# solemnwind/fast-go-icp

Hardware: AMD Instinct MI355X
Metric: BnB subcubes/sec + wall-clock to global optimum, bunny 40k pts, 1/2/4/8 GPU (higher is better)
Workload: dtype f32; 1 GPU; bunny-shape synthetic pair (nt=40256, ns=40097), lut_resolution=0.005, mse_threshold=5e-05, full FastGoICP::run() per step; schedule=round

## Files before the change

fast-go-icp_amd/_lib.py:

```python
import ctypes as C
import os

from . import build as _build

c_float_p = C.POINTER(C.c_float)
c_int_p = C.POINTER(C.c_int)
c_uint32_p = C.POINTER(C.c_uint32)
c_uint8_p = C.POINTER(C.c_uint8)
c_double_p = C.POINTER(C.c_double)


class CtxInfo(C.Structure):
    _fields_ = [("struct_size", C.c_size_t), ("lut_dims", C.c_int * 3), ("lut_layout", C.c_int), ("lut_nodes", C.c_uint64), ("lut_bytes", C.c_uint64),
                ("source_points_per_face_voxel", C.c_double), ("points_per_item", C.c_int), ("items_per_evaluation", C.c_int),
                ("max_subcubes_per_window", C.c_int), ("source_order", C.c_int), ("tree_order", C.c_int), ("chunks_per_item_with_thresholds", C.c_int)]


class CloudStats(C.Structure):
    _fields_ = [("n", C.c_uint64), ("centroid", C.c_float * 3), ("min", C.c_float * 3), ("max", C.c_float * 3), ("max_abs_centred", C.c_float),
                ("rms_radius", C.c_float)]


class Exchange(C.Structure):
    ALLREDUCE_MIN = C.CFUNCTYPE(C.c_int, c_float_p, C.c_size_t, C.c_void_p)
    ALLGATHER = C.CFUNCTYPE(C.c_int, c_float_p, c_float_p, C.c_size_t, C.c_void_p)
    ALLGATHER_DEVICE = C.CFUNCTYPE(C.c_int, C.c_void_p, C.c_size_t, C.c_void_p)
    _fields_ = [("struct_size", C.c_size_t), ("rank", C.c_int), ("world_size", C.c_int), ("allreduce_min", ALLREDUCE_MIN),
                ("allgather", ALLGATHER), ("user", C.c_void_p), ("allgather_device", ALLGATHER_DEVICE)]

    def __init__(self, rank=0, world_size=1, allreduce_min=None, allgather=None, user=None, allgather_device=None):
        super().__init__()
        self.struct_size = C.sizeof(Exchange)
        self.rank, self.world_size, self.user = rank, world_size, user
        if allreduce_min is not None:
            self.allreduce_min = allreduce_min
        if allgather is not None:
            self.allgather = allgather
        if allgather_device is not None:
            self.allgather_device = allgather_device


class SolverOpts(C.Structure):
    _fields_ = [("schedule", C.c_int), ("round_width", C.c_int), ("ctx_flags", C.c_uint), ("device", C.c_int), ("trim_fraction", C.c_float)]


class RunStats(C.Structure):
    _fields_ = [("trans_cubes", C.c_uint64), ("bounds_calls", C.c_uint64), ("rot_cubes", C.c_uint64),
                ("icp_runs", C.c_uint64), ("icp_iters", C.c_uint64), ("inner_bnb", C.c_uint64),
                ("rounds", C.c_uint64), ("seconds_total", C.c_double), ("seconds_bnb", C.c_double),
                ("seconds_icp", C.c_double), ("initial_icp_sse", C.c_double)]

    def as_dict(self):
        return {n: getattr(self, n) for n, _ in self._fields_}


FLAG_NO_WEIGHT_QUANT = 1 << 0
FLAG_NO_MORTON = 1 << 1
FLAG_PROFILE = 1 << 2
FLAG_BRUTE_FORCE_NN = 1 << 3
FLAG_CURVE_ORDER = 1 << 4
class BatchPair(C.Structure):
    _fields_ = [("tgt_xyz", c_float_p), ("nt", C.c_size_t), ("src_xyz", c_float_p), ("ns", C.c_size_t), ("lut_resolution", C.c_float),
                ("mse_threshold", C.c_float)]


class BatchOpts(C.Structure):
    _fields_ = [("struct_size", C.c_size_t), ("solver", SolverOpts), ("max_live", C.c_int), ("trim_fractions", c_float_p),
                ("alignment", C.c_int)]
# ... 130 lines not shown

    def __init__(self):
        super().__init__()
        self.struct_size = C.sizeof(MeshInfo)


OUTLIER_STATISTICAL = 0
OUTLIER_RADIUS = 1

SCHEDULE_SERIAL = 0
SCHEDULE_ROUND = 1

_SIGS = {
    "fgoicp_last_error": (C.c_char_p, []),
    "fgoicp_version": (C.c_char_p, []),
    "fgoicp_dev_knobs": (C.c_int, []),
    "fgoicp_abi_version": (C.c_int, []),
    "fgoicp_ctx_create": (C.c_int, [c_float_p, C.c_size_t, c_float_p, C.c_size_t, c_float_p, C.c_float, C.c_int, C.c_uint,
                                    C.POINTER(C.c_void_p)]),
    "fgoicp_ctx_destroy": (None, [C.c_void_p]),
    "fgoicp_lut_dims": (C.c_int, [C.c_void_p, c_int_p]),
    "fgoicp_ctx_get_info": (C.c_int, [C.c_void_p, C.POINTER(CtxInfo)]),
    "fgoicp_cloud_stats": (C.c_int, [c_float_p, C.c_size_t, C.POINTER(CloudStats)]),
    "fgoicp_voxel_downsample": (C.c_int, [c_float_p, C.c_size_t, C.c_float, c_float_p, C.c_int, c_float_p, C.c_size_t, c_uint32_p, c_uint32_p, C.POINTER(VoxelInfo)]),
    "fgoicp_remove_outliers": (C.c_int, [c_float_p, C.c_size_t, C.c_int, C.c_int, C.c_float, C.c_int, c_float_p, C.c_size_t, c_uint32_p, c_uint8_p, c_double_p, c_float_p,
                                         C.POINTER(OutlierInfo)]),
    "fgoicp_farthest_point_sample": (C.c_int, [c_float_p, C.c_size_t, C.c_size_t, C.c_size_t, C.c_int, c_float_p, c_uint32_p, c_float_p, c_float_p, c_uint32_p,
                                               C.POINTER(FpsInfo)]),
    "fgoicp_cluster_dbscan": (C.c_int, [c_float_p, C.c_size_t, C.c_float, C.c_int, C.c_size_t, C.c_int, c_float_p, C.c_size_t, c_uint32_p, C.POINTER(C.c_int32), c_uint32_p,
                                        C.POINTER(C.c_uint64), C.c_size_t, C.POINTER(ClusterInfo)]),
    "fgoicp_segment_planes": (C.c_int, [c_float_p, C.c_size_t, C.c_float, C.c_int, C.c_uint64, C.c_int, C.c_size_t, C.c_int, C.c_int, C.c_int, c_float_p, C.c_size_t,
                                        c_uint32_p, C.POINTER(C.c_int32), C.POINTER(SegmentModel), C.c_size_t, C.c_size_t, C.POINTER(SegmentInfo)]),
    "fgoicp_segment_hypotheses": (C.c_int, [c_float_p, C.c_size_t, c_uint32_p, C.c_size_t, C.c_int, C.c_uint64, C.c_int, c_uint32_p, C.POINTER(C.c_double), c_uint8_p]),
    "fgoicp_segment_fit_from_moments": (C.c_int, [C.c_uint64, C.POINTER(C.c_double), C.POINTER(C.c_double), C.POINTER(C.c_double), C.POINTER(C.c_double),
                                                  C.POINTER(C.c_double)]),
    "fgoicp_mesh_sample": (C.c_int, [c_float_p, C.c_size_t, c_uint32_p, C.c_size_t, C.c_size_t, C.c_uint64, C.c_int, c_float_p, c_float_p, c_uint32_p, c_double_p, c_double_p,
                                     C.POINTER(MeshInfo)]),
    "fgoicp_solver_set_target_normals": (C.c_int, [C.c_void_p, c_float_p]),
    "fgoicp_solver_set_source_normals": (C.c_int, [C.c_void_p, c_float_p]),
    "fgoicp_lut_read": (C.c_int, [C.c_void_p, c_float_p, C.c_size_t]),
    "fgoicp_lut_search": (C.c_int, [C.c_void_p, c_float_p, C.c_size_t, c_float_p]),
    "fgoicp_lut_nodes": (C.c_int, [C.c_void_p, c_int_p, C.c_size_t, c_float_p]),
    "fgoicp_bounds_point_distances": (C.c_int, [C.c_void_p, c_float_p, C.c_float, c_float_p, C.c_int, c_float_p]),
    "fgoicp_ctx_sort_fallbacks": (C.c_int, [C.c_void_p, C.POINTER(C.c_uint64), C.POINTER(C.c_uint64)]),
    "fgoicp_ctx_test_sort_fault": (C.c_int, [C.c_void_p, C.c_int]),
    "fgoicp_test_live_resources": (C.c_int, [C.POINTER(C.c_uint64)]),
    "fgoicp_bounds_batch": (C.c_int, [C.c_void_p, c_float_p, C.c_float, c_float_p, C.c_int, C.c_int, c_float_p, c_float_p]),
    "fgoicp_bounds_multi": (C.c_int, [C.c_void_p, C.c_int, c_float_p, c_float_p, c_int_p, c_int_p, c_float_p, c_float_p,
                                      c_float_p]),
    "fgoicp_bounds_submit": (C.c_int, [C.c_void_p, C.c_int, C.c_int, c_float_p, c_float_p, c_int_p, c_int_p, c_float_p]),
    "fgoicp_bounds_submit_twins": (C.c_int, [C.c_void_p, C.c_int, C.c_int, c_float_p, c_float_p, c_int_p, c_int_p, c_float_p, c_int_p]),
    "fgoicp_bounds_submit_cut": (C.c_int, [C.c_void_p, C.c_int, C.c_int, c_float_p, c_float_p, c_int_p, c_int_p, c_float_p, c_int_p, c_float_p]),
    "fgoicp_bounds_submit_leaf": (C.c_int, [C.c_void_p, C.c_int, C.c_int, c_float_p, c_float_p, c_int_p, c_int_p, c_float_p, c_int_p, c_float_p, c_float_p]),
    "fgoicp_ctx_cut_stats": (C.c_int, [C.c_void_p, C.POINTER(C.c_uint64), C.POINTER(C.c_uint64), C.c_int]),
    "fgoicp_solver_set_early_exit": (C.c_int, [C.c_void_p, C.c_int]),
    "fgoicp_bounds_collect": (C.c_int, [C.c_void_p, C.c_int, c_float_p, c_float_p]),
    "fgoicp_sse": (C.c_int, [C.c_void_p, c_float_p, c_float_p, c_float_p]),
    "fgoicp_alignment": (C.c_int, [C.c_void_p, c_float_p, c_float_p, c_uint32_p, c_float_p, c_uint8_p, c_uint8_p, C.POINTER(AlignmentSummary)]),
    "fgoicp_solver_alignment": (C.c_int, [C.c_void_p, c_uint32_p, c_float_p, c_uint8_p, c_uint8_p, C.POINTER(AlignmentSummary)]),
    "fgoicp_batch_alignment": (C.c_int, [C.c_void_p, C.c_int, c_uint32_p, c_float_p, c_uint8_p, c_uint8_p, C.POINTER(AlignmentSummary)]),
    "fgoicp_information": (C.c_int, [C.c_void_p, c_float_p, c_float_p, C.c_float, C.POINTER(Information)]),
    "fgoicp_solver_information": (C.c_int, [C.c_void_p, C.c_float, C.POINTER(Information)]),
    "fgoicp_batch_information": (C.c_int, [C.c_void_p, C.c_int, C.POINTER(Information)]),
    "fgoicp_information_from_moments": (C.c_int, [C.c_uint64, C.POINTER(C.c_double), C.POINTER(C.c_double), c_float_p, C.c_float, C.POINTER(C.c_double),
                                                  C.POINTER(C.c_double), C.POINTER(C.c_double)]),
    "fgoicp_ctx_set_target_normals": (C.c_int, [C.c_void_p, c_float_p, C.c_int]),
    "fgoicp_target_normals": (C.c_int, [C.c_void_p, c_float_p]),
    "fgoicp_target_knn": (C.c_int, [C.c_void_p, C.c_int, c_uint32_p, c_float_p]),
    "fgoicp_plane_moments": (C.c_int, [C.c_void_p, c_float_p, c_float_p, C.c_float, C.POINTER(PlaneMoments)]),
    "fgoicp_plane_step_from_moments": (C.c_int, [C.c_uint64, C.POINTER(C.c_double), C.POINTER(C.c_double), c_int_p]),
    "fgoicp_plane_apply_step": (C.c_int, [c_float_p, c_float_p, C.POINTER(C.c_double), c_float_p, c_float_p]),
    "fgoicp_icp_plane": (C.c_int, [C.c_void_p, c_float_p, c_float_p, C.c_size_t, C.c_float, C.c_float, C.POINTER(PlaneResult)]),
    "fgoicp_solver_refine_plane": (C.c_int, [C.c_void_p, C.c_int, C.c_size_t, C.c_float, C.c_float, C.POINTER(PlaneResult)]),
    "fgoicp_ctx_set_source_normals": (C.c_int, [C.c_void_p, c_float_p, C.c_int]),
    "fgoicp_source_normals": (C.c_int, [C.c_void_p, c_float_p]),
    "fgoicp_gicp_moments": (C.c_int, [C.c_void_p, c_float_p, c_float_p, C.c_float, C.c_double, C.POINTER(PlaneMoments)]),
    "fgoicp_icp_gicp": (C.c_int, [C.c_void_p, c_float_p, c_float_p, C.c_size_t, C.c_float, C.c_float, C.c_double, C.POINTER(PlaneResult)]),
    "fgoicp_solver_refine_gicp": (C.c_int, [C.c_void_p, C.c_int, C.c_size_t, C.c_float, C.c_float, C.c_double, C.POINTER(PlaneResult)]),
    "fgoicp_gicp_terms": (C.c_int, [c_float_p, c_float_p, c_float_p, c_float_p, c_float_p, C.c_double, C.POINTER(C.c_double), C.POINTER(C.c_double)]),
    "fgoicp_robust_weight": (C.c_int, [C.c_int, C.c_double, C.c_double, C.POINTER(C.c_double)]),
    "fgoicp_robust_moments": (C.c_int, [C.c_void_p, c_float_p, c_float_p, C.c_float, C.c_int, C.c_double, C.c_int, C.c_double, C.POINTER(RobustMoments)]),
    "fgoicp_robust_residuals": (C.c_int, [C.c_void_p, c_float_p, c_float_p, C.c_float, C.c_int, C.c_double, C.c_int, C.c_double, C.POINTER(C.c_double),
                                          C.POINTER(C.c_double), c_uint8_p]),
    "fgoicp_robust_scale": (C.c_int, [C.c_void_p, c_float_p, c_float_p, C.c_float, C.c_int, C.c_double, C.POINTER(C.c_double)]),
    "fgoicp_icp_robust": (C.c_int, [C.c_void_p, c_float_p, c_float_p, C.c_size_t, C.c_float, C.c_float, C.c_int, C.c_double, C.c_int, C.c_double, C.POINTER(RobustResult)]),
    "fgoicp_solver_refine_robust": (C.c_int, [C.c_void_p, C.c_int, C.c_int, C.c_size_t, C.c_float, C.c_float, C.c_double, C.c_int, C.c_double, C.POINTER(RobustResult)]),
    "fgoicp_icp": (C.c_int, [C.c_void_p, c_float_p, c_float_p, C.c_size_t, C.c_float, c_float_p, c_float_p, c_float_p, c_int_p]),
    "fgoicp_icp_batch": (C.c_int, [C.c_void_p, C.c_int, c_float_p, c_float_p, C.c_size_t, C.c_float, c_float_p, c_float_p, c_float_p, c_int_p]),
    "fgoicp_procrustes": (C.c_int, [C.c_void_p, c_float_p, c_float_p, c_float_p, c_float_p, c_float_p, c_int_p]),
    "fgoicp_ctx_set_inliers": (C.c_int, [C.c_void_p, C.c_size_t]),
    "fgoicp_ctx_profile": (C.c_int, [C.c_void_p, C.POINTER(C.c_double), C.POINTER(C.c_uint64), C.POINTER(C.c_uint64), C.c_int]),
    "fgoicp_ctx_profile_evaluations": (C.c_int, [C.c_void_p, C.POINTER(C.c_uint64)]),
    "fgoicp_ctx_profile_select_ms": (C.c_int, [C.c_void_p, C.POINTER(C.c_double)]),
    "fgoicp_ctx_trim_stats": (C.c_int, [C.c_void_p, C.POINTER(C.c_uint64), C.c_int]),
    "fgoicp_ctx_set_coop_split": (C.c_int, [C.c_void_p, C.c_size_t, C.c_size_t]),
    "fgoicp_ctx_set_profile": (C.c_int, [C.c_void_p, C.c_int]),
    "fgoicp_ctx_ns": (C.c_size_t, [C.c_void_p]),
    "fgoicp_ctx_nt": (C.c_size_t, [C.c_void_p]),
    "fgoicp_solver_create": (C.c_int, [c_float_p, C.c_size_t, c_float_p, C.c_size_t, C.c_float, C.c_float,
                                       C.POINTER(SolverOpts), C.POINTER(C.c_void_p)]),
    "fgoicp_solver_destroy": (None, [C.c_void_p]),
    "fgoicp_solver_set_exchange": (C.c_int, [C.c_void_p, C.POINTER(Exchange)]),
    "fgoicp_solver_set_log": (C.c_int, [C.c_void_p, C.c_void_p, C.c_void_p]),
    "fgoicp_solver_run": (C.c_int, [C.c_void_p, c_float_p, c_float_p]),
    "fgoicp_solver_best_error": (C.c_int, [C.c_void_p, c_float_p]),
    "fgoicp_solver_best_transform": (C.c_int, [C.c_void_p, c_float_p, c_float_p]),
# ... 99 lines not shown
```

fast-go-icp_amd/csrc/device/bounds_item.hpp:

```cpp
#pragma once

constexpr double kCutMargin = 1.000001;

typedef float f2v __attribute__((ext_vector_type(2)));
typedef float f4v __attribute__((ext_vector_type(4)));
typedef unsigned u4v __attribute__((ext_vector_type(4)));

__device__ __forceinline__ f2v pk_fma(f2v a, f2v b, f2v c) { return __builtin_elementwise_fma(a, b, c); }
__device__ __forceinline__ f2v splat2(float v) { return f2v{v, v}; }

struct ItemGeom {
    f2v off_xy, dmax_xy;
    float off_z, dmax_z, scale;
    float pyf;
    int px;
    int c0;
    unsigned nbx3, nby2;
    unsigned nby3;
};
__device__ __forceinline__ ItemGeom item_geom(const LutGeom& g) {
    ItemGeom G;
    G.off_xy = f2v{g.off_x, g.off_y};
    G.dmax_xy = f2v{(float)(g.dx - 1), (float)(g.dy - 1)};
    G.off_z = g.off_z;
// ... 103 lines not shown
            const float4a send = odd ? qp[k].r1 : qp[k].r2;
            float4a recv;
            recv.x = swap_lane_pair(send.x); recv.y = swap_lane_pair(send.y); recv.z = swap_lane_pair(send.z); recv.w = swap_lane_pair(send.w);
            const float4a a = odd ? recv : qp[k].r1, b = odd ? qp[k].r2 : recv;
            ga[k] = f4v{a.x, a.y, a.z, a.w};
            gb[k] = f4v{b.x, b.y, b.z, b.w};
        }
    }
    float te0[TRIM ? P : 1], te1[TRIM ? P : 1];
#pragma unroll
    for (int k = 0; k < P; ++k) {
        float dsq;
        if (LAYOUT == 1 || LAYOUT == 6) dsq = item_blend(tx[k], f2v{ga[k].x, ga[k].y}, f2v{ga[k].z, ga[k].w}, f2v{gb[k].x, gb[k].y}, f2v{gb[k].z, gb[k].w});
        else dsq = item_blend(tx[k], f2v{ga[k].x, ga[k].y}, f2v{gb[k].x, gb[k].y}, f2v{ga[k].z, ga[k].w}, f2v{gb[k].z, gb[k].w});
        const float d1 = sqrtf(dsq);
        const float d0 = d1 - 2.0f * p[k].w * sin_half;
        const int i = first + 64 * k;
        if (TRIM) {
            const float e0 = fmaxf(MODE == 1 ? d0 : d1, 0.0f), e1 = fmaxf(d0, 0.0f);
            if (FULL || i < ns) {
                row0[i] = e0;
                if (MODE == 2) row1[i] = e1;
            }
            te0[k] = e0;
            te1[k] = e1;
            continue;
        }
        if (MODE != 1) {
            const float m = fmaxf(d1, 0.0f), l = fmaxf(d1 - trans_radius, 0.0f);
            const float ubv = m * m, lbv = l * l;
            acc[0] += (FULL || i < ns) ? (double)ubv : 0.0;
            acc[1] += (FULL || i < ns) ? (double)lbv : 0.0;
        }
        if (MODE != 0) {
            const float m = fmaxf(d0, 0.0f), l = fmaxf(d0 - trans_radius, 0.0f);
            const float ubv = m * m, lbv = l * l;
            acc[MODE == 2 ? 2 : 0] += (FULL || i < ns) ? (double)ubv : 0.0;
            acc[MODE == 2 ? 3 : 1] += (FULL || i < ns) ? (double)lbv : 0.0;
        }
    }
    if (TRIM && samp_shift > 0) {
        const size_t off = trim_sample_offset(ns);
#pragma unroll
        for (int k = 0; k < P; ++k) {
            const int i = first + 64 * k;
            if ((FULL || i < ns) && trim_is_sample(i, samp_shift, ns)) {
                row0[off + (size_t)(i >> samp_shift)] = te0[k];
                if (MODE == 2) row1[off + (size_t)(i >> samp_shift)] = te1[k];
            }
        }
    }
}

template <int LAYOUT, int TRIM, bool WIDE, bool QUANT, int MODE>
__device__ __forceinline__ void item_walk(const float4* __restrict__ src, int ns, const char* __restrict__ lutp, const ItemGeom& G, const float (&R)[9], f2v t_xy, float t_z,
                                          float sin_half, float trans_radius, int base, int chunk_pts, int lane, double (&acc)[4], float* __restrict__ row0,
                                          float* __restrict__ row1, int samp_shift) {
    const int odd = lane & 1;
    for (int pass = 0; pass < chunk_pts; pass += 256) {
        const int first = base + pass + lane;
        if (base + pass + 256 <= ns)
            item_pass<LAYOUT, TRIM, WIDE, QUANT, MODE, true>(src, ns, lutp, G, R, t_xy, t_z, sin_half, trans_radius, first, odd, acc, row0, row1, samp_shift);
        else
            item_pass<LAYOUT, TRIM, WIDE, QUANT, MODE, false>(src, ns, lutp, G, R, t_xy, t_z, sin_half, trans_radius, first, odd, acc, row0, row1, samp_shift);
    }
}

template <int LAYOUT, int TRIM, bool WIDE, bool QUANT, bool SPAN >
__global__ __launch_bounds__(64) void bounds_item_kernel(const float4* __restrict__ src, int ns, const char* __restrict__ lutp, LutGeom g,
                                                         const TickGroup* __restrict__ groups, const TickSub* __restrict__ subs, const unsigned* __restrict__ sorted,
                                                         int nchunk, int chunk_pts, double2* __restrict__ partials, float* __restrict__ evals, size_t erow, int samp_shift,
                                                         unsigned nitems, unsigned* __restrict__ sort_err, TickCut cut, int span ) {
    unsigned slot;
    if (!TRIM && cut.tier_split && sorted) {
        const unsigned n0 = min(*cut.tier_split, gridDim.x);
        slot = blockIdx.x < n0 ? xcd_remap(blockIdx.x, n0) : n0 + xcd_remap(blockIdx.x - n0, gridDim.x - n0);
    } else {
        slot = xcd_remap(blockIdx.x, gridDim.x);
    }
    const unsigned item = sorted ? sorted[slot] : slot;
    if (item >= nitems) {
        if (sort_err && threadIdx.x == 0) *sort_err = 1u;
        return;
    }
    const unsigned per_eval = SPAN ? ((unsigned)nchunk + (unsigned)span - 1u) / (unsigned)span : (unsigned)nchunk;
    const int s = (int)(item / per_eval);
    const int chunk0 = (int)(item - (unsigned)s * per_eval) * (SPAN ? span : 1);
    const int nsub = SPAN ? min(span, nchunk - chunk0) : 1;
    const int lane = (int)threadIdx.x;
    const TickSub sb = subs[s];
    bool cutting = false, term0 = false, term1 = false;
    if (!TRIM && cut.acc) {
        TickGate* const gate = cut.gate + s;
        const unsigned long long gw = __hip_atomic_load(reinterpret_cast<unsigned long long*>(gate), __ATOMIC_RELAXED, __HIP_MEMORY_SCOPE_WORKGROUP);
        if (__builtin_amdgcn_readfirstlane((int)(unsigned)gw) && !(cut.probe & 4)) return;
        const unsigned flags = (unsigned)__builtin_amdgcn_readfirstlane((int)(unsigned)(gw >> 32));
        cutting = (flags & kGateCutting) != 0u;
        term0 = (flags & kGateTerm0) != 0u;
        term1 = (flags & kGateTerm1) != 0u;
        if (cutting && !(cut.probe & 1)) {
            const double a0 = __hip_atomic_load(&cut.acc[2 * (size_t)s], __ATOMIC_RELAXED, __HIP_MEMORY_SCOPE_AGENT);
            const double a1 = sb.dual ? __hip_atomic_load(&cut.acc[2 * (size_t)s + 1], __ATOMIC_RELAXED, __HIP_MEMORY_SCOPE_AGENT) : 0.0;
            const bool reached = a0 >= (double)sb.cut0 * kCutMargin && (!sb.dual || a1 >= (double)sb.cut1 * kCutMargin);
            if (__builtin_amdgcn_readfirstlane((int)reached)) {
                if (lane == 0) __hip_atomic_store(&gate->done, 1u, __ATOMIC_RELAXED, __HIP_MEMORY_SCOPE_AGENT);
                return;
            }
        }
    }
    const TickGroup gr = groups[sb.group];
    float R[9];
#pragma unroll
    for (int k = 0; k < 9; ++k) R[k] = gr.R[k];
    const ItemGeom G = item_geom(g);
    const float trans_radius = kSqrt3 * sb.span;
    const f2v t_xy = f2v{sb.tx, sb.ty};
    float* row0 = TRIM ? evals + (size_t)sb.out0 * erow : nullptr;
    float* row1 = TRIM ? evals + (size_t)sb.out1 * erow : nullptr;
    double lb_fix = 0.0, lb_rot = 0.0;
    for (int sub = 0; sub < (SPAN ? nsub : 1); ++sub) {
        const int chunk = chunk0 + sub;
        const int base = chunk * chunk_pts;
        double acc[4] = {0.0, 0.0, 0.0, 0.0};
        if (sb.dual) item_walk<LAYOUT, TRIM, WIDE, QUANT, 2>(src, ns, lutp, G, R, t_xy, sb.tz, gr.sin_half, trans_radius, base, chunk_pts, lane, acc, row0, row1, samp_shift);
        else if (gr.fix_rot) item_walk<LAYOUT, TRIM, WIDE, QUANT, 0>(src, ns, lutp, G, R, t_xy, sb.tz, gr.sin_half, trans_radius, base, chunk_pts, lane, acc, row0, row1, samp_shift);
        else item_walk<LAYOUT, TRIM, WIDE, QUANT, 1>(src, ns, lutp, G, R, t_xy, sb.tz, gr.sin_half, trans_radius, base, chunk_pts, lane, acc, row0, row1, samp_shift);
        if (TRIM) continue;
        const double r0 = wave_sum(acc[0]), r1 = wave_sum(acc[1]);
        lb_fix += term0 ? r0 : r1;
        if (sb.dual) {
            const double r2 = wave_sum(acc[2]), r3 = wave_sum(acc[3]);
            lb_rot += term1 ? r2 : r3;
            if (lane == 0) {
                partials[(size_t)sb.out0 * nchunk + chunk] = make_double2(r0, r1);
                partials[(size_t)sb.out1 * nchunk + chunk] = make_double2(r2, r3);
            }
        } else if (lane == 0) {
            partials[(size_t)sb.out0 * nchunk + chunk] = make_double2(r0, r1);
        }
    }
    if (!TRIM && cutting && lane == 0 && !(cut.probe & 2)) {
        unsafeAtomicAdd(&cut.acc[2 * (size_t)s], lb_fix);
        if (sb.dual) unsafeAtomicAdd(&cut.acc[2 * (size_t)s + 1], lb_rot);
    }
}
```

fast-go-icp_amd/csrc/device/ctx.hip:

```cpp
#include <hip/hip_runtime.h>

#include <algorithm>
#include <chrono>
#include <limits>
#include <memory>
#include <cmath>
#include <cstddef>
#include <cstdio>
#include <cstdlib>
#include <cstring>
#include <numeric>
#include <string>
#include <thread>
#include <vector>

#include "../../../include/fgoicp_amd.h"
#include "../host/math3.hpp"
#include "../host/knobs.hpp"
#include "ctx.hpp"
#include "kernels.hpp"
#include "arena.hpp"
#include "morton.hpp"

namespace fgoicp {
// ... 19 lines not shown
            const hipError_t q = query();
            if (q != hipErrorNotReady) return q;
#if defined(__x86_64__)
            __builtin_ia32_pause();
#endif
            if ((spins & 15u) == 15u && std::chrono::steady_clock::now() - t0 > std::chrono::microseconds(g_spin_sync_us)) break;
        }
    }
    return block();
}
static hipError_t wait_event(hipEvent_t ev) { return spin_then_block([&] { return hipEventQuery(ev); }, [&] { return hipEventSynchronize(ev); }); }
static hipError_t wait_stream(hipStream_t st) { return spin_then_block([&] { return hipStreamQuery(st); }, [&] { return hipStreamSynchronize(st); }); }

int ctx_flush_profile(fgoicp_ctx* c) {
    for (int i = 0; i < c->ev_used; ++i) {
        float ms = 0.f;
        HIPCHK(hipEventElapsedTime(&ms, c->ev_start[i], c->ev_stop[i]));
        c->prof_ms += ms;
        static const bool tick_log = dev_env("FGOICP_TICK_LOG") != nullptr;
        if (tick_log && i < (int)c->ev_evals.size()) std::fprintf(stderr, "[tick] evals %d us %.1f\n", c->ev_evals[i], ms * 1e3);
        if (c->ev_has_sel[i]) {
            HIPCHK(hipEventSynchronize(c->ev_sel_stop[i]));
            HIPCHK(hipEventElapsedTime(&ms, c->ev_sel_start[i], c->ev_sel_stop[i]));
            c->prof_sel_ms += ms;
            c->ev_has_sel[i] = 0;
        }
    }
    c->ev_used = 0;
    return FGOICP_OK;
}

namespace {
struct TickTiming {
    bool on = dev_env("FGOICP_TIMING") != nullptr;
    double pack = 0, enqueue = 0, wait = 0, copyout = 0;
    uint64_t ticks = 0;
};
TickTiming g_tt;
constexpr float kNoCut = std::numeric_limits<float>::infinity();
inline double now_s() { return std::chrono::duration<double>(std::chrono::steady_clock::now().time_since_epoch()).count(); }
}

static int tick_launch_window(fgoicp_ctx* c, fgoicp_ctx::TickSlot& sl) {
    const int ng = sl.win_groups, neval = sl.win_evals, rows = sl.win_rows;
    const int span = sl.win_cut ? c->cut_span : 1;
    const int per_eval = (c->nchunk1 + span - 1) / span;
    const bool tiers = sl.win_cut && c->cut_tier_level > 0.0f;
    const size_t nitems = (size_t)neval * (size_t)per_eval;
    const bool small = nitems <= (size_t)c->small_tick_items;
    const TickGroup* dev_groups = small ? sl.h_groups.dev() : sl.d_groups;
    const TickSub* dev_subs = small ? sl.h_subs.dev() : sl.d_subs;
    TickCut cut;
    if (sl.win_cut) { cut.acc = sl.d_cut_acc; cut.gate = sl.d_cut_gate; cut.row_cut = sl.d_row_cut; cut.row_term = sl.d_row_term; cut.stat = c->d_cut_stat; }
    if (tiers && !small) cut.tier_split = sl.d_cursor + kTickTierSplit;
    static const int cut_probe = [] { const char* e = dev_env("FGOICP_CUT_PROBE"); return e ? std::atoi(e) : 0; }();
    cut.probe = cut_probe;
    *sl.h_sort_err = 0u;
    unsigned* fused_err = !small && c->sort_check ? sl.h_sort_err.dev() : nullptr;
    if (!small) {
        static const int upload_kernel = [] { const char* e = dev_env("FGOICP_UPLOAD_KERNEL"); return e ? std::atoi(e) : 1; }();
        if (upload_kernel) {
            launch_tick_upload(sl.h_groups.dev(), sl.d_groups, ng, sl.h_subs.dev(), sl.d_subs, neval, sl.sort_stream);
        } else {
            HIPCHK(hipMemcpyAsync(sl.d_groups, sl.h_groups, sizeof(TickGroup) * ng, hipMemcpyHostToDevice, sl.sort_stream));
            HIPCHK(hipMemcpyAsync(sl.d_subs, sl.h_subs, sizeof(TickSub) * neval, hipMemcpyHostToDevice, sl.sort_stream));
        }
        ++c->sorted_ticks;
        const int fault = c->sort_fault_tick && c->sorted_ticks == (uint64_t)c->sort_fault_tick;
        launch_tick_sort(c->geom, span > 1 ? c->d_span_cen : c->d_chunk_cen, per_eval, sl.d_groups, sl.d_subs, neval, c->cell_shift, sl.d_keys, sl.d_ranks, sl.d_hist, sl.d_hist_xcd, sl.d_xoff, sl.d_block_sums, sl.d_cursor, sl.d_sorted,
                         c->sort_xcd ? 1 : 0, c->sort_check ? 1 : 0, fault, sl.sort_stream, tiers ? c->d_lut : nullptr, c->cut_tier_level / (float)c->ns,
                         sl.win_cut ? &cut : nullptr, sl.d_partials, c->nchunk1, span);
        HIPCHK(hipEventRecord(sl.sorted_ev, sl.sort_stream));
        HIPCHK(hipStreamWaitEvent(sl.stream, sl.sorted_ev, 0));
    } else if (sl.win_cut) {
        launch_tick_prefill(dev_subs, neval, c->nchunk1, cut, sl.d_partials, sl.stream);
    }
    hipEvent_t e0 = nullptr, e1 = nullptr;
    if (c->profile) {
        if (c->ev_used == (int)c->ev_start.size()) {
            HIPCHK(hipStreamSynchronize(c->stream));
            int rc = ctx_flush_profile(c);
            if (rc) return rc;
        }
        e0 = c->ev_start[c->ev_used];
        e1 = c->ev_stop[c->ev_used];
        if ((int)c->ev_evals.size() <= c->ev_used) c->ev_evals.resize(c->ev_start.size(), 0);
        c->ev_evals[c->ev_used] = neval;
        c->ev_used++;
        c->prof_launches++;
        c->prof_subcubes += rows;
        c->prof_evals += neval;
    }
    const bool cut_on = launch_bounds_sorted(c->d_src, (int)c->ns, c->d_lut_zp, c->lut_layout, c->geom, c->nchunk1, c->chunk_pts, dev_groups, dev_subs, neval, small ? nullptr : sl.d_sorted,
                                             sl.d_partials, c->inliers ? sl.d_evals : nullptr, c->erow, c->trim_samp_shift, fused_err, cut, span, e0, e1, sl.stream);
    if (cut_on) c->cut_items_offered += (size_t)neval * c->nchunk1;
    hipStream_t fin = c->finalize_on_side ? sl.sort_stream : sl.stream;
    if (fin != sl.stream) {
        HIPCHK(hipEventRecord(sl.bounds_ev, sl.stream));
        HIPCHK(hipStreamWaitEvent(fin, sl.bounds_ev, 0));
    }
    if (c->inliers) {
        const int pi = e0 ? c->ev_used - 1 : -1;
        if (pi >= 0) { HIPCHK(hipEventRecord(c->ev_sel_start[pi], fin)); c->ev_has_sel[pi] = 1; }
        launch_trim_rows(sl.d_evals, c->erow, (int)c->ns, (int)c->inliers, rows, sl.h_row_span.dev(), sl.h_ub.dev(), sl.h_lb.dev(), fin, c->trim_samp_shift, c->trim_margin, c->d_trim_stat);
        if (pi >= 0) HIPCHK(hipEventRecord(c->ev_sel_stop[pi], fin));
    } else
        launch_bounds_finalize(sl.d_partials, c->nchunk1, rows, sl.h_lb.dev(), sl.h_ub.dev(), cut_on ? cut : TickCut(), fin);
    HIPCHK(hipGetLastError());
    HIPCHK(hipEventRecord(sl.done, fin));
    return FGOICP_OK;
}

static int tick_enqueue_window(fgoicp_ctx* c, fgoicp_ctx::TickSlot& sl, int G, const float* R9, const float* rot_span, const int* fix_rot,
                               const int* offsets, const float* tn4, const int* twin, const float* cut_above, const float* ub_below_span, int pos, int* end_out) {
    const double t0 = g_tt.on ? now_s() : 0;
    int g = 0;
    while (g < G && offsets[g + 1] <= pos) ++g;
    const int cap = c->inliers ? std::min(c->max_subcubes, c->vals_rows) : c->max_subcubes;
    int end = pos, ng = 0;
    sl.row_group.resize((size_t)cap);
    for (int gg = g; gg < G && ng < c->max_groups && end - pos < cap; ++gg) {
        TickGroup& tg = sl.h_groups[ng];
        std::memcpy(tg.R, R9 + 9 * gg, sizeof(tg.R));
        const float half_angle = rot_span[gg] * kSqrt3 * kPi / 2.0f;
        tg.sin_half = std::sin(half_angle);
        tg.fix_rot = fix_rot[gg] ? 1 : 0;
        tg.pad_ = gg;
        const int first = std::max(offsets[gg], pos);
        const int last = std::min(offsets[gg + 1], pos + cap);
        for (int i = first; i < last; ++i) sl.row_group[(size_t)(i - pos)] = ng;
        end = std::max(end, last);
        ++ng;
        if (last < offsets[gg + 1]) break;
    }
    const int rows = end - pos;
    *end_out = end;
    if (rows <= 0) return FGOICP_OK;
    static const bool leaf_rule = [] { const char* e = dev_env("FGOICP_CUT_LEAF"); return !e || std::atoi(e) != 0; }();
    const auto terminal = [&](int sub_group, float span) { return leaf_rule && cut_above && ub_below_span && span < ub_below_span[sub_group]; };
    int neval = 0;
    for (int r = 0; r < rows; ++r) {
        const int i = pos + r;
        const int gi = sl.row_group[(size_t)r];
        sl.h_row_span[r] = tn4[4 * (size_t)i + 3];
        int j = twin ? twin[i] : -1;
        if (j >= pos && j < end && j != i && twin[j] == i) {
            const int gj = sl.row_group[(size_t)(j - pos)];
            const TickGroup &a = sl.h_groups[gi], &b = sl.h_groups[gj];
            const bool ok = a.fix_rot != b.fix_rot && a.sin_half == b.sin_half && std::memcmp(a.R, b.R, sizeof(a.R)) == 0 &&
                            std::memcmp(tn4 + 4 * (size_t)i, tn4 + 4 * (size_t)j, 4 * sizeof(float)) == 0;
            if (ok) {
                if (j < i) continue;
                TickSub& ts = sl.h_subs[neval++];
                ts.tx = tn4[4 * (size_t)i]; ts.ty = tn4[4 * (size_t)i + 1]; ts.tz = tn4[4 * (size_t)i + 2]; ts.span = tn4[4 * (size_t)i + 3];
                ts.group = gi;
                ts.out0 = a.fix_rot ? r : j - pos;
                ts.out1 = a.fix_rot ? j - pos : r;
                ts.dual = 1;
                const float ca = cut_above ? cut_above[a.pad_] : kNoCut, cb = cut_above ? cut_above[b.pad_] : kNoCut;
                ts.cut0 = a.fix_rot ? ca : cb;
                ts.cut1 = a.fix_rot ? cb : ca;
                const unsigned ta = terminal(a.pad_, ts.span) ? 1u : 0u, tb = terminal(b.pad_, ts.span) ? 1u : 0u;
                ts.term = a.fix_rot ? (ta * kSubTerm0 | tb * kSubTerm1) : (tb * kSubTerm0 | ta * kSubTerm1);
                ts.pad_ = 0;
                continue;
            }
        }
        TickSub& ts = sl.h_subs[neval++];
        ts.tx = tn4[4 * (size_t)i]; ts.ty = tn4[4 * (size_t)i + 1]; ts.tz = tn4[4 * (size_t)i + 2]; ts.span = tn4[4 * (size_t)i + 3];
        ts.group = gi;
        ts.out0 = r;
        ts.out1 = r;
        ts.dual = 0;
        ts.cut0 = ts.cut1 = cut_above ? cut_above[sl.h_groups[gi].pad_] : kNoCut;
        ts.term = terminal(sl.h_groups[gi].pad_, ts.span) ? kSubTerm0 : 0u;
        ts.pad_ = 0;
    }
    sl.win_cut = cut_above != nullptr && !c->inliers;
    for (int k = 0; k < ng; ++k) sl.h_groups[k].pad_ = 0;
    const double t1 = g_tt.on ? now_s() : 0;
    sl.win_pos = pos;
    sl.win_rows = rows;
    sl.win_groups = ng;
    sl.win_evals = neval;
    const int rc = tick_launch_window(c, sl);
    if (g_tt.on) { g_tt.pack += t1 - t0; g_tt.enqueue += now_s() - t1; g_tt.ticks++; }
    return rc;
}

static int tick_wait_window(fgoicp_ctx* c, fgoicp_ctx::TickSlot& sl) {
    const double t2 = g_tt.on ? now_s() : 0;
    HIPCHK(wait_event(sl.done));
    if (*sl.h_sort_err) {
        c->sort_xcd = false;
        c->sort_fallbacks++;
        HIPCHK(hipStreamSynchronize(sl.sort_stream));
        HIPCHK(hipMemsetAsync(sl.d_hist, 0, sizeof(unsigned) * kTickNumKeys, sl.sort_stream));
        HIPCHK(hipMemsetAsync(sl.d_hist_xcd, 0, sizeof(unsigned) * 16 * kTickNumKeys, sl.sort_stream));
        int rc = tick_launch_window(c, sl);
        if (rc) return rc;
        HIPCHK(hipEventSynchronize(sl.done));
        if (*sl.h_sort_err) { set_error("tick sort did not produce a permutation of the work items (device-scope atomics)"); return FGOICP_ERR_HIP; }
    }
#ifdef FGOICP_DEV_KNOBS
    const bool cut_verify = [] { const char* e = dev_env("FGOICP_CUT_VERIFY"); return e && std::atoi(e) != 0; }();
    if (cut_verify && sl.win_cut) {
        const int rows = sl.win_rows;
        std::vector<float> lb(sl.h_lb.get(), sl.h_lb + rows), ub(sl.h_ub.get(), sl.h_ub + rows);
        sl.win_cut = false;
        int rc = tick_launch_window(c, sl);
        sl.win_cut = true;
        if (rc) return rc;
        HIPCHK(hipEventSynchronize(sl.done));
        if (*sl.h_sort_err) { set_error("FGOICP_CUT_VERIFY: the repeated window's sort failed"); return FGOICP_ERR_HIP; }
        for (int e = 0; e < sl.win_evals; ++e) {
            const TickSub& ts = sl.h_subs[e];
            for (int v = 0; v < (ts.dual ? 2 : 1); ++v) {
                const int r = v ? ts.out1 : ts.out0;
                const float T = v ? ts.cut1 : ts.cut0;
                const bool term = (ts.term & (v ? kSubTerm1 : kSubTerm0)) != 0u;
                const bool above = (term ? sl.h_ub[r] : sl.h_lb[r]) >= T;
                const bool ok = above ? (lb[(size_t)r] == T && ub[(size_t)r] == T)
                                      : (std::memcmp(&lb[(size_t)r], &sl.h_lb[r], 4) == 0 && std::memcmp(&ub[(size_t)r], &sl.h_ub[r], 4) == 0);
                c->cut_verify_rows++;
                c->cut_verify_above += above ? 1 : 0;
                if (!ok) {
                    if (c->cut_verify_bad++ < 5)
                        std::fprintf(stderr, "[fgoicp cut verify] row %d: threshold %.9g, exact {%.9g, %.9g}, reported {%.9g, %.9g}\n", r, (double)T, (double)sl.h_lb[r], (double)sl.h_ub[r],
                                     (double)lb[(size_t)r], (double)ub[(size_t)r]);
                }
            }
        }
        c->cut_verify_windows++;
        std::memcpy(sl.h_lb, lb.data(), sizeof(float) * rows);
        std::memcpy(sl.h_ub, ub.data(), sizeof(float) * rows);
    }
#endif
    const double t3 = g_tt.on ? now_s() : 0;
    std::memcpy(sl.lb.data() + sl.win_pos, sl.h_lb, sizeof(float) * sl.win_rows);
    std::memcpy(sl.ub.data() + sl.win_pos, sl.h_ub, sizeof(float) * sl.win_rows);
    if (g_tt.on) { g_tt.wait += t3 - t2; g_tt.copyout += now_s() - t3; }
    return FGOICP_OK;
}

int ctx_bounds_submit(fgoicp_ctx* c, int slot, int G, const float* R9, const float* rot_span, const int* fix_rot, const int* offsets,
                      const float* tn4, const int* twin, const float* cut_above, const float* ub_below_span) {
    HIPCHK(hipSetDevice(c->device));
    fgoicp_ctx::TickSlot& sl = c->slots[slot];
    if (sl.inflight) { set_error("fgoicp_bounds_submit: slot still in flight (collect it first)"); return FGOICP_ERR_INVALID_ARG; }
    sl.total = offsets[G];
    sl.lb.resize(sl.total);
    sl.ub.resize(sl.total);
    sl.win_rows = 0;
    int pos = 0;
    while (pos < sl.total) {
        int end = pos;
        int rc = tick_enqueue_window(c, sl, G, R9, rot_span, fix_rot, offsets, tn4, twin, cut_above, ub_below_span, pos, &end);
        if (rc) return rc;
        if (end <= pos) break;
        pos = end;
        if (pos < sl.total) {
            rc = tick_wait_window(c, sl);
            if (rc) return rc;
            sl.win_rows = 0;
        }
    }
    sl.inflight = true;
    return FGOICP_OK;
}

int ctx_cut_stats(fgoicp_ctx* c, uint64_t* items_offered, uint64_t* items_cut, int reset) {
    HIPCHK(hipSetDevice(c->device));
    unsigned long long now = 0;
    if (c->d_cut_stat) {
        unsigned long long part[kCutStatSlots];
        HIPCHK(hipDeviceSynchronize());
        HIPCHK(hipMemcpy(part, c->d_cut_stat, sizeof(part), hipMemcpyDeviceToHost));
        for (unsigned long long v : part) now += v;
    }
    if (items_offered) *items_offered = c->cut_items_offered;
    if (items_cut) *items_cut = (uint64_t)now - c->cut_stat_base;
    if (reset) { c->cut_items_offered = 0; c->cut_stat_base = (uint64_t)now; }
    return FGOICP_OK;
}

int ctx_bounds_collect(fgoicp_ctx* c, int slot, float* lb_out, float* ub_out) {
    HIPCHK(hipSetDevice(c->device));
    fgoicp_ctx::TickSlot& sl = c->slots[slot];
    if (!sl.inflight) { set_error("fgoicp_bounds_collect: nothing submitted on this slot"); return FGOICP_ERR_INVALID_ARG; }
    if (sl.win_rows > 0) {
        int rc = tick_wait_window(c, sl);
        if (rc) return rc;
    }
    sl.inflight = false;
    std::memcpy(lb_out, sl.lb.data(), sizeof(float) * sl.total);
    std::memcpy(ub_out, sl.ub.data(), sizeof(float) * sl.total);
    if (c->profile && !c->slots[0].inflight && !c->slots[1].inflight) {
        int rc = ctx_flush_profile(c);
        if (rc) return rc;
    }
    return FGOICP_OK;
}

int ctx_bounds_multi(fgoicp_ctx* c, int G, const float* R9, const float* rot_span, const int* fix_rot, const int* offsets,
                     const float* tn4, float* lb_out, float* ub_out, const float* cut_above) {
    HIPCHK(hipSetDevice(c->device));
    int rc = ctx_bounds_submit(c, 0, G, R9, rot_span, fix_rot, offsets, tn4, nullptr, cut_above);
    if (rc) return rc;
    return ctx_bounds_collect(c, 0, lb_out, ub_out);
}

static double tree64(double (&v)[64]) {
    for (int off = 32; off > 0; off >>= 1)
        for (int i = 0; i < off; ++i) v[i] += v[i + off];
    return v[0];
}
static double fold_blocks(const double* bp, int nblocks, int width, int k) {
    double lane[64] = {0};
    for (int b = 0; b < nblocks; ++b) lane[b & 63] += bp[(size_t)b * width + k];
    return tree64(lane);
}
static double fold_wave_sums(const double* w, int nwaves) {
    double lane[64] = {0};
    const int nblocks = (nwaves + 3) / 4;
    for (int b = 0; b < nblocks; ++b) {
        double blk = w[4 * b];
        for (int k = 1; k < 4; ++k) blk += 4 * b + k < nwaves ? w[4 * b + k] : 0.0;
        lane[b & 63] += blk;
    }
    return tree64(lane);
}
static bool icp_fused(const fgoicp_ctx* c) { return c->icp_fuse && !c->brute_force_nn && !c->inliers && c->ns <= 262144; }

static bool trim_skips(const fgoicp_ctx* c) { return c->inliers && c->trim_skip; }

// ... 1027 lines not shown
    if (c->brute_force_nn) {
        Dev<float4> d_tgt_shift;
        e3 = d_tgt_shift.alloc(nt);
        if (e3 == hipSuccess) e3 = hipMemcpy(d_tgt_shift, hs.data(), sizeof(float4) * nt, hipMemcpyHostToDevice);
        if (e3 == hipSuccess) {
            launch_lut_build(d_tgt_shift, (int)nt, g, c->d_lut, c->stream);
            e3 = hipGetLastError();
            if (e3 == hipSuccess) e3 = hipStreamSynchronize(c->stream);
        }
    } else {
        std::vector<uint32_t> order;
        c->tree_order = bvh_kd_order() ? 1 : 0;
        HIPCHK(bvh_upload(bvh_build_host(h.data(), nt, &order), &c->bvh_tgt));
        BvhOwned shifted;
        e3 = bvh_upload(bvh_build_host(hs.data(), nt, &order), &shifted);
        Dev<float> scratch;
        if (e3 == hipSuccess) e3 = scratch.alloc(total);
        static const bool want_idx = [] { const char* e = dev_env("FGOICP_LUT_INDEX"); return e && std::atoi(e) != 0; }();
        if (e3 == hipSuccess && want_idx && c->d_lut_idx.alloc(total) != hipSuccess) (void)hipGetLastError();
        if (e3 == hipSuccess) {
            launch_lut_build_scan(shifted.view(), g, scratch, c->d_lut, c->stream, c->d_lut_idx);
            e3 = hipGetLastError();
            if (e3 == hipSuccess) e3 = hipStreamSynchronize(c->stream);
        }
    }
    if (e3 != hipSuccess) { set_error(std::string("LUT build failed: ") + hipGetErrorString(e3)); return e3 == hipErrorOutOfMemory ? FGOICP_ERR_OOM : FGOICP_ERR_HIP; }
    g.idx = c->d_lut_idx;
    return FGOICP_OK;
}
int create_packed_lut(fgoicp_ctx* c) {
    const LutGeom& g = c->geom;
    const size_t total = (size_t)g.px * g.py * g.pz;
    const double face_voxels = (double)g.dx * g.dy + (double)g.dy * g.dz + (double)g.dx * g.dz;
    int layout = ((double)c->ns / face_voxels < 0.5 && total * sizeof(float4) <= ((size_t)16 << 30)) ? 2 : 1;
    const size_t apron_bytes = packed_lut_bytes(g, 4);
    if (layout == 2 && apron_bytes <= ((size_t)16 << 30)) layout = 4;
    if (layout == 4 && apron_bytes > ((size_t)256 << 20)) layout = 6;
    if (const char* e = dev_env("FGOICP_LUT_ZPAIR")) { const int v = std::atoi(e); if (v == 1 || v == 2 || v == 4 || v == 6) layout = v; }
    if ((layout == 4 || layout == 6) && (g.px > 1023 || g.py > 1023 || g.pz > 1023)) layout = 2;
    c->lut_layout = layout;
    if (layout == 6) {
        HIPCHK(c->d_lut_zp.alloc(packed_lut_bytes(g, 6) / sizeof(float2)));
        launch_lut_zpair_apron(c->d_lut, g, c->d_lut_zp, c->stream);
    } else if (layout == 4) {
        HIPCHK(c->d_lut_zp.alloc(apron_bytes / sizeof(float2)));
        launch_lut_quad_apron(c->d_lut, g, reinterpret_cast<float4*>(c->d_lut_zp.get()), c->stream);
    } else if (layout == 2) {
        HIPCHK(c->d_lut_zp.alloc(total * 2));
        launch_lut_quad(c->d_lut, g, reinterpret_cast<float4*>(c->d_lut_zp.get()), c->stream);
    } else {
        HIPCHK(c->d_lut_zp.alloc(total));
        launch_lut_zpair(c->d_lut, g, c->d_lut_zp, c->stream);
    }
    HIPCHK(hipGetLastError());
    HIPCHK(hipStreamSynchronize(c->stream));
    return FGOICP_OK;
}
int create_window_sizes(fgoicp_ctx* c) {
    const LutGeom& g = c->geom;
    const size_t ns = c->ns;
    const double face_voxels = (double)g.dx * g.dy + (double)g.dy * g.dz + (double)g.dx * g.dz;
    const double density = (double)ns / face_voxels;
    c->chunk_pts = density >= 1.0 ? 2048 : density >= 0.5 ? 1024 : density >= 0.25 ? 512 : 256;
    if (const char* e = dev_env("FGOICP_CHUNK_PTS")) {
        const int v = std::atoi(e);
        if (v == 256 || v == 512 || v == 1024 || v == 2048 || v == 4096) c->chunk_pts = v;
    }
    const size_t nchunk1 = (ns + c->chunk_pts - 1) / c->chunk_pts;
    const size_t fit = ((size_t)4 << 30) / (nchunk1 * (sizeof(double2) + 2 * sizeof(unsigned) + sizeof(unsigned short)));
    c->max_subcubes = (int)std::max<size_t>(4096, std::min<size_t>(131072, fit));
    if (const char* e = dev_env("FGOICP_MAX_SUBCUBES")) c->max_subcubes = std::max(kMaxBatch, std::min(1 << 18, std::atoi(e)));
    const size_t launch_fit = (((size_t)1 << 24) - 1) / nchunk1;
    if (launch_fit < (size_t)kMaxBatch) {
        set_error("fgoicp_ctx_create: source cloud too large for one bounds launch per batch (ns > ~134M)");
        return FGOICP_ERR_TOO_LARGE;
    }
    c->max_subcubes = (int)std::min<size_t>((size_t)c->max_subcubes, launch_fit);
    c->nchunk1 = (int)nchunk1;
    c->max_groups = std::max(512, c->max_subcubes / 8);
    if (const char* e = dev_env("FGOICP_FINALIZE_SIDE")) c->finalize_on_side = std::atoi(e) != 0;
    if (const char* e = dev_env("FGOICP_ICP_SEED")) c->icp_seeding = std::atoi(e) != 0;
    if (const char* e = dev_env("FGOICP_COOP_SPLIT_MIN")) c->coop_split_min = c->coop_split_trim_min = (size_t)std::max(0L, std::atol(e));
    if (const char* e = dev_env("FGOICP_SMALL_TICK")) c->small_tick_items = std::max(0, std::atoi(e));
    const int maxd = std::max(g.dx, std::max(g.dy, g.dz));
    c->cell_shift = 0;
    while ((maxd >> c->cell_shift) > 32) ++c->cell_shift;
    c->cut_span = c->chunk_pts == 256 ? 2 : 1;
    if (const char* e = dev_env("FGOICP_CUT_TIERS")) c->cut_tier_level = (float)std::atof(e);
    if (const char* e = dev_env("FGOICP_CUT_SPAN")) { const int v = std::atoi(e); if (v == 1 || v == 2 || v == 4) c->cut_span = v; }
    return FGOICP_OK;
}
int create_run_centres(fgoicp_ctx* c, const float* src_xyz, size_t pts, Dev<float4>& d_cen) {
    const size_t ns = c->ns, n = (ns + pts - 1) / pts;
    std::vector<float4> cen(n);
    for (size_t k = 0; k < n; ++k) {
        double sx = 0, sy = 0, sz = 0;
        const size_t a = k * pts, b = std::min(ns, a + pts);
        for (size_t i = a; i < b; ++i) {
            const float* p = src_xyz + 3 * (size_t)c->perm[i];
            sx += p[0]; sy += p[1]; sz += p[2];
        }
        const double inv = 1.0 / (double)(b - a);
        cen[k] = make_float4((float)(sx * inv), (float)(sy * inv), (float)(sz * inv), 0.f);
    }
    HIPCHK(d_cen.alloc(n));
    HIPCHK(hipMemcpy(d_cen, cen.data(), sizeof(float4) * n, hipMemcpyHostToDevice));
    return FGOICP_OK;
}
int create_tick_slot(fgoicp_ctx* c, fgoicp_ctx::TickSlot& sl) {
    const size_t subcubes = (size_t)c->max_subcubes, max_items = subcubes * c->nchunk1;
    sl.stream.borrow(c->stream);
    HIPCHK(sl.done.create(hipEventDisableTiming));
    const char* e = dev_env("FGOICP_SORT_STREAM");
    if (e && std::atoi(e) == 0) sl.sort_stream.borrow(c->stream);
    else {
        const char* pe = dev_env("FGOICP_SIDE_PRIORITY");
        const int pri = pe ? std::atoi(pe) : 0;
        int least = 0, greatest = 0;
        if (pri) HIPCHK(hipDeviceGetStreamPriorityRange(&least, &greatest));
        if (pri) HIPCHK(sl.sort_stream.create(hipStreamNonBlocking, pri < 0 ? greatest : least));
        else HIPCHK(sl.sort_stream.create(hipStreamNonBlocking));
    }
    for (Event* ev : {&sl.sorted_ev, &sl.bounds_ev}) HIPCHK(ev->create(hipEventDisableTiming));
    HIPCHK(sl.d_groups.alloc(c->max_groups));
    HIPCHK(sl.d_subs.alloc(subcubes));
    HIPCHK(sl.h_groups.alloc(c->max_groups));
    HIPCHK(sl.h_subs.alloc(subcubes));
    HIPCHK(sl.h_row_span.alloc(subcubes));
    HIPCHK(sl.h_sort_err.alloc(4));
    *sl.h_sort_err = 0u;
    HIPCHK(sl.d_keys.alloc(max_items));
    HIPCHK(sl.d_ranks.alloc(max_items));
    HIPCHK(sl.d_hist.alloc(kTickNumKeys));
    HIPCHK(hipMemset(sl.d_hist, 0, sizeof(unsigned) * kTickNumKeys));
    HIPCHK(sl.d_block_sums.alloc(64));
    HIPCHK(sl.d_hist_xcd.alloc(16 * kTickNumKeys));
    HIPCHK(hipMemset(sl.d_hist_xcd, 0, sizeof(unsigned) * 16 * kTickNumKeys));
    HIPCHK(sl.d_xoff.alloc(16 * kTickNumKeys));
    HIPCHK(sl.d_cursor.alloc(kTickNumKeys));
    HIPCHK(sl.d_sorted.alloc(max_items));
    HIPCHK(sl.d_partials.alloc(max_items));
    HIPCHK(sl.d_cut_acc.alloc(2 * subcubes));
    HIPCHK(hipMemset(sl.d_cut_acc, 0, sizeof(double) * 2 * subcubes));
    static_assert(sizeof(float) == sizeof(unsigned), "d_row_term is the second half of d_row_cut's allocation");
    HIPCHK(sl.d_row_cut.alloc(2 * subcubes));
    sl.d_row_term = reinterpret_cast<unsigned*>(sl.d_row_cut + subcubes);
    HIPCHK(sl.d_cut_gate.alloc(subcubes));
    if (!c->d_cut_stat) { HIPCHK(c->d_cut_stat.alloc(kCutStatSlots)); HIPCHK(hipMemset(c->d_cut_stat, 0, sizeof(unsigned long long) * kCutStatSlots)); }
    for (Mapped<float>* h : {&sl.h_lb, &sl.h_ub}) HIPCHK(h->alloc(subcubes));
    return FGOICP_OK;
}
int create_icp_lane(fgoicp_ctx* c, fgoicp_ctx::IcpLane& L, bool first) {
    const size_t ns = c->ns;
    if (first) L.stream.borrow(c->stream);
    else HIPCHK(L.stream.create(hipStreamNonBlocking));
    HIPCHK(L.d_work.alloc(ns));
    HIPCHK(L.d_min_bits.alloc(ns));
    if (first) HIPCHK(L.d_thr_bits.alloc(ns));
    for (Dev<uint32_t>* d : {&L.d_first_idx, &L.d_first_idx2}) HIPCHK(d->alloc(ns));
    for (Dev<double>* d : {&L.d_bp, &L.d_bp2, &L.d_bp3}) HIPCHK(d->alloc(1024 * 16));
    HIPCHK(L.icp_stream.create(hipStreamNonBlocking));
    for (Event* e : {&L.icp_ev_w, &L.icp_ev_b}) HIPCHK(e->create(hipEventDisableTiming));
    HIPCHK(L.d_cen.alloc(8));
    HIPCHK(L.h_cen.alloc(8));
    HIPCHK(L.h_sums.alloc(16));
    HIPCHK(L.d_wsum.alloc(4096 * 6));
    HIPCHK(L.h_wsse.alloc(4096));
    HIPCHK(L.h_covbp.alloc(1024 * 9));
    return FGOICP_OK;
}
}

template <class T, class Launch>
static int lut_query(fgoicp_ctx* c, const T* q, size_t n, float* out, Launch launch) {
    if (!c || !q || !out) return FGOICP_ERR_INVALID_ARG;
    if (n == 0) return FGOICP_OK;
    HIPCHK(hipSetDevice(c->device));
    Dev<T> dq;
    Dev<float> dout;
    HIPCHK(dq.alloc(3 * n));
    hipError_t e = dout.alloc(n);
    if (e == hipSuccess) e = hipMemcpyAsync(dq, q, 3 * n * sizeof(T), hipMemcpyHostToDevice, c->stream);
    if (e == hipSuccess) { launch(dq.get(), dout.get()); e = hipGetLastError(); }
    if (e == hipSuccess) e = hipMemcpyAsync(out, dout, n * sizeof(float), hipMemcpyDeviceToHost, c->stream);
    if (e == hipSuccess) e = hipStreamSynchronize(c->stream);
    HIPCHK(e);
    return FGOICP_OK;
}

}

using namespace fgoicp;

static RefineSpec refine_spec(bool weighted, float max_dist2, int model, double epsilon, int loss, double scale) {
    RefineSpec r;
    r.weighted = weighted; r.model = model; r.epsilon = epsilon; r.loss = loss; r.scale = scale; r.max_dist2 = max_dist2;
// ... 83 lines not shown
    *out = nullptr;
    const CreateArgs a{tgt_xyz, nt, src_xyz, ns, bounds6, lut_resolution, device, flags};
    return fgoicp::abi_guard("fgoicp_ctx_create", [&] { return ctx_create_impl(a, out); });
}

fgoicp_ctx::~fgoicp_ctx() {
    (void)hipSetDevice(device);
    stream.sync();
    for (auto& L : lanes) { L.stream.sync(); L.icp_stream.sync(); }
    for (auto& sl : slots) sl.sort_stream.sync();
}

void fgoicp_ctx_destroy(fgoicp_ctx* c) {
    if (!c) return;
    if (c->cut_verify_windows)
        std::fprintf(stderr, "[fgoicp cut verify] %llu windows with thresholds evaluated again without them: %llu rows, %llu of them at or above their threshold, %llu violations of the contract\n",
                     (unsigned long long)c->cut_verify_windows, (unsigned long long)c->cut_verify_rows, (unsigned long long)c->cut_verify_above, (unsigned long long)c->cut_verify_bad);
    if (g_tt.on && g_tt.ticks) {
        std::fprintf(stderr, "[fgoicp timing] ticks %llu: pack %.1f us, enqueue %.1f us, wait %.1f us, copyout %.1f us per tick\n", (unsigned long long)g_tt.ticks,
                     1e6 * g_tt.pack / g_tt.ticks, 1e6 * g_tt.enqueue / g_tt.ticks, 1e6 * g_tt.wait / g_tt.ticks, 1e6 * g_tt.copyout / g_tt.ticks);
        g_tt = TickTiming{};
    }
    delete c;
}

int fgoicp_lut_dims(const fgoicp_ctx* c, int* dims3) {
    if (!c || !dims3) return FGOICP_ERR_INVALID_ARG;
    dims3[0] = c->geom.dx; dims3[1] = c->geom.dy; dims3[2] = c->geom.dz;
    return FGOICP_OK;
}

int fgoicp_ctx_get_info(const fgoicp_ctx* c, fgoicp_ctx_info* out) {
    if (!c || !out) return FGOICP_ERR_INVALID_ARG;
    const size_t caller = out->struct_size;
    if (caller < offsetof(fgoicp_ctx_info, lut_layout)) { set_error("fgoicp_ctx_get_info: set struct_size = sizeof(fgoicp_ctx_info) before the call"); return FGOICP_ERR_INVALID_ARG; }
    fgoicp_ctx_info full{};
    fgoicp_ctx_info* const user_out = out;
    out = &full;
    const LutGeom& g = c->geom;
    *out = fgoicp_ctx_info{};
    out->lut_dims[0] = g.dx; out->lut_dims[1] = g.dy; out->lut_dims[2] = g.dz;
    out->lut_layout = c->d_lut_zp ? c->lut_layout : 0;
    out->lut_nodes = (uint64_t)g.dx * g.dy * g.dz;
    const uint64_t padded = (uint64_t)g.px * g.py * g.pz;
    const size_t packed = c->d_lut_zp ? packed_lut_bytes(g, c->lut_layout) : 0;
    out->lut_bytes = padded * sizeof(float) + packed + (c->d_lut_idx ? padded * sizeof(uint32_t) : 0);
    out->source_points_per_face_voxel = (double)c->ns / ((double)g.dx * g.dy + (double)g.dy * g.dz + (double)g.dx * g.dz);
    out->points_per_item = c->chunk_pts;
    out->items_per_evaluation = c->nchunk1;
    out->max_subcubes_per_window = c->max_subcubes;
    out->source_order = c->source_order;
    out->tree_order = c->tree_order;
    out->chunks_per_item_with_thresholds = c->cut_span;
    full.struct_size = caller < sizeof(full) ? caller : sizeof(full);
    std::memcpy(user_out, &full, full.struct_size);
    return FGOICP_OK;
}

int fgoicp_lut_read(fgoicp_ctx* c, float* out, size_t capacity) {
    if (!c || !out) return FGOICP_ERR_INVALID_ARG;
    const size_t total = (size_t)c->geom.dx * c->geom.dy * c->geom.dz;
    if (capacity < total) { set_error("fgoicp_lut_read: buffer too small"); return FGOICP_ERR_INVALID_ARG; }
    HIPCHK(hipSetDevice(c->device));
    Dev<float> d;
    HIPCHK(d.alloc(total));
    launch_lut_unpad(c->d_lut, c->geom, d, c->stream);
    HIPCHK(hipMemcpyAsync(out, d, total * sizeof(float), hipMemcpyDeviceToHost, c->stream));
    HIPCHK(hipStreamSynchronize(c->stream));
    return FGOICP_OK;
}

int fgoicp_lut_nodes(fgoicp_ctx* c, const int* xyz, size_t n, float* out) {
    return lut_query(c, xyz, n, out, [&](const int* dq, float* dout) { launch_lut_nodes(c->d_lut, c->geom, dq, n, dout, c->stream); });
}
int fgoicp_lut_search(fgoicp_ctx* c, const float* q, size_t n, float* out) {
    return lut_query(c, q, n, out, [&](const float* dq, float* dout) { launch_lut_search(c->d_lut, c->geom, dq, n, dout, c->stream); });
}

int fgoicp_bounds_multi(fgoicp_ctx* c, int G, const float* R9, const float* rot_span, const int* fix_rot, const int* offsets,
                        const float* tn4, float* lb_out, float* ub_out) {
    if (!c || G < 0 || (G > 0 && (!R9 || !rot_span || !fix_rot || !offsets || !tn4 || !lb_out || !ub_out))) return FGOICP_ERR_INVALID_ARG;
    if (G == 0) return FGOICP_OK;
    for (int g = 0; g < G; ++g)
        if (offsets[g + 1] < offsets[g] || offsets[0] != 0) { set_error("fgoicp_bounds_multi: offsets must start at 0 and be non-decreasing"); return FGOICP_ERR_INVALID_ARG; }
    if (offsets[G] == 0) return FGOICP_OK;
    return ctx_bounds_multi(c, G, R9, rot_span, fix_rot, offsets, tn4, lb_out, ub_out);
}

int fgoicp_bounds_submit_twins(fgoicp_ctx* c, int slot, int G, const float* R9, const float* rot_span, const int* fix_rot, const int* offsets,
                               const float* tn4, const int* twin) {
    return fgoicp_bounds_submit_cut(c, slot, G, R9, rot_span, fix_rot, offsets, tn4, twin, nullptr);
}

int fgoicp_bounds_submit_cut(fgoicp_ctx* c, int slot, int G, const float* R9, const float* rot_span, const int* fix_rot, const int* offsets,
                             const float* tn4, const int* twin, const float* cut_above) {
    return fgoicp_bounds_submit_leaf(c, slot, G, R9, rot_span, fix_rot, offsets, tn4, twin, cut_above, nullptr);
}

int fgoicp_bounds_submit_leaf(fgoicp_ctx* c, int slot, int G, const float* R9, const float* rot_span, const int* fix_rot, const int* offsets,
                              const float* tn4, const int* twin, const float* cut_above, const float* ub_below_span) {
    if (!c || slot < 0 || slot > 1 || G < 0 || (G > 0 && (!R9 || !rot_span || !fix_rot || !offsets || !tn4))) return FGOICP_ERR_INVALID_ARG;
    static const int zero[1] = {0};
    if (G == 0) offsets = zero;
    for (int g = 0; g < G; ++g)
        if (offsets[g + 1] < offsets[g] || offsets[0] != 0) { set_error("fgoicp_bounds_submit: offsets must start at 0 and be non-decreasing"); return FGOICP_ERR_INVALID_ARG; }
    return ctx_bounds_submit(c, slot, G, R9, rot_span, fix_rot, offsets, tn4, twin, cut_above, ub_below_span);
}

int fgoicp_ctx_cut_stats(fgoicp_ctx* c, uint64_t* items_offered, uint64_t* items_cut, int reset) {
    if (!c) return FGOICP_ERR_INVALID_ARG;
    return ctx_cut_stats(c, items_offered, items_cut, reset);
}

int fgoicp_bounds_submit(fgoicp_ctx* c, int slot, int G, const float* R9, const float* rot_span, const int* fix_rot, const int* offsets,
                         const float* tn4) {
    return fgoicp_bounds_submit_twins(c, slot, G, R9, rot_span, fix_rot, offsets, tn4, nullptr);
}

int fgoicp_bounds_collect(fgoicp_ctx* c, int slot, float* lb_out, float* ub_out) {
    if (!c || slot < 0 || slot > 1 || !lb_out || !ub_out) return FGOICP_ERR_INVALID_ARG;
    return ctx_bounds_collect(c, slot, lb_out, ub_out);
}

int fgoicp_bounds_batch(fgoicp_ctx* c, const float* R9, float rot_span, const float* tn4, int B, int fix_rot, float* lb_out, float* ub_out) {
    if (B < 0) return FGOICP_ERR_INVALID_ARG;
    const int offsets[2] = {0, B};
    return fgoicp_bounds_multi(c, 1, R9, &rot_span, &fix_rot, offsets, tn4, lb_out, ub_out);
}

int fgoicp_bounds_point_distances(fgoicp_ctx* c, const float* R9, float rot_span, const float* tnode4, int fix_rot, float* e_out) {
    if (!c || !R9 || !tnode4 || !e_out) return FGOICP_ERR_INVALID_ARG;
    if (!c->inliers) { set_error("fgoicp_bounds_point_distances: trimming is off (fgoicp_ctx_set_inliers)"); return FGOICP_ERR_INVALID_ARG; }
    const int offsets[2] = {0, 1};
    float lb = 0.f, ub = 0.f;
    int rc = ctx_bounds_submit(c, 0, 1, R9, &rot_span, &fix_rot, offsets, tnode4, nullptr);
    if (rc) return rc;
    rc = ctx_bounds_collect(c, 0, &lb, &ub);
    if (rc) return rc;
    std::vector<float> row(c->ns);
    HIPCHK(hipMemcpy(row.data(), c->slots[0].d_evals, sizeof(float) * c->ns, hipMemcpyDeviceToHost));
    for (size_t i = 0; i < c->ns; ++i) e_out[c->perm[i]] = row[i];
    return FGOICP_OK;
}

int fgoicp_ctx_test_sort_fault(fgoicp_ctx* c, int nth_tick) {
    if (!c || nth_tick < 0) return FGOICP_ERR_INVALID_ARG;
    c->sort_fault_tick = nth_tick ? (int)c->sorted_ticks + nth_tick : 0;
    return FGOICP_OK;
}

int fgoicp_test_live_resources(uint64_t out4[4]) {
    if (!out4) return FGOICP_ERR_INVALID_ARG;
    out4[0] = live::dev; out4[1] = live::pinned; out4[2] = live::streams; out4[3] = live::events;
    return FGOICP_OK;
}

int fgoicp_ctx_sort_fallbacks(const fgoicp_ctx* c, uint64_t* sorted_ticks, uint64_t* fallbacks) {
    if (!c) return FGOICP_ERR_INVALID_ARG;
    if (sorted_ticks) *sorted_ticks = c->sorted_ticks;
// ... 219 lines not shown
```

fast-go-icp_amd/csrc/device/ctx.hpp:

```cpp
#pragma once
#include <exception>
#include <new>
#include <string>
#include <hip/hip_runtime.h>

#include <cstdint>
#include <cstring>
#include <string>
#include <vector>

#include "../host/math3.hpp"
#include "../host/icp_loop.hpp"
#include "../host/abi_guard.hpp"
#include "../host/information.hpp"
#include "../host/plane.hpp"
#include "../host/gicp.hpp"
#include "../host/robust.hpp"
#include "bvh.hpp"
#include "kernels.hpp"
#include "owned.hpp"

struct fgoicp_ctx {
    ~fgoicp_ctx();
    int device = 0;
    fgoicp::Stream stream;
    size_t ns = 0, nt = 0;
    bool profile = false;

    fgoicp::Dev<float4> d_src;
    fgoicp::Dev<float4> d_tgt;
    fgoicp::Dev<float> d_lut;
    int lut_layout = 1;
    int source_order = 0, tree_order = 0;
    fgoicp::Dev<uint32_t> d_lut_idx;
    fgoicp::Dev<float2> d_lut_zp;
    fgoicp::LutGeom geom{};
    fgoicp::BvhOwned bvh_tgt;
    bool brute_force_nn = false;
    std::vector<uint32_t> perm;

    int max_subcubes = 0;

    struct TickSlot {
        fgoicp::Stream stream;
        fgoicp::Event done;
        fgoicp::Stream sort_stream;
        fgoicp::Event bounds_ev;
        fgoicp::Event sorted_ev;
        fgoicp::Dev<fgoicp::TickGroup> d_groups; fgoicp::Mapped<fgoicp::TickGroup> h_groups;
        fgoicp::Dev<fgoicp::TickSub> d_subs; fgoicp::Mapped<fgoicp::TickSub> h_subs;
        fgoicp::Dev<unsigned short> d_keys;
        fgoicp::Dev<unsigned> d_ranks;
        fgoicp::Dev<unsigned> d_hist, d_block_sums, d_cursor, d_sorted;
        fgoicp::Dev<unsigned> d_hist_xcd, d_xoff;
        fgoicp::Dev<double2> d_partials;
        fgoicp::Dev<double> d_cut_acc;
        fgoicp::Dev<float> d_row_cut;
        unsigned* d_row_term = nullptr;
        fgoicp::Dev<fgoicp::TickGate> d_cut_gate;
        bool win_cut = false;
        fgoicp::Mapped<float> h_lb, h_ub;
        fgoicp::Dev<float> d_evals;
        fgoicp::Mapped<float> h_row_span;
        fgoicp::Mapped<unsigned> h_sort_err;
        int win_groups = 0, win_evals = 0;
        std::vector<float> lb, ub;
        std::vector<int> row_group;
        int total = 0, win_pos = 0, win_rows = 0;
        bool inflight = false;
    };
    fgoicp::Dev<unsigned long long> d_cut_stat;
    uint64_t cut_items_offered = 0;
    uint64_t cut_verify_windows = 0, cut_verify_rows = 0, cut_verify_above = 0, cut_verify_bad = 0;
    uint64_t cut_stat_base = 0;
    bool sort_xcd = true;
    bool sort_check = true;
    int sort_fault_tick = 0;
    uint64_t sorted_ticks = 0, sort_fallbacks = 0;
    int nchunk1 = 0, max_groups = 0, cell_shift = 4;
    int chunk_pts = 256;
    bool finalize_on_side = true;
    int small_tick_items = 4096;
    size_t coop_split_min = (size_t)-1;
    size_t coop_split_trim_min = 262144;
    bool icp_seeding = true;
    fgoicp::Dev<float4> d_chunk_cen;
    float cut_tier_level = 0.5f;
    int cut_span = 1;
    fgoicp::Dev<float4> d_span_cen;
    TickSlot slots[2];

    size_t inliers = 0;
    int vals_rows = 0;
    size_t erow = 0;
    int trim_samp_shift = 5;
    float trim_margin_sd = 1.0f;
    int trim_margin = 0;
    fgoicp::Dev<uint32_t> d_coop;
    size_t coop_cap = 0;
    fgoicp::Dev<unsigned long long> d_trim_stat;
    uint64_t trim_stat_acc[3] = {0, 0, 0};
    bool trim_ready = false;
    bool trim_skip = true;
    float bounds6[6] = {0, 0, 0, 0, 0, 0};
    float tgt_box6[6] = {0, 0, 0, 0, 0, 0};
    fgoicp::Dev<uint32_t> d_orig_of_slot;

    struct AlignScratch {
        fgoicp::Dev<char> base;
        uint32_t* d_idx = nullptr;
        uint32_t* d_corr = nullptr;
        float* d_d2 = nullptr;
        unsigned char *d_inl = nullptr, *d_hit = nullptr;
        uint2* d_partials = nullptr;
        uint32_t* d_sum = nullptr;
        size_t nt16 = 0;
        fgoicp::MomentRow<fgoicp::kAlignInfoTerms>* d_info_rows = nullptr;
        unsigned long long* d_info = nullptr;
    } align;

    fgoicp::Dev<float4> d_normals;
    bool normals_set = false;
    fgoicp::Dev<float4> d_src_normals;
    bool src_normals_set = false;
    fgoicp::Dev<fgoicp::MomentRow<fgoicp::kPlaneTerms>> d_plane_rows;
    fgoicp::Dev<fgoicp::MomentRow<fgoicp::kRobustTerms>> d_robust_rows;
    fgoicp::Dev<unsigned long long> d_refine_out;
    fgoicp::Dev<double> d_robust_point;
    fgoicp::Dev<unsigned char> d_robust_counted;
    fgoicp::Event refine_ready;

    struct IcpLane {
        fgoicp::Stream stream;
        fgoicp::Stream icp_stream;
        fgoicp::Event icp_ev_w, icp_ev_b;
        fgoicp::Dev<float4> d_work;
        fgoicp::Dev<uint32_t> d_min_bits, d_thr_bits, d_first_idx, d_first_idx2;
        fgoicp::Dev<double> d_bp, d_bp2, d_bp3;
        fgoicp::Mapped<double> h_sums;
        fgoicp::Dev<float> d_cen;
        fgoicp::Mapped<float> h_cen;
        fgoicp::Dev<float> d_d2;
        fgoicp::Dev<float> d_nn_lb, d_nn_ub, d_nn_lb2, d_nn_ub2;
        fgoicp::Dev<uint32_t> d_sel, d_eq, d_sel_wide, d_sel_wide2;
        fgoicp::Dev<unsigned char> d_use;
        fgoicp::Mapped<float> h_trim;
        fgoicp::Dev<double> d_wsum;
        fgoicp::Mapped<double> h_wsse;
        fgoicp::Mapped<double> h_covbp;
        bool cov_on_host = false, sse_on_host = false;
        int cov_blocks = 0;
    };
    std::vector<IcpLane> lanes;
    bool icp_overlap = true;
    bool icp_fuse = true;
    int icp_dual_env = -1;

    std::vector<fgoicp::Event> ev_start, ev_stop, ev_sel_start, ev_sel_stop;
    std::vector<char> ev_has_sel;
    std::vector<int> ev_evals;
    double prof_sel_ms = 0.0, prof_sel_ms_last = 0.0;
    int ev_used = 0;
    double prof_ms = 0.0;
    uint64_t prof_launches = 0, prof_subcubes = 0, prof_evals = 0;
};

namespace fgoicp {
void set_error(const std::string& s);

int ctx_bounds_multi(fgoicp_ctx* c, int G, const float* R9, const float* rot_span, const int* fix_rot, const int* offsets,
                     const float* tn4, float* lb_out, float* ub_out, const float* cut_above = nullptr);
int ctx_cut_stats(fgoicp_ctx* c, uint64_t* items_offered, uint64_t* items_cut, int reset);
int ctx_bounds_submit(fgoicp_ctx* c, int slot, int G, const float* R9, const float* rot_span, const int* fix_rot, const int* offsets, const float* tn4,
                      const int* twin = nullptr, const float* cut_above = nullptr, const float* ub_below_span = nullptr);
int ctx_bounds_collect(fgoicp_ctx* c, int slot, float* lb_out, float* ub_out);
int ctx_set_inliers(fgoicp_ctx* c, size_t k);
inline unsigned trim_ctx_flags(unsigned flags, float f) { return flags | (f > 0.0f ? (unsigned)FGOICP_FLAG_CURVE_ORDER : 0u); }
inline size_t trim_inliers(size_t ns, float f) {
    if (!(f > 0.0f)) return 0;
    size_t k = (size_t)((double)ns * (1.0 - (double)f));
    if (k < 1) k = 1;
    return k < ns ? k : 0;
}
int ctx_set_inliers_batch(fgoicp_ctx* c, size_t k);
size_t trim_rows_budget(size_t free_bytes);
size_t trim_icp_bytes(size_t ns, size_t lanes);
int ctx_sse(fgoicp_ctx* c, const float* R9, const float* t3, float* sse_out, const uint32_t* seed_idx = nullptr);
int ctx_alignment(fgoicp_ctx* c, const float* R9, const float* t3, uint32_t* corr_idx, float* dist2, uint8_t* inlier, uint8_t* target_hit,
                  fgoicp_alignment_summary* out);
int ctx_information(fgoicp_ctx* c, const float* R9, const float* t3, float max_dist2, InfoMoments* m);
int ctx_alignment_information(fgoicp_ctx* c, const float* R9, const float* t3, uint32_t* corr_idx, float* dist2, uint8_t* inlier, uint8_t* target_hit,
                              fgoicp_alignment_summary* out, float max_dist2, InfoMoments* m);
int ctx_set_target_normals(fgoicp_ctx* c, const float* normals, int k);
int ctx_target_normals(fgoicp_ctx* c, float* out_nt3);
int ctx_target_knn(fgoicp_ctx* c, int k, uint32_t* idx, float* d2);
int ctx_set_source_normals(fgoicp_ctx* c, const float* normals, int k);
int ctx_source_normals(fgoicp_ctx* c, float* out_ns3);
struct RefineSpec {
    int model = FGOICP_MODEL_PLANE;
    double epsilon = 1e-3;
    bool weighted = false;
    int loss = FGOICP_LOSS_NONE;
    double scale = 0.0;
    float max_dist2 = 0.f;
};
enum class ScaleCheck { none, given, or_estimated };
int refine_refusals(const fgoicp_ctx* c, const RefineSpec& r, ScaleCheck scale, const char* where);
int refine_evaluate(fgoicp_ctx* c, const float* R9, const float* t3, const RefineSpec& r, RefineMoments* m, float* sse_out = nullptr, double* residual = nullptr,
                    double* weight = nullptr, unsigned char* counted = nullptr);
int ctx_robust_scale(fgoicp_ctx* c, const float* R9, const float* t3, const RefineSpec& r, double* scale, const char* where);
struct RefineEnd {
    Mat3f R;
    Vec3f t;
    RefineMoments m;
    float sse = 0.f;
    int iterations = 0, rank = 0;
    RefineSpec spec;
    int scale_estimated = 0;
};
int refine_loop(fgoicp_ctx* c, const float* R0, const float* t0, size_t max_iter, float thr, const RefineSpec& spec, const char* where, RefineEnd* end);
struct RefineStepRun {
    RefineEnd end;
    size_t max_iter = 0;
    float thr = 0.f;
    std::string where;
    bool stop = false, done = false;
    int evaluations = 0;
// ... 33 lines not shown
```

fast-go-icp_amd/csrc/device/kernels.hip:

```cpp
#include "kernels.hpp"

#include <algorithm>
#include <cstdio>
#include <cstdlib>

#include "../host/knobs.hpp"
#include "dist_sq.hpp"
#include "slab.hpp"
#include "bvh.hpp"
#include "../host/math3.hpp"
#include "../host/gicp.hpp"
#include "../host/robust.hpp"

namespace fgoicp {
namespace {

typedef float float2u __attribute__((ext_vector_type(2), aligned(4)));

struct Rt {
    float R[9];
    float t[3];
};

__device__ __forceinline__ void rotate(const float* R, float x, float y, float z, float& ox, float& oy, float& oz) {
// ... 135 lines not shown
__global__ __launch_bounds__(kBlock) void lut_quad_kernel(const float* __restrict__ lut, LutGeom g, float4* __restrict__ qd) {
    const size_t total = (size_t)g.px * g.py * g.pz, sy = (size_t)g.px, sz = (size_t)g.px * g.py;
    for (size_t n = (size_t)blockIdx.x * kBlock + threadIdx.x; n < total; n += (size_t)gridDim.x * kBlock) {
        const size_t nz = n + sz < total ? n + sz : n, ny = n + sy < total ? n + sy : n, nyz = n + sy + sz < total ? n + sy + sz : n;
        qd[n] = make_float4(lut[n], lut[nz], lut[ny], lut[nyz]);
    }
}

__global__ __launch_bounds__(kBlock) void lut_zpair_kernel(const float* __restrict__ lut, LutGeom g, float2* __restrict__ zp) {
    const size_t total = (size_t)g.px * g.py * g.pz, sz = (size_t)g.px * g.py;
    for (size_t n = (size_t)blockIdx.x * kBlock + threadIdx.x; n < total; n += (size_t)gridDim.x * kBlock)
        zp[n] = make_float2(lut[n], n + sz < total ? lut[n + sz] : lut[n]);
}

__device__ __forceinline__ unsigned xcd_remap(unsigned id, unsigned total) {
    const unsigned q = total >> 3, r = total & 7u, xcd = id & 7u, k = id >> 3;
    return (xcd < r ? xcd * (q + 1) : r * (q + 1) + (xcd - r) * q) + k;
}

constexpr int kKeyBits = 15;
constexpr int kNumKeys = 1 << kKeyBits;

__device__ __forceinline__ unsigned part1by2_5(unsigned v) {
    v &= 31u;
    v = (v | (v << 8)) & 0x100fu;
    v = (v | (v << 4)) & 0x10c3u;
    v = (v | (v << 2)) & 0x1249u;
    return v;
}

__device__ __forceinline__ unsigned hilbert15(unsigned x, unsigned y, unsigned z) {
    unsigned X[3] = {x & 31u, y & 31u, z & 31u};
#pragma unroll
    for (unsigned Q = 16u; Q > 1u; Q >>= 1) {
        const unsigned P = Q - 1u;
#pragma unroll
        for (int i = 0; i < 3; ++i) {
            if (X[i] & Q) X[0] ^= P;
            else { const unsigned t = (X[0] ^ X[i]) & P; X[0] ^= t; X[i] ^= t; }
        }
    }
    X[1] ^= X[0];
    X[2] ^= X[1];
    unsigned t = 0;
#pragma unroll
    for (unsigned Q = 16u; Q > 1u; Q >>= 1)
        if (X[2] & Q) t ^= Q - 1u;
    X[0] ^= t; X[1] ^= t; X[2] ^= t;
    return part1by2_5(X[2]) | (part1by2_5(X[1]) << 1) | (part1by2_5(X[0]) << 2);
}

constexpr int kTickXcds = 16;

__device__ __forceinline__ void cut_prefill(const TickSub& sb, int s, int chunk_first, int chunk_end, int row_chunks, const TickCut& cut, double2* __restrict__ partials) {
    const bool cutting = sb.cut0 < kCutNone && (!sb.dual || sb.cut1 < kCutNone);
    if (chunk_first == 0) {
        *reinterpret_cast<uint2*>(cut.gate + s) = make_uint2(0u, (cutting ? kGateCutting : 0u) | sb.term << 1);
        cut.row_cut[sb.out0] = sb.cut0;
        cut.row_term[sb.out0] = sb.term & kSubTerm0;
        if (sb.dual) { cut.row_cut[sb.out1] = sb.cut1; cut.row_term[sb.out1] = sb.term & kSubTerm1; }
    }
    if (!cutting) return;
    for (int chunk = chunk_first; chunk < chunk_end; ++chunk) {
        partials[(size_t)sb.out0 * row_chunks + chunk] = make_double2(-1.0, (double)sb.cut0);
        if (sb.dual) partials[(size_t)sb.out1 * row_chunks + chunk] = make_double2(0.0, (double)sb.cut1);
    }
}
__global__ __launch_bounds__(64) void tick_prefill_kernel(const TickSub* __restrict__ subs, int nsub, int nchunk, TickCut cut, double2* __restrict__ partials) {
    const size_t nitems = (size_t)nsub * nchunk;
    for (size_t i = (size_t)blockIdx.x * 64 + threadIdx.x; i < nitems; i += (size_t)gridDim.x * 64) {
        const int s = (int)(i / nchunk), c = (int)(i - (size_t)s * nchunk);
        cut_prefill(subs[s], s, c, c + 1, nchunk, cut, partials);
    }
}

template <int XCD>
__global__ __launch_bounds__(64) void tick_keys_kernel(const float4* __restrict__ chunk_cen, int nchunk, const TickGroup* __restrict__ groups,
                                                       const TickSub* __restrict__ subs, int nsub, LutGeom g, int cell_shift,
                                                       unsigned short* __restrict__ keys, unsigned* __restrict__ ranks, unsigned* __restrict__ hist,
                                                       unsigned* __restrict__ prefill ,
                                                       const float* __restrict__ tier_lut , float tier_level,
                                                       TickCut cut, double2* __restrict__ partials ,
                                                       int row_chunks, int span) {
    const size_t nitems = (size_t)nsub * nchunk;
    for (size_t i = (size_t)blockIdx.x * 64 + threadIdx.x; i < nitems; i += (size_t)gridDim.x * 64) {
        if (prefill) prefill[i] = 0xFFFFFFFFu;
        const int s = (int)(i / nchunk), c = (int)(i - (size_t)s * nchunk);
        const TickSub sb = subs[s];
        if (partials) cut_prefill(sb, s, c * span, min(c * span + span, row_chunks), row_chunks, cut, partials);
        const TickGroup& gr = groups[sb.group];
        const float4 cc = chunk_cen[c];
        float rx, ry, rz;
        rotate(gr.R, cc.x, cc.y, cc.z, rx, ry, rz);
        const int vx = (int)fminf(fmaxf((rx + sb.tx + g.off_x) * g.scale, 0.0f), (float)(g.dx - 1)) >> cell_shift;
        const int vy = (int)fminf(fmaxf((ry + sb.ty + g.off_y) * g.scale, 0.0f), (float)(g.dy - 1)) >> cell_shift;
        const int vz = (int)fminf(fmaxf((rz + sb.tz + g.off_z) * g.scale, 0.0f), (float)(g.dz - 1)) >> cell_shift;
        unsigned key = hilbert15((unsigned)vx, (unsigned)vy, (unsigned)vz);
        if (tier_lut) {
            const int ix = (int)fminf(fmaxf((rx + sb.tx + g.off_x) * g.scale, 0.0f), (float)(g.dx - 1));
            const int iy = (int)fminf(fmaxf((ry + sb.ty + g.off_y) * g.scale, 0.0f), (float)(g.dy - 1));
            const int iz = (int)fminf(fmaxf((rz + sb.tz + g.off_z) * g.scale, 0.0f), (float)(g.dz - 1));
            const float d = sqrtf(tier_lut[((size_t)(iz + 1) * g.py + (size_t)(iy + 1)) * g.px + (size_t)(ix + 1)]);
            const float r_rot = 2.0f * gr.sin_half * sqrtf(cc.x * cc.x + cc.y * cc.y + cc.z * cc.z);
            const bool term0 = (sb.term & kSubTerm0) != 0u, term1 = (sb.term & kSubTerm1) != 0u;
            const float e_fix = fmaxf(d - (term0 ? 0.0f : kSqrt3 * sb.span), 0.0f);
            const float e_rot = fmaxf(d - ((sb.dual ? term1 : term0) ? 0.0f : kSqrt3 * sb.span) - r_rot, 0.0f);
            bool heavy;
            if (sb.dual) heavy = e_fix * e_fix >= tier_level * sb.cut0 && e_rot * e_rot >= tier_level * sb.cut1;
            else heavy = (gr.fix_rot ? e_fix * e_fix : e_rot * e_rot) >= tier_level * sb.cut0;
            key = (key >> 1) | (heavy ? 0u : 1u << 14);
        }
        keys[i] = (unsigned short)key;
        if (XCD) {
// ... 501 lines not shown
    use[i] = u < vk ? 1 : (u == vk ? 2 : 0);
    if (u == vk) atomicAdd(equal_count, 1u);
}
__global__ __launch_bounds__(1024) void icp_inlier_ties_kernel(int n, const uint32_t* __restrict__ sel_info, const uint32_t* __restrict__ equal_count,
                                                               const uint32_t* __restrict__ orig_of_slot, unsigned char* __restrict__ use) {
    const uint32_t need = sel_info[1];
    if (*equal_count == need) {
        for (int i = blockIdx.x * 1024 + threadIdx.x; i < n; i += gridDim.x * 1024)
            if (use[i] == 2) use[i] = 1;
        return;
    }
    if (blockIdx.x != 0) return;
    __shared__ unsigned hist[2048];
    __shared__ unsigned s_bin, s_below;
    const int tid = threadIdx.x;
    unsigned prefix = 0, mask = 0, want = need;
    for (int lvl = 0; lvl < 3; ++lvl) {
        const int shift = lvl == 0 ? 21 : lvl == 1 ? 10 : 0, nb = lvl == 2 ? 1024 : 2048;
        for (int q = tid; q < 2048; q += 1024) hist[q] = 0;
        __syncthreads();
        for (int i = tid; i < n; i += 1024) {
            if (use[i] != 2) continue;
            const unsigned o = orig_of_slot[i];
            if ((o & mask) == prefix) atomicAdd(&hist[(o >> shift) & (nb - 1)], 1u);
        }
        __syncthreads();
        if (tid == 0) {
            unsigned below = 0;
            int q = 0;
            for (; q < nb - 1; ++q) {
                if (want <= below + hist[q]) break;
                below += hist[q];
            }
            s_bin = (unsigned)q;
            s_below = below;
        }
        __syncthreads();
        prefix |= s_bin << shift;
        mask |= (unsigned)(nb - 1) << shift;
        want -= s_below;
        __syncthreads();
    }
    for (int i = tid; i < n; i += 1024)
        if (use[i] == 2) use[i] = orig_of_slot[i] <= prefix ? 1 : 0;
}

__global__ __launch_bounds__(64) void bounds_finalize_kernel(const double2* __restrict__ partials, int nchunk, int total,
                                                             float* __restrict__ out_lb, float* __restrict__ out_ub, TickCut cut) {
    const int s = blockIdx.x;
    if (s >= total) return;
    const double2* row = partials + (size_t)s * nchunk;
    double u = 0.0, l = 0.0;
    unsigned skipped = 0;
    for (int c = threadIdx.x; c < nchunk; c += 64) {
        const double2 v = row[c];
        skipped += v.x < 0.0 ? 1u : 0u;
        u += v.x;
        l += v.y;
    }
    u = wave_sum(u);
    l = wave_sum(l);
    if (cut.stat) {
        for (int off = 32; off > 0; off >>= 1) skipped += __shfl_down(skipped, off);
        if (threadIdx.x == 0 && skipped) atomicAdd(&cut.stat[s & (kCutStatSlots - 1)], (unsigned long long)skipped);
    }
    if (threadIdx.x == 0) {
        float ubf = (float)u, lbf = (float)l;
        if (cut.row_cut) {
            const float T = cut.row_cut[s];
            if (lbf >= T || (cut.row_term[s] && ubf >= T)) lbf = ubf = T;
        }
        out_ub[s] = ubf;
        out_lb[s] = lbf;
    }
    if (cut.acc && threadIdx.x < 2) cut.acc[2 * (size_t)s + threadIdx.x] = 0.0;
}

constexpr int kLutNodes = 4;
constexpr int kTile = 1024;

__global__ __launch_bounds__(kBlock) void lut_build_kernel(const float4* __restrict__ tgt, int nt, LutGeom g, float* __restrict__ lut) {
    __shared__ float4 tile[kTile];
    const size_t total = (size_t)g.px * g.py * g.pz;
    const size_t base = (size_t)blockIdx.x * (kBlock * kLutNodes) + threadIdx.x;
    float cx[kLutNodes], cy[kLutNodes], cz[kLutNodes], m[kLutNodes];
#pragma unroll
    for (int k = 0; k < kLutNodes; ++k) {
        size_t n = base + (size_t)k * kBlock;
        if (n >= total) n = total - 1;
        const int x = (int)(n % g.px);
        const size_t r = n / g.px;
        const int y = (int)(r % g.py);
        const int z = (int)(r / g.py);
        cx[k] = (float)min(max(x - 1, 0), g.dx - 1) * g.resolution;
        cy[k] = (float)min(max(y - 1, 0), g.dy - 1) * g.resolution;
        cz[k] = (float)min(max(z - 1, 0), g.dz - 1) * g.resolution;
        m[k] = 3.402823466e+38f;
    }
    for (int t0 = 0; t0 < nt; t0 += kTile) {
        const int cnt = min(kTile, nt - t0);
        for (int j = threadIdx.x; j < cnt; j += kBlock) tile[j] = tgt[t0 + j];
        __syncthreads();
        for (int j = 0; j < cnt; ++j) {
            const float4 p = tile[j];
#pragma unroll
            for (int k = 0; k < kLutNodes; ++k) {
                const float d = dist_sq(cx[k], cy[k], cz[k], p.x, p.y, p.z);
                m[k] = m[k] < d ? m[k] : d;
            }
        }
        __syncthreads();
    }
#pragma unroll
    for (int k = 0; k < kLutNodes; ++k) {
        const size_t n = base + (size_t)k * kBlock;
        if (n < total) lut[n] = m[k];
    }
}

__global__ __launch_bounds__(kBlock) void lut_unpad_kernel(const float* __restrict__ lut, LutGeom g, float* __restrict__ out) {
    const size_t total = (size_t)g.dx * g.dy * g.dz;
    for (size_t n = (size_t)blockIdx.x * kBlock + threadIdx.x; n < total; n += (size_t)gridDim.x * kBlock) {
        const int x = (int)(n % g.dx);
        const size_t r = n / g.dx;
        const int y = (int)(r % g.dy);
        const int z = (int)(r / g.dy);
        out[n] = lut[((size_t)(z + 1) * g.py + (y + 1)) * g.px + (x + 1)];
    }
}

__global__ __launch_bounds__(kBlock) void lut_nodes_kernel(const float* __restrict__ lut, LutGeom g, const int* __restrict__ xyz, size_t n, float* __restrict__ out) {
    for (size_t i = (size_t)blockIdx.x * kBlock + threadIdx.x; i < n; i += (size_t)gridDim.x * kBlock) {
        const int x = min(max(xyz[3 * i], 0), g.dx - 1), y = min(max(xyz[3 * i + 1], 0), g.dy - 1), z = min(max(xyz[3 * i + 2], 0), g.dz - 1);
        out[i] = lut[((size_t)(z + 1) * g.py + (y + 1)) * g.px + (x + 1)];
    }
}

__global__ __launch_bounds__(kBlock) void lut_search_kernel(const float* __restrict__ lut, LutGeom g, const float* __restrict__ q,
                                                            size_t n, float* __restrict__ out) {
    for (size_t i = (size_t)blockIdx.x * kBlock + threadIdx.x; i < n; i += (size_t)gridDim.x * kBlock)
        out[i] = lut_search(lut, g, q[3 * i], q[3 * i + 1], q[3 * i + 2]);
}

constexpr int kNnQ = 4;

__device__ __forceinline__ void load_queries(const float4* __restrict__ pts, int n, const Rt& rt, int apply, float (&qx)[kNnQ],
                                             float (&qy)[kNnQ], float (&qz)[kNnQ], int (&qi)[kNnQ]) {
#pragma unroll
    for (int k = 0; k < kNnQ; ++k) {
        const int i = (blockIdx.x * kNnQ + k) * kBlock + threadIdx.x;
        qi[k] = i;
        const float4 p = pts[i < n ? i : n - 1];
        if (apply) {
            float rx, ry, rz;
            rotate(rt.R, p.x, p.y, p.z, rx, ry, rz);
            qx[k] = rx + rt.t[0];
            qy[k] = ry + rt.t[1];
            qz[k] = rz + rt.t[2];
        } else {
            qx[k] = p.x;
            qy[k] = p.y;
            qz[k] = p.z;
        }
    }
}

__global__ __launch_bounds__(kBlock) void nn_min_kernel(const float4* __restrict__ pts, int n, const float4* __restrict__ tgt, int nt,
                                                        Rt rt, int apply, int slice_len, uint32_t* __restrict__ min_bits) {
    __shared__ float4 tile[kTile];
    float qx[kNnQ], qy[kNnQ], qz[kNnQ], best[kNnQ];
    int qi[kNnQ];
    load_queries(pts, n, rt, apply, qx, qy, qz, qi);
#pragma unroll
    for (int k = 0; k < kNnQ; ++k) best[k] = kInf;
    const int s0 = blockIdx.y * slice_len;
    const int s1 = min(nt, s0 + slice_len);
    for (int t0 = s0; t0 < s1; t0 += kTile) {
        const int cnt = min(kTile, s1 - t0);
        for (int j = threadIdx.x; j < cnt; j += kBlock) tile[j] = tgt[t0 + j];
        __syncthreads();
// ... 944 lines not shown

void launch_fused_trim_select(const FusedTrimRow* rows, int nrows, float* out_ub, float* out_lb, hipStream_t s) {
    if (nrows <= 0) return;
    hipLaunchKernelGGL(fused_trim_select_kernel, dim3(nrows), dim3(kTrimThreads), 0, s, rows, out_ub, out_lb);
}

void launch_fused_finalize(const FusedEval* evals, int nevals, const double2* partials, float* out_lb, float* out_ub, hipStream_t s) {
    if (nevals <= 0) return;
    hipLaunchKernelGGL(fused_bounds_finalize_kernel, dim3(nevals), dim3(64), 0, s, evals, nevals, partials, out_lb, out_ub);
}

void launch_tick_upload(const TickGroup* h_groups, TickGroup* d_groups, int ngroups, const TickSub* h_subs, TickSub* d_subs, int nsubs, hipStream_t s) {
    static_assert(sizeof(TickGroup) % 16 == 0 && sizeof(TickSub) % 16 == 0, "descriptors are copied in 16-byte units");
    const unsigned ng16 = (unsigned)ngroups * (sizeof(TickGroup) / 16), ns16 = (unsigned)nsubs * (sizeof(TickSub) / 16);
    hipLaunchKernelGGL(tick_upload_kernel, dim3(std::min(1024u, (ng16 + ns16 + 63) / 64)), dim3(64), 0, s, reinterpret_cast<const uint4*>(h_groups),
                       reinterpret_cast<uint4*>(d_groups), ng16, reinterpret_cast<const uint4*>(h_subs), reinterpret_cast<uint4*>(d_subs), ns16);
}

void launch_tick_prefill(const TickSub* subs, int nsub, int nchunk, const TickCut& cut, double2* partials, hipStream_t s) {
    const size_t nitems = (size_t)nsub * nchunk;
    if (nitems == 0) return;
    hipLaunchKernelGGL(tick_prefill_kernel, dim3((unsigned)std::min<size_t>((nitems + 63) / 64, 8192)), dim3(64), 0, s, subs, nsub, nchunk, cut, partials);
}

void launch_bounds_finalize(const double2* partials, int nchunk, int total, float* out_lb, float* out_ub, const TickCut& cut, hipStream_t s) {
    hipLaunchKernelGGL(bounds_finalize_kernel, dim3(total), dim3(64), 0, s, partials, nchunk, total, out_lb, out_ub, cut);
}

void launch_lut_build(const float4* tgt_shifted, int nt, const LutGeom& g, float* lut_padded, hipStream_t s) {
    const size_t total = (size_t)g.px * g.py * g.pz;
    const size_t per_block = (size_t)kBlock * kLutNodes;
    const unsigned blocks = (unsigned)((total + per_block - 1) / per_block);
    hipLaunchKernelGGL(lut_build_kernel, dim3(blocks), dim3(kBlock), 0, s, tgt_shifted, nt, g, lut_padded);
}

void launch_lut_quad_apron(const float* lut_padded, const LutGeom& g, float4* qd, hipStream_t s) {
    hipLaunchKernelGGL(lut_quad_apron_kernel, dim3(4096), dim3(kBlock), 0, s, lut_padded, g, qd);
}
void launch_lut_zpair_apron(const float* lut_padded, const LutGeom& g, float2* zp, hipStream_t s) {
    hipLaunchKernelGGL(lut_zpair_apron_kernel, dim3(4096), dim3(kBlock), 0, s, lut_padded, g, zp);
}
void launch_lut_quad(const float* lut_padded, const LutGeom& g, float4* qd, hipStream_t s) {
    hipLaunchKernelGGL(lut_quad_kernel, dim3(8192), dim3(kBlock), 0, s, lut_padded, g, qd);
}

void launch_lut_zpair(const float* lut_padded, const LutGeom& g, float2* zp, hipStream_t s) {
    hipLaunchKernelGGL(lut_zpair_kernel, dim3(8192), dim3(kBlock), 0, s, lut_padded, g, zp);
}

void launch_lut_unpad(const float* lut_padded, const LutGeom& g, float* out, hipStream_t s) {
    hipLaunchKernelGGL(lut_unpad_kernel, dim3(4096), dim3(kBlock), 0, s, lut_padded, g, out);
}

void launch_lut_nodes(const float* lut, const LutGeom& g, const int* xyz, size_t n, float* out, hipStream_t s) {
    const unsigned blocks = (unsigned)((n + kBlock - 1) / kBlock);
    hipLaunchKernelGGL(lut_nodes_kernel, dim3(blocks < 4096 ? (blocks ? blocks : 1) : 4096), dim3(kBlock), 0, s, lut, g, xyz, n, out);
}

void launch_lut_search(const float* lut, const LutGeom& g, const float* q_xyz, size_t n, float* out, hipStream_t s) {
    const unsigned blocks = (unsigned)((n + kBlock - 1) / kBlock);
    hipLaunchKernelGGL(lut_search_kernel, dim3(blocks < 4096 ? (blocks ? blocks : 1) : 4096), dim3(kBlock), 0, s, lut, g, q_xyz, n, out);
}

void launch_fill_u32(uint32_t* p, uint32_t v, size_t n, hipStream_t s) {
    const unsigned blocks = (unsigned)((n + kBlock - 1) / kBlock);
    hipLaunchKernelGGL(fill_u32_kernel, dim3(blocks < 2048 ? (blocks ? blocks : 1) : 2048), dim3(kBlock), 0, s, p, v, n);
}

void launch_nn_min(const float4* pts, int n, const float4* tgt, int nt, const float* R9, const float* t3, int apply,
                   uint32_t* min_bits, hipStream_t s) {
    const int qtiles = (n + kBlock * kNnQ - 1) / (kBlock * kNnQ);
    const int slices = nn_slices(n, nt);
    const int slice_len = ((nt + slices - 1) / slices + kTile - 1) / kTile * kTile;
    const int nsl = (nt + slice_len - 1) / slice_len;
    hipLaunchKernelGGL(nn_min_kernel, dim3(qtiles, nsl), dim3(kBlock), 0, s, pts, n, tgt, nt, make_rt(R9, t3), apply, slice_len, min_bits);
}

void launch_nn_tie_threshold(const uint32_t* min_bits, int n, uint32_t* thr_bits, hipStream_t s) {
    hipLaunchKernelGGL(nn_tie_threshold_kernel, dim3((n + kBlock - 1) / kBlock), dim3(kBlock), 0, s, min_bits, n, thr_bits);
}

void launch_nn_first_index(const float4* pts, int n, const float4* tgt, int nt, const uint32_t* thr_bits, uint32_t* first_idx,
                           hipStream_t s) {
    const int qtiles = (n + kBlock * kNnQ - 1) / (kBlock * kNnQ);
    const int slices = nn_slices(n, nt);
    const int slice_len = ((nt + slices - 1) / slices + kTile - 1) / kTile * kTile;
    const int nsl = (nt + slice_len - 1) / slice_len;
    hipLaunchKernelGGL(nn_first_index_kernel, dim3(qtiles, nsl), dim3(kBlock), 0, s, pts, n, tgt, nt, slice_len, thr_bits, first_idx);
}

void launch_nn_scan(const float4* pts, int n, const BvhView& t, const float* lut, const LutGeom& g, const float* R9, const float* t3, int apply,
                    int want_index, const float4* tgt, int nt, const uint32_t* seed_idx, const float* skip_lb, const uint32_t* skip_u, uint32_t* out, hipStream_t s,
                    float4* writeback, const float* rt_dev, const int* done, double* wsum) {
    const int groups = (n + 63) / 64;
    int nparts = 4;
    while (nparts < 8 && groups * nparts < 4096) nparts <<= 1;
    const int forced = [] { const char* e = dev_env("FGOICP_NN_PARTS"); return e ? std::atoi(e) : 0; }();
    if (forced == 1 || forced == 2 || forced == 4 || forced == 8 || forced == 16) nparts = forced;
    const int dyn_env = [] { const char* e = dev_env("FGOICP_NN_CLAIM"); return e ? std::atoi(e) : -1; }();
    const int dyn = dyn_env >= 0 ? dyn_env : (groups * nparts <= 8192 ? 1 : 0);
    const int flat = [] { const char* e = dev_env("FGOICP_NN_FLAT"); return e ? std::atoi(e) : 0; }();
    if (want_index) hipLaunchKernelGGL(nn_scan_kernel<1>, dim3(groups), dim3(64 * nparts), 0, s, pts, n, t, lut, g, make_rt(R9, t3), apply, tgt, nt, seed_idx, skip_lb, skip_u, out, writeback, rt_dev, done, wsum, dyn, flat);
    else hipLaunchKernelGGL(nn_scan_kernel<0>, dim3(groups), dim3(64 * nparts), 0, s, pts, n, t, lut, g, make_rt(R9, t3), apply, tgt, nt, seed_idx, skip_lb, skip_u, out, writeback, rt_dev, done, wsum, dyn, flat);
}

void launch_nn_scan_dual(const float4* ptsA, const float* RA9, const float* tA3, int applyA, const float4* ptsB, const float* RB9, const float* tB3, int n, const BvhView& t,
// ... 497 lines not shown
```

fast-go-icp_amd/csrc/device/kernels.hpp:

```cpp
#pragma once
#include <hip/hip_runtime.h>

#include <cstddef>
#include <cstdint>

#include "fixed_sum.hpp"

namespace fgoicp {

struct BvhView;

constexpr int kMaxBatch = 32;
constexpr int kBlock = 256;
constexpr float kSqrt3 = 1.732050807568877f;
constexpr float kPi = 3.141592653589793f;
constexpr float kInf = 1E+10f;

struct LutGeom {
    float off_x, off_y, off_z;
    float scale;
    float resolution;
    int dx, dy, dz;
    int px, py, pz;
    int quantize;
    const uint32_t* idx;
};

struct TickGroup {
    float R[9];
    float sin_half;
    int fix_rot;
    int pad_;
};
struct TickSub {
    float tx, ty, tz, span;
    int group;
    int out0;
    int out1;
    int dual;
    float cut0;
    float cut1;
    unsigned term;
    int pad_;
};
constexpr unsigned kSubTerm0 = 1u, kSubTerm1 = 2u;
static_assert(sizeof(TickSub) == 48, "TickSub is copied in 16-byte units");
constexpr int kCutStatSlots = 64;
constexpr float kCutNone = 3.0e38f;
struct TickGate {
    unsigned done;
    unsigned flags;
};
static_assert(sizeof(TickGate) == 8, "TickGate is read and written as one 8-byte word");
constexpr unsigned kGateCutting = 1u;
constexpr unsigned kGateTerm0 = 2u, kGateTerm1 = 4u;
struct TickCut {
    double* acc = nullptr;
    TickGate* gate = nullptr;
    float* row_cut = nullptr;
    unsigned* row_term = nullptr;
    unsigned long long* stat = nullptr;
    const unsigned* tier_split = nullptr;
    int probe = 0;
};
constexpr int kTickNumKeys = 1 << 15;
void launch_tick_sort(const LutGeom& g, const float4* chunk_cen, int nchunk, const TickGroup* groups, const TickSub* subs, int nsub, int cell_shift,
                      unsigned short* keys, unsigned* ranks , unsigned* hist ,
                      unsigned* hist_xcd , unsigned* xoff ,
                      unsigned* block_sums , unsigned* cursor, unsigned* sorted,
                      int allow_xcd , int prefill ,
                      int inject_fault , hipStream_t s,
                      const float* tier_lut = nullptr ,
                      float tier_level = 0.0f ,
                      const TickCut* prefill_cut = nullptr ,
                      double2* partials = nullptr, int row_chunks = 0 , int span = 1 );
constexpr int kTickTierSplit = 1 << 14;
void launch_tick_prefill(const TickSub* subs, int nsub, int nchunk, const TickCut& cut, double2* partials, hipStream_t s);
void launch_tick_upload(const TickGroup* hd_groups, TickGroup* d_groups, int ngroups, const TickSub* hd_subs, TickSub* d_subs, int nsubs, hipStream_t s);
bool launch_bounds_sorted(const float4* src, int ns, const float2* packed, int layout , const LutGeom& g,
                          int nchunk, int chunk_pts , const TickGroup* groups, const TickSub* subs, int nsub, const unsigned* sorted,
                          double2* partials, float* evals_or_null , size_t erow ,
                          int samp_shift ,
                          unsigned* sort_err ,
                          const TickCut& cut ,
                          int span ,
                          hipEvent_t ev_start, hipEvent_t ev_stop, hipStream_t s);
void launch_trim_rows(const float* evals, size_t erow, int n, int k, int rows, const float* row_span, float* out_ub, float* out_lb, hipStream_t s,
                      int samp_shift = 0, int margin = 0, unsigned long long* stat = nullptr);
void launch_trim_select(const float* vals, int n, int k, float* out, uint32_t* sel_info,
                        uint32_t* wide_scratch , hipStream_t s);
void launch_icp_inliers(const float4* work, const float4* tgt, const uint32_t* idx, int n, int nt, int k, float* d2, uint32_t* sel_info,
                        uint32_t* equal_count, const uint32_t* orig_of_slot, unsigned char* use, uint32_t* wide_scratch, hipStream_t s);
void launch_inlier_mask(const float* d2, int n, int k, uint32_t* sel_info, uint32_t* equal_count, const uint32_t* orig_of_slot, unsigned char* use,
                        uint32_t* wide_scratch, hipStream_t s);
void launch_align_scatter(const uint32_t* idx, const uint32_t* min_bits, const unsigned char* use, const uint32_t* orig_of_slot, int n, int nt, uint32_t* corr_out,
                          float* d2_out, unsigned char* inlier_out, unsigned char* target_hit, size_t nt16, uint2* partials, uint32_t* summary3, hipStream_t s);
constexpr int kAlignInfoTerms = 10;
void launch_align_info(const unsigned char* inlier, const float* d2, const uint32_t* corr, const float4* tgt, int n, int nt, float max_d2, MomentRow<kAlignInfoTerms>* rows,
                       unsigned long long* out11, hipStream_t s);
constexpr int kKnnMin = 4, kKnnMax = 32;
void launch_target_knn(const BvhView& t, const float4* tgt, int nt, int k, uint32_t* knn_idx, float* knn_d2, float4* normals, hipStream_t s);
constexpr int kOutlierKnnMin = 2;
void launch_outlier_knn(const BvhView& t, int nt, int k, double* mean_dist, float* kth_dist2, hipStream_t s);
void launch_cluster_count(const BvhView& t, int nt, float eps2, uint32_t min_points, uint32_t* neighbours, uint32_t* core, unsigned long long* core_count, hipStream_t s);
void launch_cluster_round(const BvhView& t, int nt, float eps2, const uint32_t* core, uint32_t* parent, uint32_t* changed, hipStream_t s);
void launch_cluster_border(const BvhView& t, int nt, float eps2, const uint32_t* core, const uint32_t* parent, const uint32_t* rank, int32_t* label, hipStream_t s);
struct RefineInputs {
    const float4* moved;
    const uint32_t* orig_of_slot;
    const unsigned char* inlier;
    const float* d2;
    const uint32_t* corr;
    const float4 *tgt, *normals, *src_normals;
    int n, nt;
    float max_d2;
};
constexpr int kPlaneTerms = 28, kRobustTerms = 29;
// ... 6 lines not shown
    RefineInputs in;
    float R[9];
    int loss;
    double eps, scale;
    void* rows;
    int first_block;
    int nblocks;
};
void launch_fused_refine_moments(bool gicp, bool weighted, const FusedRefineView* views, int n, int total_blocks, unsigned long long* out, hipStream_t s);
void launch_slot_order(const float4* in, const uint32_t* orig_of_slot, int n, float4* out, hipStream_t s);
struct FusedPairView {
    const float4* src;
    const char* lutp;
    LutGeom g;
    int ns;
    int chunk_pts;
};
struct FusedEval {
    float R[9];
    float sin_half;
    float tx, ty, tz, span;
    int fix_rot;
    int pair;
    int nchunk;
    int samp_shift;
    union {
        unsigned long long partial_base;
        unsigned long long row_off;
    };
};
static_assert(sizeof(FusedEval) == 80, "FusedEval: one layout for both kinds of row");
struct FusedTrimRow {
    const float* row;
    int n, k, samp_shift, margin;
    float span;
    int out;
};
bool bounds_lut_wide(const LutGeom& g, int layout);
size_t packed_lut_bytes(const LutGeom& g, int layout);
void launch_fused_bounds(int layout, bool wide, bool quant, const FusedPairView* pairs, const FusedEval* evals, const uint2* items, unsigned nitems, double2* partials,
                         hipStream_t s);
void launch_fused_finalize(const FusedEval* evals, int nevals, const double2* partials, float* out_lb, float* out_ub, hipStream_t s);
void launch_fused_trim_bounds(int layout, bool wide, bool quant, const FusedPairView* pairs, const FusedEval* evals, const uint2* items, unsigned nitems, float* arena,
                              hipStream_t s);
void launch_fused_trim_select(const FusedTrimRow* rows, int nrows, float* out_ub, float* out_lb, hipStream_t s);

void launch_bounds_finalize(const double2* partials, int nchunk, int total, float* out_lb, float* out_ub, const TickCut& cut, hipStream_t s);

void launch_lut_build(const float4* tgt_shifted, int nt, const LutGeom& g, float* lut_padded, hipStream_t s);
void launch_lut_zpair(const float* lut_padded, const LutGeom& g, float2* zp, hipStream_t s);
void launch_lut_quad(const float* lut_padded, const LutGeom& g, float4* qd, hipStream_t s);
void launch_lut_quad_apron(const float* lut_padded, const LutGeom& g, float4* qd , hipStream_t s);
void launch_lut_zpair_apron(const float* lut_padded, const LutGeom& g, float2* zp , hipStream_t s);
void launch_lut_unpad(const float* lut_padded, const LutGeom& g, float* out, hipStream_t s);
void launch_lut_search(const float* lut, const LutGeom& g, const float* q_xyz, size_t n, float* out, hipStream_t s);
void launch_lut_nodes(const float* lut_padded, const LutGeom& g, const int* xyz , size_t n, float* out, hipStream_t s);

void launch_fill_u32(uint32_t* p, uint32_t v, size_t n, hipStream_t s);
void launch_nn_min(const float4* pts, int n, const float4* tgt, int nt, const float* R9, const float* t3, int apply,
                   uint32_t* min_bits, hipStream_t s);
void launch_nn_tie_threshold(const uint32_t* min_bits, int n, uint32_t* thr_bits, hipStream_t s);
void launch_nn_first_index(const float4* pts, int n, const float4* tgt, int nt, const uint32_t* thr_bits, uint32_t* first_idx,
                           hipStream_t s);

void launch_nn_scan(const float4* pts, int n, const BvhView& t, const float* lut, const LutGeom& g, const float* R9, const float* t3, int apply,
                    int want_index, const float4* tgt, int nt, const uint32_t* seed_idx,
                    const float* skip_lb , const uint32_t* skip_u, uint32_t* out, hipStream_t s,
                    float4* writeback = nullptr ,
                    const float* rt_dev = nullptr ,
                    const int* done = nullptr ,
                    double* wsum = nullptr );
void launch_nn_scan_dual(const float4* ptsA, const float* RA9, const float* tA3, int applyA, const float4* ptsB, const float* RB9, const float* tB3, int n, const BvhView& t,
                         const float* lut, const LutGeom& g, const float4* tgt, int nt, const uint32_t* seed_idx, const float* skip_lbA, const uint32_t* skip_uA,
                         const float* skip_lbB, const uint32_t* skip_uB, uint32_t* out_idx, uint32_t* out_min, float4* writeback, double* wsumA, double* wsumB, hipStream_t s);
void launch_nn_prep(const float4* pts, int n, const float* lut, const LutGeom& g, const float* R9, const float* t3, int apply, const float4* tgt, int nt,
                    const uint32_t* seed_idx, const float* box6, float* ub_out, float* lb_out, hipStream_t s);
void launch_lut_build_scan(const BvhView& shifted_targets, const LutGeom& g, float* scratch_padded, float* lut_padded, hipStream_t s, uint32_t* lut_idx_padded = nullptr);

void launch_sum_f32_as_f64(const uint32_t* bits, int n, double* block_partials, int nblocks, hipStream_t s, const int* done = nullptr);
void launch_sum_partials(const double* block_partials, int nblocks, int width, double* out, hipStream_t s);

void launch_transform_inplace(float4* pts, int n, const float* R9, const float* t3, hipStream_t s);
void launch_icp_sums(const float4* work, const float4* tgt, const uint32_t* idx, int n, int nt, const unsigned char* use_or_null,
                     double* block_partials, int nblocks, hipStream_t s, const int* done = nullptr);
void launch_icp_centroids(const double* block_partials, int nblocks, int ns, float* cen_dev, float* cen_host, hipStream_t s);
void launch_icp_cov(const float4* work, const float4* tgt, const uint32_t* idx, int n, int nt, const float* cen_dev, const unsigned char* use_or_null,
                    double* block_partials, int nblocks, hipStream_t s);


void launch_icp_cov_cen(const float4* work, const float4* tgt, const uint32_t* idx, int n, int nt, const double* sums_bp, int sums_nblocks, int from_waves,
                        float* cen_out, double* block_partials, int nblocks, hipStream_t s, const int* done = nullptr);

int reduce_blocks_for(int n);

}
```

fast-go-icp_amd/csrc/host/driver.hpp:

```cpp
#pragma once
#include <algorithm>
#include <atomic>
#include <chrono>
#include <condition_variable>
#include <cstdlib>
#include <array>
#include <functional>
#include <iterator>
#include <map>
#include <thread>
#include <tuple>
#include <cstdint>
#include <cstdio>
#include <cstring>
#include <memory>
#include <mutex>
#include <queue>
#include <vector>

#include "math3.hpp"
#include "knobs.hpp"

namespace fgoicp {

// ... 971 lines not shown
            int hit = -1;
            for (uint32_t sl = (uint32_t)NodeKeyHash()(ki) & 1023u; table[sl] >= 0; sl = (sl + 1) & 1023u)
                if (node_key(lb.batch[(size_t)table[sl]]) == ki) { hit = table[sl]; break; }
            if (hit >= 0) tw.push_back({ub.brow[i], lb.brow[(size_t)hit]});
            else if (memo_on && !lb.memo.find(ki)) {
                tw.push_back({ub.brow[i], lb.nrows + (int)lb.phantom.size()});
                lb.phantom.push_back(ub.batch[i]);
            }
        }
    }
    static void pack_group(Half& h, size_t a, const Task& tk, const RotCube& cube) {
        std::memcpy(&h.R9[9 * a], cube.q.R.m, 9 * sizeof(float));
        h.spans[a] = cube.span;
        h.fix[a] = tk.fix_rot ? 1 : 0;
        h.cut[a] = tk.cut_above();
        float* base = &h.tn4[4 * (size_t)h.offsets[a]];
        for (size_t q = 0; q < tk.batch.size(); ++q) {
            if (tk.brow[q] < 0) continue;
            const TransCube& c = tk.batch[q];
            float* out = base + 4 * (size_t)tk.brow[q];
            out[0] = c.t.x; out[1] = c.t.y; out[2] = c.t.z; out[3] = c.span;
        }
        float* out = base + 4 * (size_t)tk.nrows;
        for (const TransCube& c : tk.phantom) { out[0] = c.t.x; out[1] = c.t.y; out[2] = c.t.z; out[3] = c.span; out += 4; }
    }
    static void rebalance(Half& from, Half& to) {
        if (from.members.size() < to.members.size() + 2 + to.members.size() / 4) return;
        const size_t move = (from.members.size() - to.members.size()) / 2;
        std::vector<size_t> keep;
        keep.reserve(from.members.size());
        size_t moved = 0, unit = 0;
        for (size_t k = from.members.size(); k-- > 0;) {
            const bool pair = k > 0 && (from.members[k] ^ 1) == from.members[k - 1];
            const size_t n = pair ? 2 : 1;
            const bool go = moved + n <= move && (unit & 1) == 0;
            for (size_t q = 0; q < n; ++q) {
                if (go) { to.members.push_back(from.members[k - (n - 1) + q]); ++moved; }
                else keep.push_back(from.members[k - q]);
            }
            if (pair) --k;
            ++unit;
        }
        std::reverse(keep.begin(), keep.end());
        from.members.swap(keep);
    }
    template <class O>
    static auto submit_leaf(O& ops, int slot, Half& h, int) -> decltype(ops.bounds_submit_leaf(slot, 0, h.R9.data(), h.spans.data(), h.fix.data(), h.offsets.data(), h.tn4.data(), h.twin.data(), h.cut.data(), h.leaf.data())) {
        return ops.bounds_submit_leaf(slot, (int)h.live.size(), h.R9.data(), h.spans.data(), h.fix.data(), h.offsets.data(), h.tn4.data(), h.twin.data(), h.cut.data(), h.leaf.data());
    }
    template <class O>
    static int submit_leaf(O& ops, int slot, Half& h, long) {
        return ops.bounds_submit(slot, (int)h.live.size(), h.R9.data(), h.spans.data(), h.fix.data(), h.offsets.data(), h.tn4.data(), h.twin.data(), h.cut.data());
    }
    int submit_half(int slot, Half& h) {
        if (use_cut_) return submit_leaf(ops_, slot, h, 0);
        return ops_.bounds_submit(slot, (int)h.live.size(), h.R9.data(), h.spans.data(), h.fix.data(), h.offsets.data(), h.tn4.data(), h.twin.data(), nullptr);
    }
    void consume_half(Half& h, std::vector<Task*>& tasks, bool par) {
        const std::function<void(size_t)> push_fn = [&](size_t k) {
            Task& tk = *tasks[h.live[k]];
            const float *lb = h.lb.data() + h.offsets[k], *ub = h.ub.data() + h.offsets[k];
            for (size_t q = 0; q < tk.batch.size(); ++q)
                if (tk.brow[q] >= 0) { tk.blb[q] = lb[tk.brow[q]]; tk.bub[q] = ub[tk.brow[q]]; }
            for (size_t j = 0; j < tk.phantom.size(); ++j)
                tk.memo.insert(node_key(tk.phantom[j]), lb[tk.nrows + (int)j], ub[tk.nrows + (int)j]);
            tk.consume(tk.blb.data(), tk.bub.data());
        };
        if (par) pool_->parallel_for(h.live.size(), push_fn);
        else for (size_t k = 0; k < h.live.size(); ++k) push_fn(k);
        if (account_submissions_) stats_.bounds_calls++;
    }

    void overlap_report(std::vector<Task*>& tasks, const std::vector<const RotCube*>& cubes) {
        for (size_t i = 0; i + 1 < tasks.size(); i += 2) {
            if (cubes[i] != cubes[i + 1]) continue;
            auto &a = tasks[i]->seen, &b = tasks[i + 1]->seen;
            std::sort(a.begin(), a.end()); std::sort(b.begin(), b.end());
            std::vector<std::array<uint32_t, 4>> both;
            std::set_intersection(a.begin(), a.end(), b.begin(), b.end(), std::back_inserter(both));
            ov_ub_ += a.size(); ov_lb_ += b.size(); ov_both_ += both.size();
        }
    }
    int run_task_list(std::vector<Task*>& tasks, const std::vector<const RotCube*>& cubes) {
        const int rc_ = run_task_list_impl(tasks, cubes);
        if (overlap_stats_) overlap_report(tasks, cubes);
        if (account_submissions_)
            for (const Task* t : tasks) stats_.trans_cubes += t->count;
        return rc_;
    }
    int run_task_list_impl(std::vector<Task*>& tasks, const std::vector<const RotCube*>& cubes) {
        const bool par = tasks.size() >= 8 && pool_->size() > 1;
        const bool timing = timing_;
        if (tasks.size() >= 4 && ops_.async()) {
            Half h[2];
            for (size_t i = 0; i < tasks.size(); ++i) h[(i >> 1) & 1].members.push_back(i);
            for (;;) {
                bool any = false;
                for (int k = 0; k < 2; ++k) {
                    const auto ta = clock::now();
                    if (h[k].inflight) {
                        int rc = ops_.bounds_collect(k, h[k].lb.data(), h[k].ub.data());
                        if (rc) return rc;
                        h[k].inflight = false;
                    }
                    const auto tb = clock::now();
                    if (!h[k].live.empty()) consume_half(h[k], tasks, par);
                    h[k].live.clear();
                    const auto tc = clock::now();
// ... 73 lines not shown
```

fast-go-icp_amd/csrc/host/solver.cpp:

```cpp
#include <cstddef>
#include <cstdlib>
#include <cmath>
#include <cstring>
#include <memory>
#include <string>
#include <vector>

#include "../../../include/fgoicp_amd.h"
#include "../device/ctx.hpp"
#include "driver.hpp"
#include "segment.hpp"

namespace fgoicp {

struct HipOps {
    fgoicp_ctx* ctx = nullptr;
    int bounds_multi(int G, const float* R9, const float* rot_span, const int* fix_rot, const int* offsets, const float* tn4, float* lb,
                     float* ub, const float* cut_above) {
        return ctx_bounds_multi(ctx, G, R9, rot_span, fix_rot, offsets, tn4, lb, ub, cut_above);
    }
    int bounds_submit(int slot, int G, const float* R9, const float* rot_span, const int* fix_rot, const int* offsets, const float* tn4,
                      const int* twin, const float* cut_above) {
        return ctx_bounds_submit(ctx, slot, G, R9, rot_span, fix_rot, offsets, tn4, twin, cut_above);
    }
    int bounds_submit_leaf(int slot, int G, const float* R9, const float* rot_span, const int* fix_rot, const int* offsets, const float* tn4,
                           const int* twin, const float* cut_above, const float* ub_below_span) {
        return ctx_bounds_submit(ctx, slot, G, R9, rot_span, fix_rot, offsets, tn4, twin, cut_above, ub_below_span);
    }
    int bounds_collect(int slot, float* lb, float* ub) { return ctx_bounds_collect(ctx, slot, lb, ub); }
    bool async() const { return pipeline; }
    bool twins() const { return true; }
    int icp(const float* R0, const float* t0, size_t max_iter, float thr, float* sse, float* R9, float* t3, int* iters) {
        return ctx_icp(ctx, R0, t0, max_iter, thr, sse, R9, t3, iters);
    }
    int icp_coop(int rank, int world, int (*gather)(void*, size_t, void*), void* user, const float* R0, const float* t0, size_t max_iter, float thr, float* sse,
                 float* R9, float* t3, int* iters) {
        return ctx_icp_coop(ctx, rank, world, gather, user, R0, t0, max_iter, thr, sse, R9, t3, iters);
    }
    int icp_background(const float* R0, const float* t0, size_t max_iter, float thr, float* sse, float* R9, float* t3, int* iters) {
        return ctx_icp_lane(ctx, 1, R0, t0, max_iter, thr, sse, R9, t3, iters);
    }
    bool pipeline = [] { const char* e = dev_env("FGOICP_PIPELINE"); return e ? std::atoi(e) != 0 : true; }();
};

void information_from_moments(uint64_t n, const double* sq_s, const double* sqq_s, const float* offset3, float scale, double* info36, double* sum_q3_out,
                                     double* sum_qq6_out) {
    const double N = (double)n, s = (double)scale;
    const double c[3] = {offset3 ? (double)offset3[0] : 0.0, offset3 ? (double)offset3[1] : 0.0, offset3 ? (double)offset3[2] : 0.0};
    double q[3], qq[6];
    static const int A[6] = {0, 0, 0, 1, 1, 2}, B[6] = {0, 1, 2, 1, 2, 2};
    if (!offset3 && scale == 1.0f) {
        for (int k = 0; k < 3; ++k) q[k] = sq_s[k];
        for (int k = 0; k < 6; ++k) qq[k] = sqq_s[k];
    } else {
        for (int k = 0; k < 3; ++k) q[k] = sq_s[k] / s + N * c[k];
        for (int k = 0; k < 6; ++k) {
            const int a = A[k], b = B[k];
            qq[k] = sqq_s[k] / (s * s) + (c[a] * sq_s[b] + sq_s[a] * c[b]) / s + N * c[a] * c[b];
        }
    }
    if (sum_q3_out) std::memcpy(sum_q3_out, q, sizeof(q));
    if (sum_qq6_out) std::memcpy(sum_qq6_out, qq, sizeof(qq));
    if (!info36) return;
    const double xx = qq[0], xy = qq[1], xz = qq[2], yy = qq[3], yz = qq[4], zz = qq[5];
    const double M[6][6] = {{yy + zz, -xy, -xz, 0.0, -q[2], q[1]},
                            {-xy, xx + zz, -yz, q[2], 0.0, -q[0]},
                            {-xz, -yz, xx + yy, -q[1], q[0], 0.0},
                            {0.0, q[2], -q[1], N, 0.0, 0.0},
                            {-q[2], 0.0, q[0], 0.0, N, 0.0},
                            {q[1], -q[0], 0.0, 0.0, 0.0, N}};
    for (int r = 0; r < 6; ++r)
        for (int k = 0; k < 6; ++k) info36[6 * r + k] = M[r][k] + 0.0;
}

}

using namespace fgoicp;

struct fgoicp_solver {
    std::vector<Vec3f> pcs, pct;
// ... 359 lines not shown
```

fast-go-icp_amd/registration.py:

```python
import ctypes as C

import numpy as np

from . import _lib
from .nodes import RotNode, from_glm, pack_tnodes, to_glm


def _fp(a):
    return a.ctypes.data_as(_lib.c_float_p)


def _cloud(pc):
    a = np.ascontiguousarray(pc, dtype=np.float32)
    if a.ndim != 2 or a.shape[1] != 3:
        raise ValueError("point cloud must be (n, 3)")
    return a


class StreamPool:

    def __init__(self, size=32):
        self.size = size


# ... 403 lines not shown
    return np.triu(M) + np.triu(M, 1).T, v


class Registration:

    def __init__(self, pct, pcs, target_bounds, lut_resolution, device=0, flags=0):
        self._lib = _lib.load()
        self.pct = _cloud(pct)
        self.pcs = _cloud(pcs)
        self.nt, self.ns = len(self.pct), len(self.pcs)
        b = np.asarray(target_bounds, dtype=np.float32).reshape(6)
        self._h = C.c_void_p()
        _lib.check(self._lib.fgoicp_ctx_create(_fp(self.pct), self.nt, _fp(self.pcs), self.ns, _fp(b), float(lut_resolution),
                                               int(device), int(flags), C.byref(self._h)), "fgoicp_ctx_create")

    @classmethod
    def _borrow(cls, handle, owner):
        self = cls.__new__(cls)
        self._lib = _lib.load()
        self._h = C.c_void_p(handle)
        self._owner = owner
        self.ns = self._lib.fgoicp_ctx_ns(self._h)
        self.nt = self._lib.fgoicp_ctx_nt(self._h)
        return self

    def close(self):
        if getattr(self, "_h", None) and not hasattr(self, "_owner"):
            self._lib.fgoicp_ctx_destroy(self._h)
        self._h = None

    def __del__(self):
        try:
            self.close()
        except Exception:
            pass

    def lut_dims(self):
        d = (C.c_int * 3)()
        _lib.check(self._lib.fgoicp_lut_dims(self._h, d), "fgoicp_lut_dims")
        return tuple(d)

    def set_coop_split(self, min_points_untrimmed=None, min_points_trimmed=None):
        never = (1 << 64) - 1
        _lib.check(self._lib.fgoicp_ctx_set_coop_split(self._h, never if min_points_untrimmed is None else int(min_points_untrimmed),
                                                       never if min_points_trimmed is None else int(min_points_trimmed)), "fgoicp_ctx_set_coop_split")

    def info(self):
        i = _lib.CtxInfo()
        i.struct_size = C.sizeof(_lib.CtxInfo)
        _lib.check(self._lib.fgoicp_ctx_get_info(self._h, C.byref(i)), "fgoicp_ctx_get_info")
        return dict(lut_dims=tuple(i.lut_dims), lut_layout=i.lut_layout, lut_nodes=i.lut_nodes, lut_bytes=i.lut_bytes,
                    source_points_per_face_voxel=i.source_points_per_face_voxel, points_per_item=i.points_per_item,
                    items_per_evaluation=i.items_per_evaluation, max_subcubes_per_window=i.max_subcubes_per_window,
                    source_order=i.source_order, tree_order=i.tree_order, chunks_per_item_with_thresholds=i.chunks_per_item_with_thresholds)

    def lut_read(self):
        dx, dy, dz = self.lut_dims()
        out = np.empty(dx * dy * dz, dtype=np.float32)
        _lib.check(self._lib.fgoicp_lut_read(self._h, _fp(out), out.size), "fgoicp_lut_read")
        return out.reshape(dz, dy, dx)

    def lut_nodes(self, xyz):
        q = np.ascontiguousarray(xyz, dtype=np.int32).reshape(-1, 3)
        out = np.empty(len(q), dtype=np.float32)
        _lib.check(self._lib.fgoicp_lut_nodes(self._h, q.ctypes.data_as(_lib.c_int_p), len(q), _fp(out)), "fgoicp_lut_nodes")
        return out

    def lut_search(self, queries):
        q = _cloud(queries)
        out = np.empty(len(q), dtype=np.float32)
        _lib.check(self._lib.fgoicp_lut_search(self._h, _fp(q), len(q), _fp(out)), "fgoicp_lut_search")
        return out

    def compute_sse_error(self, *args):
        if isinstance(args[0], RotNode):
            rnode, tnodes, fix_rot = args[0], args[1], args[2]
            return self.compute_bounds(rnode.q.R, rnode.span, tnodes, fix_rot)
        R, t = args
        Rg = to_glm(R)
        tt = np.ascontiguousarray(t, dtype=np.float32).reshape(3)
        out = C.c_float()
        _lib.check(self._lib.fgoicp_sse(self._h, _fp(Rg), _fp(tt), C.byref(out)), "fgoicp_sse")
        return np.float32(out.value)

    def alignment(self, R, t):
        Rg = to_glm(R)
        tt = np.ascontiguousarray(t, dtype=np.float32).reshape(3)
        return _alignment(lambda *a: self._lib.fgoicp_alignment(self._h, _fp(Rg), _fp(tt), *a), "fgoicp_alignment", self.ns, self.nt)

    def information(self, R, t, max_dist2=np.inf):
        Rg = to_glm(R)
        tt = np.ascontiguousarray(t, dtype=np.float32).reshape(3)
        return _information(lambda out: self._lib.fgoicp_information(self._h, _fp(Rg), _fp(tt), float(max_dist2), out), "fgoicp_information")

    def set_target_normals(self, normals=None, k=16):
        if normals is None:
            _lib.check(self._lib.fgoicp_ctx_set_target_normals(self._h, None, int(k)), "fgoicp_ctx_set_target_normals")
            return
        n = _cloud(normals)
        if len(n) != self.nt:
            raise ValueError("normals must be (nt, 3)")
        _lib.check(self._lib.fgoicp_ctx_set_target_normals(self._h, _fp(n), int(k)), "fgoicp_ctx_set_target_normals")

    def target_normals(self):
        out = np.empty((self.nt, 3), np.float32)
        _lib.check(self._lib.fgoicp_target_normals(self._h, _fp(out)), "fgoicp_target_normals")
        return out
# ... 57 lines not shown
            return
        n = _cloud(normals)
        if len(n) != self.ns:
            raise ValueError("normals must be (ns, 3)")
        _lib.check(self._lib.fgoicp_ctx_set_source_normals(self._h, _fp(n), int(k)), "fgoicp_ctx_set_source_normals")

    def source_normals(self):
        out = np.empty((self.ns, 3), np.float32)
        _lib.check(self._lib.fgoicp_source_normals(self._h, _fp(out)), "fgoicp_source_normals")
        return out

    def gicp_moments(self, R, t, max_dist2=np.inf, epsilon=1e-3):
        Rg = to_glm(R)
        tt = np.ascontiguousarray(t, dtype=np.float32).reshape(3)
        raw = _lib.PlaneMoments()
        _lib.check(self._lib.fgoicp_gicp_moments(self._h, _fp(Rg), _fp(tt), float(max_dist2), float(epsilon), C.byref(raw)), "fgoicp_gicp_moments")
        return PlaneMomentsResult(raw)

    def icp_gicp(self, R, t, max_iter=30, conv_thr=1e-6, max_dist2=np.inf, epsilon=1e-3, loss=None, loss_scale=None):
        if loss is not None:
            return self._icp_robust(_lib.MODEL_GICP, R, t, max_iter, conv_thr, max_dist2, epsilon, loss, loss_scale)
        Rg = to_glm(R)
        tt = np.ascontiguousarray(t, dtype=np.float32).reshape(3)
        raw = _lib.PlaneResult()
        _lib.check(self._lib.fgoicp_icp_gicp(self._h, _fp(Rg), _fp(tt), int(max_iter), float(conv_thr), float(max_dist2), float(epsilon), C.byref(raw)), "fgoicp_icp_gicp")
        return GicpRefinement(raw)

    def compute_bounds(self, R, rot_span, tnodes, fix_rot):
        Rg = to_glm(R)
        tn = pack_tnodes(tnodes)
        B = len(tn)
        lb = np.empty(B, dtype=np.float32)
        ub = np.empty(B, dtype=np.float32)
        _lib.check(self._lib.fgoicp_bounds_batch(self._h, _fp(Rg), float(rot_span), _fp(tn), B, int(bool(fix_rot)), _fp(lb), _fp(ub)),
                   "fgoicp_bounds_batch")
        return lb, ub

    def compute_bounds_multi(self, Rs, rot_spans, fix_rots, tnode_groups):
        G = len(Rs)
        Rg = np.concatenate([to_glm(R) for R in Rs]).astype(np.float32) if G else np.zeros(0, np.float32)
        spans = np.asarray(rot_spans, dtype=np.float32)
        fr = np.asarray([int(bool(f)) for f in fix_rots], dtype=np.int32)
        packed = [pack_tnodes(t) for t in tnode_groups]
        offs = np.zeros(G + 1, dtype=np.int32)
        offs[1:] = np.cumsum([len(p) for p in packed])
        tn = np.concatenate(packed) if G else np.zeros((0, 4), np.float32)
        lb = np.empty(len(tn), dtype=np.float32)
        ub = np.empty(len(tn), dtype=np.float32)
        _lib.check(self._lib.fgoicp_bounds_multi(self._h, G, _fp(Rg), _fp(spans), fr.ctypes.data_as(_lib.c_int_p),
                                                 offs.ctypes.data_as(_lib.c_int_p), _fp(np.ascontiguousarray(tn)), _fp(lb), _fp(ub)),
                   "fgoicp_bounds_multi")
        return [(lb[offs[g]:offs[g + 1]], ub[offs[g]:offs[g + 1]]) for g in range(G)]

    def compute_bounds_cut(self, Rs, rot_spans, fix_rots, tnode_groups, cut_above, twin=None, slot=0, ub_below_span=None):
        G = len(Rs)
        Rg = np.concatenate([to_glm(R) for R in Rs]).astype(np.float32) if G else np.zeros(0, np.float32)
        spans = np.asarray(rot_spans, dtype=np.float32)
        fr = np.asarray([int(bool(f)) for f in fix_rots], dtype=np.int32)
        packed = [pack_tnodes(t) for t in tnode_groups]
        offs = np.zeros(G + 1, dtype=np.int32)
        offs[1:] = np.cumsum([len(p) for p in packed])
        tn = np.ascontiguousarray(np.concatenate(packed) if G else np.zeros((0, 4), np.float32))
        cut = None if cut_above is None else np.ascontiguousarray(cut_above, dtype=np.float32)
        assert cut is None or len(cut) == G
        tw = None if twin is None else np.ascontiguousarray(twin, dtype=np.int32)
        lb = np.empty(len(tn), dtype=np.float32)
        ub = np.empty(len(tn), dtype=np.float32)
        args = (self._h, int(slot), G, _fp(Rg), _fp(spans), fr.ctypes.data_as(_lib.c_int_p), offs.ctypes.data_as(_lib.c_int_p),
                _fp(tn), None if tw is None else tw.ctypes.data_as(_lib.c_int_p), None if cut is None else _fp(cut))
        if ub_below_span is None:
            _lib.check(self._lib.fgoicp_bounds_submit_cut(*args), "fgoicp_bounds_submit_cut")
        else:
            leaf = np.ascontiguousarray(ub_below_span, dtype=np.float32)
            assert len(leaf) == G
            _lib.check(self._lib.fgoicp_bounds_submit_leaf(*args, _fp(leaf)), "fgoicp_bounds_submit_leaf")
        _lib.check(self._lib.fgoicp_bounds_collect(self._h, int(slot), _fp(lb), _fp(ub)), "fgoicp_bounds_collect")
        return [(lb[offs[g]:offs[g + 1]], ub[offs[g]:offs[g + 1]]) for g in range(G)]

    def cut_stats(self, reset=False):
        a = C.c_uint64(); b = C.c_uint64()
        _lib.check(self._lib.fgoicp_ctx_cut_stats(self._h, C.byref(a), C.byref(b), int(reset)), "fgoicp_ctx_cut_stats")
        return a.value, b.value

    def procrustes(self, working):
        w = _cloud(working)
        assert len(w) == self.ns
        R = np.empty(9, np.float32); t = np.empty(3, np.float32); cen = np.empty(6, np.float32); ABt = np.empty(9, np.float32)
        idx = np.empty(self.ns, np.int32)
        _lib.check(self._lib.fgoicp_procrustes(self._h, _fp(w), _fp(R), _fp(t), _fp(cen), _fp(ABt), idx.ctypes.data_as(_lib.c_int_p)),
                   "fgoicp_procrustes")
        return from_glm(R), t, cen, ABt, idx

    def set_inliers(self, k):
        _lib.check(self._lib.fgoicp_ctx_set_inliers(self._h, int(k)), "fgoicp_ctx_set_inliers")

    def point_distances(self, R, rot_span, tnode, fix_rot):
        tn = pack_tnodes(np.asarray(tnode, np.float32).reshape(1, 4))
        out = np.empty(self.ns, dtype=np.float32)
        _lib.check(self._lib.fgoicp_bounds_point_distances(self._h, _fp(to_glm(R)), float(rot_span), _fp(tn), int(bool(fix_rot)), _fp(out)),
                   "fgoicp_bounds_point_distances")
        return out

    def test_sort_fault(self, nth_tick):
        _lib.check(self._lib.fgoicp_ctx_test_sort_fault(self._h, int(nth_tick)), "fgoicp_ctx_test_sort_fault")

    def sort_fallbacks(self):
        a = C.c_uint64(); b = C.c_uint64()
        _lib.check(self._lib.fgoicp_ctx_sort_fallbacks(self._h, C.byref(a), C.byref(b)), "fgoicp_ctx_sort_fallbacks")
        return a.value, b.value

    def trim_stats(self, reset=False):
        out = (C.c_uint64 * 3)()
        _lib.check(self._lib.fgoicp_ctx_trim_stats(self._h, out, int(reset)), "fgoicp_ctx_trim_stats")
        return int(out[0]), int(out[1]), int(out[2])

    def set_profile(self, enabled):
        _lib.check(self._lib.fgoicp_ctx_set_profile(self._h, int(bool(enabled))), "fgoicp_ctx_set_profile")

    def profile(self, reset=False):
        ms = C.c_double(); launches = C.c_uint64(); sub = C.c_uint64(); ev = C.c_uint64(); sel = C.c_double()
        _lib.check(self._lib.fgoicp_ctx_profile_evaluations(self._h, C.byref(ev)), "fgoicp_ctx_profile_evaluations")
        _lib.check(self._lib.fgoicp_ctx_profile_select_ms(self._h, C.byref(sel)), "fgoicp_ctx_profile_select_ms")
        _lib.check(self._lib.fgoicp_ctx_profile(self._h, C.byref(ms), C.byref(launches), C.byref(sub), int(reset)), "fgoicp_ctx_profile")
        return {"kernel_ms": ms.value, "launches": launches.value, "subcubes": sub.value, "evaluations": ev.value, "select_ms": sel.value}


def icp_batch(reg, Rs, ts, max_iter=100, convergence_threshold=0.005):
    n = len(Rs)
    R0 = np.concatenate([to_glm(R) for R in Rs]).astype(np.float32) if n else np.zeros(0, np.float32)
    t0 = np.ascontiguousarray(np.asarray(ts, np.float32).reshape(-1))
    sse = np.empty(n, np.float32); Ro = np.empty(9 * n, np.float32); to = np.empty(3 * n, np.float32); it = np.empty(n, np.int32)
    _lib.check(reg._lib.fgoicp_icp_batch(reg._h, n, _fp(R0), _fp(t0), int(max_iter), float(convergence_threshold), _fp(sse), _fp(Ro), _fp(to),
                                         it.ctypes.data_as(_lib.c_int_p)), "fgoicp_icp_batch")
    return sse, np.stack([from_glm(Ro[9 * i:9 * i + 9]) for i in range(n)]) if n else np.zeros((0, 3, 3), np.float32), to.reshape(n, 3), it

# ... 20 lines not shown
```

include/fgoicp_amd.h:

```cpp
#ifndef FGOICP_AMD_H
#define FGOICP_AMD_H

#include <stddef.h>
#include <stdint.h>

#ifdef __cplusplus
extern "C" {
#endif

typedef enum fgoicp_status {
    FGOICP_OK = 0,
    FGOICP_ERR_INVALID_ARG = 1,
    FGOICP_ERR_NO_DEVICE = 2,
    FGOICP_ERR_HIP = 3,
    FGOICP_ERR_OOM = 4,
    FGOICP_ERR_TOO_LARGE = 5,
    FGOICP_ERR_EXCHANGE = 6
} fgoicp_status;

const char* fgoicp_last_error(void);
const char* fgoicp_version(void);
int fgoicp_dev_knobs(void);
#define FGOICP_ABI_VERSION 2
int fgoicp_abi_version(void);

typedef struct fgoicp_ctx fgoicp_ctx;

enum {
    FGOICP_FLAG_NO_WEIGHT_QUANT = 1u << 0,
    FGOICP_FLAG_NO_MORTON       = 1u << 1,
    FGOICP_FLAG_PROFILE         = 1u << 2,
    FGOICP_FLAG_BRUTE_FORCE_NN  = 1u << 3,
    FGOICP_FLAG_CURVE_ORDER     = 1u << 4
};

int fgoicp_ctx_create(const float* tgt_xyz, size_t nt, const float* src_xyz, size_t ns, const float* bounds6,
                      float lut_resolution, int device, unsigned flags, fgoicp_ctx** out);
void fgoicp_ctx_destroy(fgoicp_ctx* ctx);

int fgoicp_lut_dims(const fgoicp_ctx* ctx, int* dims3);
int fgoicp_lut_read(fgoicp_ctx* ctx, float* out, size_t capacity_floats);
typedef struct fgoicp_ctx_info {
    size_t struct_size;
    int lut_dims[3];
    int lut_layout;
    uint64_t lut_nodes;
    uint64_t lut_bytes;
    double source_points_per_face_voxel;
    int points_per_item;
    int items_per_evaluation;
    int max_subcubes_per_window;
    int source_order;
    int tree_order;
    int chunks_per_item_with_thresholds;
} fgoicp_ctx_info;
int fgoicp_ctx_get_info(const fgoicp_ctx* ctx, fgoicp_ctx_info* out);
int fgoicp_lut_nodes(fgoicp_ctx* ctx, const int* xyz, size_t n, float* out);
int fgoicp_lut_search(fgoicp_ctx* ctx, const float* q_xyz, size_t n, float* out);

int fgoicp_bounds_batch(fgoicp_ctx* ctx, const float* R9, float rot_span, const float* tnodes4, int B, int fix_rot,
                        float* lb_out, float* ub_out);
int fgoicp_bounds_multi(fgoicp_ctx* ctx, int G, const float* R9, const float* rot_span, const int* fix_rot,
                        const int* offsets, const float* tnodes4, float* lb_out, float* ub_out);

int fgoicp_bounds_submit(fgoicp_ctx* ctx, int slot, int G, const float* R9, const float* rot_span, const int* fix_rot,
                         const int* offsets, const float* tnodes4);
int fgoicp_bounds_submit_twins(fgoicp_ctx* ctx, int slot, int G, const float* R9, const float* rot_span, const int* fix_rot,
                               const int* offsets, const float* tnodes4, const int* twin);
int fgoicp_bounds_submit_cut(fgoicp_ctx* ctx, int slot, int G, const float* R9, const float* rot_span, const int* fix_rot,
                             const int* offsets, const float* tnodes4, const int* twin, const float* cut_above);
int fgoicp_bounds_submit_leaf(fgoicp_ctx* ctx, int slot, int G, const float* R9, const float* rot_span, const int* fix_rot,
                              const int* offsets, const float* tnodes4, const int* twin, const float* cut_above, const float* ub_below_span);
int fgoicp_bounds_collect(fgoicp_ctx* ctx, int slot, float* lb_out, float* ub_out);
int fgoicp_ctx_cut_stats(fgoicp_ctx* ctx, uint64_t* items_offered, uint64_t* items_cut, int reset);

int fgoicp_sse(fgoicp_ctx* ctx, const float* R9, const float* t3, float* sse_out);

typedef struct fgoicp_alignment_summary {
    uint32_t struct_size;
    uint64_t points, inliers;
    uint64_t targets_hit;
    float sse;
    float max_inlier_dist2;
    float scaling_factor;
} fgoicp_alignment_summary;
int fgoicp_alignment(fgoicp_ctx* ctx, const float* R9, const float* t3, uint32_t* corr_idx_ns, float* dist2_ns, uint8_t* inlier_ns,
                     uint8_t* target_hit_nt, fgoicp_alignment_summary* out);

typedef struct fgoicp_information_t {
    uint32_t struct_size;
    uint64_t points, correspondences;
    double   sum_dist2;
    double   sum_q[3], sum_qq[6];
    double   info[36];
    float    max_dist2, scaling_factor;
} fgoicp_information_t;
int fgoicp_information(fgoicp_ctx* ctx, const float* R9, const float* t3, float max_dist2, fgoicp_information_t* out);
int fgoicp_information_from_moments(uint64_t n, const double* sum_q3, const double* sum_qq6, const float* offset3, float scale, double* info36,
                                    double* sum_q3_out, double* sum_qq6_out);

typedef struct fgoicp_plane_moments_t {
    uint32_t struct_size;
    uint64_t points, correspondences;
    double   m[28];
    float    max_dist2;
} fgoicp_plane_moments_t;
typedef struct fgoicp_plane_result_t {
    uint32_t struct_size;
    float    R[9], t[3];
    int      iterations;
    int      rank;
    uint64_t correspondences;
    double   plane_rmse;
    float    sse;
    float    scaling_factor;
} fgoicp_plane_result_t;
int fgoicp_ctx_set_target_normals(fgoicp_ctx* ctx, const float* normals_nt3_or_NULL, int k);
int fgoicp_target_normals(fgoicp_ctx* ctx, float* out_nt3);
int fgoicp_target_knn(fgoicp_ctx* ctx, int k, uint32_t* idx_ntk, float* d2_ntk);
int fgoicp_plane_moments(fgoicp_ctx* ctx, const float* R9, const float* t3, float max_dist2, fgoicp_plane_moments_t* out);
int fgoicp_plane_step_from_moments(uint64_t n, const double* m28, double* xi6, int* rank);
int fgoicp_plane_apply_step(const float* R9, const float* t3, const double* xi6, float* R_out9, float* t_out3);
int fgoicp_icp_plane(fgoicp_ctx* ctx, const float* R0_9, const float* t0_3, size_t max_iter, float conv_thr, float max_dist2, fgoicp_plane_result_t* out);

int fgoicp_ctx_set_source_normals(fgoicp_ctx* ctx, const float* normals_ns3_or_NULL, int k);
int fgoicp_source_normals(fgoicp_ctx* ctx, float* out_ns3);
// ... 311 lines not shown
```

Measured before the change: 12.11 million subcubes/s.

## Skip LUT fetches via coarse max-distance grid once upper bound cut is decided

Adds a coarse per-block max-distance LUT and a gated lower-bound-only pass. Once accumulated upper-bound sums show an item's upper bound already exceeds the cut threshold, later chunks compute only lower bounds, and points whose coarse conservative distance proves a zero lower-bound contribution skip the fine LUT gathers. The aim is to cut memory traffic and arithmetic in the bounds kernel for cut items. In exchange it adds an extra atomic accumulator for the upper-bound sums, extra gate states, a coarse-table build, and partial results marked as upper-bound decided that the host must handle.

```diff
diff --git a/fast-go-icp_amd/_lib.py b/fast-go-icp_amd/_lib.py
--- a/fast-go-icp_amd/_lib.py
+++ b/fast-go-icp_amd/_lib.py
@@ -13,7 +13,7 @@
 class CtxInfo(C.Structure):
     _fields_ = [("struct_size", C.c_size_t), ("lut_dims", C.c_int * 3), ("lut_layout", C.c_int), ("lut_nodes", C.c_uint64), ("lut_bytes", C.c_uint64),
                 ("source_points_per_face_voxel", C.c_double), ("points_per_item", C.c_int), ("items_per_evaluation", C.c_int),
-                ("max_subcubes_per_window", C.c_int), ("source_order", C.c_int), ("tree_order", C.c_int), ("chunks_per_item_with_thresholds", C.c_int)]
+                ("max_subcubes_per_window", C.c_int), ("source_order", C.c_int), ("tree_order", C.c_int), ("chunks_per_item_with_thresholds", C.c_int), ("coarse_block", C.c_int)]
 
 
 class CloudStats(C.Structure):
@@ -250,6 +250,10 @@
     "fgoicp_bounds_submit_twins": (C.c_int, [C.c_void_p, C.c_int, C.c_int, c_float_p, c_float_p, c_int_p, c_int_p, c_float_p, c_int_p]),
     "fgoicp_bounds_submit_cut": (C.c_int, [C.c_void_p, C.c_int, C.c_int, c_float_p, c_float_p, c_int_p, c_int_p, c_float_p, c_int_p, c_float_p]),
     "fgoicp_bounds_submit_leaf": (C.c_int, [C.c_void_p, C.c_int, C.c_int, c_float_p, c_float_p, c_int_p, c_int_p, c_float_p, c_int_p, c_float_p, c_float_p]),
+    "fgoicp_bounds_submit_free_ub": (C.c_int, [C.c_void_p, C.c_int, C.c_int, c_float_p, c_float_p, c_int_p, c_int_p, c_float_p, c_int_p, c_float_p, c_float_p]),
+    "fgoicp_lut_coarse_read": (C.c_int, [C.c_void_p, c_int_p, c_float_p, C.c_size_t]),
+    "fgoicp_lut_coarse_search": (C.c_int, [C.c_void_p, c_float_p, C.c_size_t, c_float_p]),
+    "fgoicp_ctx_free_ub_stats": (C.c_int, [C.c_void_p, C.POINTER(C.c_uint64), C.c_int]),
     "fgoicp_ctx_cut_stats": (C.c_int, [C.c_void_p, C.POINTER(C.c_uint64), C.POINTER(C.c_uint64), C.c_int]),
     "fgoicp_solver_set_early_exit": (C.c_int, [C.c_void_p, C.c_int]),
     "fgoicp_bounds_collect": (C.c_int, [C.c_void_p, C.c_int, c_float_p, c_float_p]),
diff --git a/fast-go-icp_amd/csrc/device/bounds_item.hpp b/fast-go-icp_amd/csrc/device/bounds_item.hpp
--- a/fast-go-icp_amd/csrc/device/bounds_item.hpp
+++ b/fast-go-icp_amd/csrc/device/bounds_item.hpp
@@ -179,6 +179,120 @@
     }
 }
 
+__device__ __forceinline__ float item_coarse(const CoarseLut& cl, const ItemTex& t) {
+    const int bx = ((int)t.fl_xy.x + 1) >> kCoarseShift, by = ((int)t.fl_xy.y + 1) >> kCoarseShift, bz = ((int)t.fl_z + 1) >> kCoarseShift;
+    return cl.max[(bz * cl.ny + by) * cl.nx + bx];
+}
+template <int LAYOUT, bool WIDE, bool QUANT, int MODE, bool FULL>
+__device__ __forceinline__ void item_pass_lb(const float4* __restrict__ src, int ns, const char* __restrict__ lutp, const ItemGeom& G, const CoarseLut& cl, const float (&R)[9],
+                                             f2v t_xy, float t_z, float sin_half, float trans_radius, int first, int odd, double (&acc)[4], bool verify, unsigned (&tally)[3]) {
+    constexpr int P = 4;
+    float4 p[P];
+    ItemTex tx[P];
+    bool zero[P];
+#pragma unroll
+    for (int k = 0; k < P; ++k) {
+        const int i = first + 64 * k;
+        p[k] = src[FULL ? i : (i < ns ? i : ns - 1)];
+        tx[k] = item_tex<QUANT>(G, R, t_xy, t_z, p[k]);
+        const float c1 = sqrtf(item_coarse(cl, tx[k]) * (1.0f + kCoarseMargin));
+        const float c0 = c1 - 2.0f * p[k].w * sin_half;
+        const bool z1 = c1 - trans_radius <= 0.0f, z0 = c0 - trans_radius <= 0.0f;
+        zero[k] = MODE == 0 ? z1 : MODE == 1 ? z0 : (z1 && z0);
+#ifdef FGOICP_DEV_KNOBS
+        tally[0] += (FULL || i < ns) ? 1u : 0u;
+        tally[1] += (FULL || i < ns) && zero[k] ? 1u : 0u;
+#endif
+    }
+    f4v ga[P], gb[P];
+    if (LAYOUT == 1) {
+        const char* row1 = lutp + (size_t)G.px * sizeof(float2);
+#pragma unroll
+        for (int k = 0; k < P; ++k) {
+            const size_t idx = item_index<WIDE>(G, tx[k]);
+            ga[k] = gb[k] = f4v{0.0f, 0.0f, 0.0f, 0.0f};
+            if (!(zero[k] && !verify) && (FULL || first + 64 * k < ns)) {
+                ga[k] = *reinterpret_cast<const float4u*>(item_address<WIDE, 3>(lutp, idx));
+                gb[k] = *reinterpret_cast<const float4u*>(item_address<WIDE, 3>(row1, idx));
+            }
+        }
+    } else {
+        constexpr int kStep = LAYOUT == 6 ? 4 : 1;
+        QuadPairLoads qp[P];
+#pragma unroll
+        for (int k = 0; k < P; ++k) {
+            const int own = LAYOUT == 6   ? (int)zpair_apron_index(item_packed_index(tx[k]), G.nbx3, G.nby3)
+                            : LAYOUT == 5 ? (int)apron_index(item_packed_index(tx[k]), G.nbx3, G.nby2)
+                                          : (int)item_index<WIDE>(G, tx[k]);
+            const int other = swap_lane_pair(own);
+            const int o_even = odd ? other : own, o_odd = odd ? own : other;
+            const int need_own = (zero[k] && !verify) || !(FULL || first + 64 * k < ns) ? 0 : 1;
+            const int need_other = swap_lane_pair(need_own);
+            const int need_even = odd ? need_other : need_own, need_odd = odd ? need_own : need_other;
+            qp[k].r1 = qp[k].r2 = float4a{0.0f, 0.0f, 0.0f, 0.0f};
+            if (LAYOUT == 6) {
+                if (need_even) {
+                    const f4v r1 = *reinterpret_cast<const float4u*>(item_address<WIDE, 3>(lutp, (size_t)(unsigned)(o_even + kStep * odd)));
+                    qp[k].r1 = float4a{r1.x, r1.y, r1.z, r1.w};
+                }
+                if (need_odd) {
+                    const f4v r2 = *reinterpret_cast<const float4u*>(item_address<WIDE, 3>(lutp, (size_t)(unsigned)(o_odd + kStep * odd)));
+                    qp[k].r2 = float4a{r2.x, r2.y, r2.z, r2.w};
+                }
+            } else {
+                if (need_even) qp[k].r1 = *reinterpret_cast<const float4a*>(item_address<WIDE, 4>(lutp, (size_t)(unsigned)(o_even + kStep * odd)));
+                if (need_odd) qp[k].r2 = *reinterpret_cast<const float4a*>(item_address<WIDE, 4>(lutp, (size_t)(unsigned)(o_odd + kStep * odd)));
+            }
+        }
+#pragma unroll
+        for (int k = 0; k < P; ++k) {
+            const float4a send = odd ? qp[k].r1 : qp[k].r2;
+            float4a recv;
+            recv.x = swap_lane_pair(send.x); recv.y = swap_lane_pair(send.y); recv.z = swap_lane_pair(send.z); recv.w = swap_lane_pair(send.w);
+            const float4a a = odd ? recv : qp[k].r1, b = odd ? qp[k].r2 : recv;
+            ga[k] = f4v{a.x, a.y, a.z, a.w};
+            gb[k] = f4v{b.x, b.y, b.z, b.w};
+        }
+    }
+#pragma unroll
+    for (int k = 0; k < P; ++k) {
+        float dsq;
+        if (LAYOUT == 1 || LAYOUT == 6) dsq = item_blend(tx[k], f2v{ga[k].x, ga[k].y}, f2v{ga[k].z, ga[k].w}, f2v{gb[k].x, gb[k].y}, f2v{gb[k].z, gb[k].w});
+        else dsq = item_blend(tx[k], f2v{ga[k].x, ga[k].y}, f2v{gb[k].x, gb[k].y}, f2v{ga[k].z, ga[k].w}, f2v{gb[k].z, gb[k].w});
+        const float d1 = sqrtf(dsq);
+        const float d0 = d1 - 2.0f * p[k].w * sin_half;
+        const bool exists = FULL || first + 64 * k < ns;
+        if (MODE != 1) {
+            const float l = fmaxf(d1 - trans_radius, 0.0f);
+            const float lbv = l * l;
+#ifdef FGOICP_DEV_KNOBS
+            tally[2] += exists && zero[k] && lbv != 0.0f ? 1u : 0u;
+#endif
+            acc[1] += exists && !zero[k] ? (double)lbv : 0.0;
+        }
+        if (MODE != 0) {
+            const float l = fmaxf(d0 - trans_radius, 0.0f);
+            const float lbv = l * l;
+#ifdef FGOICP_DEV_KNOBS
+            tally[2] += exists && zero[k] && lbv != 0.0f ? 1u : 0u;
+#endif
+            acc[MODE == 2 ? 3 : 1] += exists && !zero[k] ? (double)lbv : 0.0;
+        }
+    }
+}
+
+template <int LAYOUT, bool WIDE, bool QUANT, int MODE>
+__device__ __forceinline__ void item_walk_lb(const float4* __restrict__ src, int ns, const char* __restrict__ lutp, const ItemGeom& G, const CoarseLut& cl, const float (&R)[9],
+                                             f2v t_xy, float t_z, float sin_half, float trans_radius, int base, int chunk_pts, int lane, double (&acc)[4], bool verify,
+                                             unsigned (&tally)[3]) {
+    const int odd = lane & 1;
+    for (int pass = 0; pass < chunk_pts; pass += 256) {
+        const int first = base + pass + lane;
+        if (base + pass + 256 <= ns) item_pass_lb<LAYOUT, WIDE, QUANT, MODE, true>(src, ns, lutp, G, cl, R, t_xy, t_z, sin_half, trans_radius, first, odd, acc, verify, tally);
+        else item_pass_lb<LAYOUT, WIDE, QUANT, MODE, false>(src, ns, lutp, G, cl, R, t_xy, t_z, sin_half, trans_radius, first, odd, acc, verify, tally);
+    }
+}
+
 template <int LAYOUT, int TRIM, bool WIDE, bool QUANT, int MODE>
 __device__ __forceinline__ void item_walk(const float4* __restrict__ src, int ns, const char* __restrict__ lutp, const ItemGeom& G, const float (&R)[9], f2v t_xy, float t_z,
                                           float sin_half, float trans_radius, int base, int chunk_pts, int lane, double (&acc)[4], float* __restrict__ row0,
@@ -216,22 +330,36 @@
     const int nsub = SPAN ? min(span, nchunk - chunk0) : 1;
     const int lane = (int)threadIdx.x;
     const TickSub sb = subs[s];
-    bool cutting = false, term0 = false, term1 = false;
+    bool cutting = false, term0 = false, term1 = false, free_ub = false, lb_only = false;
     if (!TRIM && cut.acc) {
         TickGate* const gate = cut.gate + s;
         const unsigned long long gw = __hip_atomic_load(reinterpret_cast<unsigned long long*>(gate), __ATOMIC_RELAXED, __HIP_MEMORY_SCOPE_WORKGROUP);
-        if (__builtin_amdgcn_readfirstlane((int)(unsigned)gw) && !(cut.probe & 4)) return;
+        const unsigned done = (unsigned)__builtin_amdgcn_readfirstlane((int)(unsigned)gw);
+        if (done >= kGateDone && !(cut.probe & 4)) return;
         const unsigned flags = (unsigned)__builtin_amdgcn_readfirstlane((int)(unsigned)(gw >> 32));
         cutting = (flags & kGateCutting) != 0u;
         term0 = (flags & kGateTerm0) != 0u;
         term1 = (flags & kGateTerm1) != 0u;
+        free_ub = cutting && (flags & kGateFreeUb) != 0u && cut.acc_ub != nullptr;
+        lb_only = free_ub && (done == kGateUbDecided || (cut.probe & 8));
         if (cutting && !(cut.probe & 1)) {
+            const bool want_ub = free_ub && !lb_only;
             const double a0 = __hip_atomic_load(&cut.acc[2 * (size_t)s], __ATOMIC_RELAXED, __HIP_MEMORY_SCOPE_AGENT);
             const double a1 = sb.dual ? __hip_atomic_load(&cut.acc[2 * (size_t)s + 1], __ATOMIC_RELAXED, __HIP_MEMORY_SCOPE_AGENT) : 0.0;
+            double u0 = 0.0, u1 = 0.0;
+            if (want_ub) {
+                u0 = __hip_atomic_load(&cut.acc_ub[2 * (size_t)s], __ATOMIC_RELAXED, __HIP_MEMORY_SCOPE_AGENT);
+                if (sb.dual) u1 = __hip_atomic_load(&cut.acc_ub[2 * (size_t)s + 1], __ATOMIC_RELAXED, __HIP_MEMORY_SCOPE_AGENT);
+            }
             const bool reached = a0 >= (double)sb.cut0 * kCutMargin && (!sb.dual || a1 >= (double)sb.cut1 * kCutMargin);
             if (__builtin_amdgcn_readfirstlane((int)reached)) {
-                if (lane == 0) __hip_atomic_store(&gate->done, 1u, __ATOMIC_RELAXED, __HIP_MEMORY_SCOPE_AGENT);
+                if (lane == 0) __hip_atomic_store(&gate->done, kGateDone, __ATOMIC_RELAXED, __HIP_MEMORY_SCOPE_AGENT);
                 return;
+            }
+            const bool decided = want_ub && u0 >= (double)sb.cut0 * kCutMargin && (!sb.dual || u1 >= (double)sb.cut1 * kCutMargin);
+            if (__builtin_amdgcn_readfirstlane((int)decided)) {
+                if (lane == 0) (void)__hip_atomic_fetch_max(&gate->done, kGateUbDecided, __ATOMIC_RELAXED, __HIP_MEMORY_SCOPE_AGENT);
+                lb_only = true;
             }
         }
     }
@@ -245,19 +373,42 @@
     float* row0 = TRIM ? evals + (size_t)sb.out0 * erow : nullptr;
     float* row1 = TRIM ? evals + (size_t)sb.out1 * erow : nullptr;
     double lb_fix = 0.0, lb_rot = 0.0;
+    double ub_fix = 0.0, ub_rot = 0.0;
+    unsigned tally[3] = {0u, 0u, 0u};
     for (int sub = 0; sub < (SPAN ? nsub : 1); ++sub) {
         const int chunk = chunk0 + sub;
         const int base = chunk * chunk_pts;
         double acc[4] = {0.0, 0.0, 0.0, 0.0};
+        if (!TRIM && lb_only) {
+            const bool verify = (cut.probe & 16) != 0;
+            if (sb.dual) item_walk_lb<LAYOUT, WIDE, QUANT, 2>(src, ns, lutp, G, cut.coarse, R, t_xy, sb.tz, gr.sin_half, trans_radius, base, chunk_pts, lane, acc, verify, tally);
+            else if (gr.fix_rot) item_walk_lb<LAYOUT, WIDE, QUANT, 0>(src, ns, lutp, G, cut.coarse, R, t_xy, sb.tz, gr.sin_half, trans_radius, base, chunk_pts, lane, acc, verify, tally);
+            else item_walk_lb<LAYOUT, WIDE, QUANT, 1>(src, ns, lutp, G, cut.coarse, R, t_xy, sb.tz, gr.sin_half, trans_radius, base, chunk_pts, lane, acc, verify, tally);
+            const double r1 = wave_sum(acc[1]);
+            lb_fix += r1;
+            if (sb.dual) {
+                const double r3 = wave_sum(acc[3]);
+                lb_rot += r3;
+                if (lane == 0) {
+                    partials[(size_t)sb.out0 * nchunk + chunk] = make_double2(kUbDecidedMarker, r1);
+                    partials[(size_t)sb.out1 * nchunk + chunk] = make_double2(kUbDecidedMarker - 1.0, r3);
+                }
+            } else if (lane == 0) {
+                partials[(size_t)sb.out0 * nchunk + chunk] = make_double2(kUbDecidedMarker, r1);
+            }
+            continue;
+        }
         if (sb.dual) item_walk<LAYOUT, TRIM, WIDE, QUANT, 2>(src, ns, lutp, G, R, t_xy, sb.tz, gr.sin_half, trans_radius, base, chunk_pts, lane, acc, row0, row1, samp_shift);
         else if (gr.fix_rot) item_walk<LAYOUT, TRIM, WIDE, QUANT, 0>(src, ns, lutp, G, R, t_xy, sb.tz, gr.sin_half, trans_radius, base, chunk_pts, lane, acc, row0, row1, samp_shift);
         else item_walk<LAYOUT, TRIM, WIDE, QUANT, 1>(src, ns, lutp, G, R, t_xy, sb.tz, gr.sin_half, trans_radius, base, chunk_pts, lane, acc, row0, row1, samp_shift);
         if (TRIM) continue;
         const double r0 = wave_sum(acc[0]), r1 = wave_sum(acc[1]);
         lb_fix += term0 ? r0 : r1;
+        ub_fix += r0;
         if (sb.dual) {
             const double r2 = wave_sum(acc[2]), r3 = wave_sum(acc[3]);
             lb_rot += term1 ? r2 : r3;
+            ub_rot += r2;
             if (lane == 0) {
                 partials[(size_t)sb.out0 * nchunk + chunk] = make_double2(r0, r1);
                 partials[(size_t)sb.out1 * nchunk + chunk] = make_double2(r2, r3);
@@ -269,5 +420,18 @@
     if (!TRIM && cutting && lane == 0 && !(cut.probe & 2)) {
         unsafeAtomicAdd(&cut.acc[2 * (size_t)s], lb_fix);
         if (sb.dual) unsafeAtomicAdd(&cut.acc[2 * (size_t)s + 1], lb_rot);
-    }
-}
+        if (free_ub && !lb_only) {
+            unsafeAtomicAdd(&cut.acc_ub[2 * (size_t)s], ub_fix);
+            if (sb.dual) unsafeAtomicAdd(&cut.acc_ub[2 * (size_t)s + 1], ub_rot);
+        }
+    }
+#ifdef FGOICP_DEV_KNOBS
+    if (!TRIM && lb_only && cut.free_stat) {
+        for (int k = 0; k < 3; ++k) {
+            unsigned v = tally[k];
+            for (int off = 32; off > 0; off >>= 1) v += __shfl_down(v, off);
+            if (lane == 0 && v) atomicAdd(&cut.free_stat[(1 + k) * kCutStatSlots + (blockIdx.x & (kCutStatSlots - 1))], (unsigned long long)v);
+        }
+    }
+#endif
+}
diff --git a/fast-go-icp_amd/csrc/device/ctx.hip b/fast-go-icp_amd/csrc/device/ctx.hip
--- a/fast-go-icp_amd/csrc/device/ctx.hip
+++ b/fast-go-icp_amd/csrc/device/ctx.hip
@@ -95,9 +95,15 @@
     const TickSub* dev_subs = small ? sl.h_subs.dev() : sl.d_subs;
     TickCut cut;
     if (sl.win_cut) { cut.acc = sl.d_cut_acc; cut.gate = sl.d_cut_gate; cut.row_cut = sl.d_row_cut; cut.row_term = sl.d_row_term; cut.stat = c->d_cut_stat; }
+    if (sl.win_cut && sl.win_free_ub) {
+        cut.acc_ub = sl.d_cut_acc_ub;
+        cut.coarse.max = c->d_lut_coarse; cut.coarse.nx = c->coarse_dims[0]; cut.coarse.ny = c->coarse_dims[1];
+        cut.free_stat = c->d_free_stat;
+    }
     if (tiers && !small) cut.tier_split = sl.d_cursor + kTickTierSplit;
     static const int cut_probe = [] { const char* e = dev_env("FGOICP_CUT_PROBE"); return e ? std::atoi(e) : 0; }();
     cut.probe = cut_probe;
+    if (sl.win_free_ub) cut.probe |= dev_int("FGOICP_FREE_UB_PROBE", 0) & (8 | 16);
     *sl.h_sort_err = 0u;
     unsigned* fused_err = !small && c->sort_check ? sl.h_sort_err.dev() : nullptr;
     if (!small) {
@@ -155,7 +161,7 @@
 }
 
 static int tick_enqueue_window(fgoicp_ctx* c, fgoicp_ctx::TickSlot& sl, int G, const float* R9, const float* rot_span, const int* fix_rot,
-                               const int* offsets, const float* tn4, const int* twin, const float* cut_above, const float* ub_below_span, int pos, int* end_out) {
+                               const int* offsets, const float* tn4, const int* twin, const float* cut_above, const float* ub_below_span, bool free_ub, int pos, int* end_out) {
     const double t0 = g_tt.on ? now_s() : 0;
     int g = 0;
     while (g < G && offsets[g + 1] <= pos) ++g;
@@ -181,6 +187,9 @@
     if (rows <= 0) return FGOICP_OK;
     static const bool leaf_rule = [] { const char* e = dev_env("FGOICP_CUT_LEAF"); return !e || std::atoi(e) != 0; }();
     const auto terminal = [&](int sub_group, float span) { return leaf_rule && cut_above && ub_below_span && span < ub_below_span[sub_group]; };
+    static const bool free_rule = [] { const char* e = dev_env("FGOICP_CUT_FREE_UB"); return !e || std::atoi(e) != 0; }();
+    const bool free_on = free_ub && free_rule && cut_above && !c->inliers && c->d_lut_coarse;
+    bool any_free = false;
     int neval = 0;
     for (int r = 0; r < rows; ++r) {
         const int i = pos + r;
@@ -205,6 +214,7 @@
                 ts.cut1 = a.fix_rot ? cb : ca;
                 const unsigned ta = terminal(a.pad_, ts.span) ? 1u : 0u, tb = terminal(b.pad_, ts.span) ? 1u : 0u;
                 ts.term = a.fix_rot ? (ta * kSubTerm0 | tb * kSubTerm1) : (tb * kSubTerm0 | ta * kSubTerm1);
+                if (free_on) { ts.term |= kSubFreeUb; any_free = true; }
                 ts.pad_ = 0;
                 continue;
             }
@@ -217,9 +227,11 @@
         ts.dual = 0;
         ts.cut0 = ts.cut1 = cut_above ? cut_above[sl.h_groups[gi].pad_] : kNoCut;
         ts.term = terminal(sl.h_groups[gi].pad_, ts.span) ? kSubTerm0 : 0u;
+        if (free_on) { ts.term |= kSubFreeUb; any_free = true; }
         ts.pad_ = 0;
     }
     sl.win_cut = cut_above != nullptr && !c->inliers;
+    sl.win_free_ub = any_free;
     for (int k = 0; k < ng; ++k) sl.h_groups[k].pad_ = 0;
     const double t1 = g_tt.on ? now_s() : 0;
     sl.win_pos = pos;
@@ -263,8 +275,9 @@
                 const float T = v ? ts.cut1 : ts.cut0;
                 const bool term = (ts.term & (v ? kSubTerm1 : kSubTerm0)) != 0u;
                 const bool above = (term ? sl.h_ub[r] : sl.h_lb[r]) >= T;
+                const float want_ub = (ts.term & kSubFreeUb) && !term && sl.h_ub[r] >= T ? T : sl.h_ub[r];
                 const bool ok = above ? (lb[(size_t)r] == T && ub[(size_t)r] == T)
-                                      : (std::memcmp(&lb[(size_t)r], &sl.h_lb[r], 4) == 0 && std::memcmp(&ub[(size_t)r], &sl.h_ub[r], 4) == 0);
+                                      : (std::memcmp(&lb[(size_t)r], &sl.h_lb[r], 4) == 0 && std::memcmp(&ub[(size_t)r], &want_ub, 4) == 0);
                 c->cut_verify_rows++;
                 c->cut_verify_above += above ? 1 : 0;
                 if (!ok) {
@@ -287,7 +300,7 @@
 }
 
 int ctx_bounds_submit(fgoicp_ctx* c, int slot, int G, const float* R9, const float* rot_span, const int* fix_rot, const int* offsets,
-                      const float* tn4, const int* twin, const float* cut_above, const float* ub_below_span) {
+                      const float* tn4, const int* twin, const float* cut_above, const float* ub_below_span, bool free_ub) {
     HIPCHK(hipSetDevice(c->device));
     fgoicp_ctx::TickSlot& sl = c->slots[slot];
     if (sl.inflight) { set_error("fgoicp_bounds_submit: slot still in flight (collect it first)"); return FGOICP_ERR_INVALID_ARG; }
@@ -298,7 +311,7 @@
     int pos = 0;
     while (pos < sl.total) {
         int end = pos;
-        int rc = tick_enqueue_window(c, sl, G, R9, rot_span, fix_rot, offsets, tn4, twin, cut_above, ub_below_span, pos, &end);
+        int rc = tick_enqueue_window(c, sl, G, R9, rot_span, fix_rot, offsets, tn4, twin, cut_above, ub_below_span, free_ub, pos, &end);
         if (rc) return rc;
         if (end <= pos) break;
         pos = end;
@@ -324,6 +337,21 @@
     if (items_offered) *items_offered = c->cut_items_offered;
     if (items_cut) *items_cut = (uint64_t)now - c->cut_stat_base;
     if (reset) { c->cut_items_offered = 0; c->cut_stat_base = (uint64_t)now; }
+    return FGOICP_OK;
+}
+
+int ctx_free_ub_stats(fgoicp_ctx* c, uint64_t* out4, int reset) {
+    HIPCHK(hipSetDevice(c->device));
+    unsigned long long part[kFreeStatSlots] = {}, now[4] = {0, 0, 0, 0};
+    if (c->d_free_stat) {
+        HIPCHK(hipDeviceSynchronize());
+        HIPCHK(hipMemcpy(part, c->d_free_stat, sizeof(part), hipMemcpyDeviceToHost));
+        for (int k = 0; k < kFreeStatSlots; ++k) now[k / kCutStatSlots] += part[k];
+    }
+    for (int k = 0; k < 4; ++k) {
+        if (out4) out4[k] = (uint64_t)now[k] - c->free_stat_base[k];
+        if (reset) c->free_stat_base[k] = (uint64_t)now[k];
+    }
     return FGOICP_OK;
 }
 
@@ -1457,6 +1485,9 @@
         HIPCHK(c->d_lut_zp.alloc(total));
         launch_lut_zpair(c->d_lut, g, c->d_lut_zp, c->stream);
     }
+    c->coarse_dims[0] = coarse_blocks(g.px); c->coarse_dims[1] = coarse_blocks(g.py); c->coarse_dims[2] = coarse_blocks(g.pz);
+    HIPCHK(c->d_lut_coarse.alloc((size_t)c->coarse_dims[0] * c->coarse_dims[1] * c->coarse_dims[2]));
+    launch_lut_coarse_max(c->d_lut, g, c->d_lut_coarse, c->stream);
     HIPCHK(hipGetLastError());
     HIPCHK(hipStreamSynchronize(c->stream));
     return FGOICP_OK;
@@ -1547,6 +1578,9 @@
     HIPCHK(sl.d_partials.alloc(max_items));
     HIPCHK(sl.d_cut_acc.alloc(2 * subcubes));
     HIPCHK(hipMemset(sl.d_cut_acc, 0, sizeof(double) * 2 * subcubes));
+    HIPCHK(sl.d_cut_acc_ub.alloc(2 * subcubes));
+    HIPCHK(hipMemset(sl.d_cut_acc_ub, 0, sizeof(double) * 2 * subcubes));
+    if (!c->d_free_stat) { HIPCHK(c->d_free_stat.alloc(kFreeStatSlots)); HIPCHK(hipMemset(c->d_free_stat, 0, sizeof(unsigned long long) * kFreeStatSlots)); }
     static_assert(sizeof(float) == sizeof(unsigned), "d_row_term is the second half of d_row_cut's allocation");
     HIPCHK(sl.d_row_cut.alloc(2 * subcubes));
     sl.d_row_term = reinterpret_cast<unsigned*>(sl.d_row_cut + subcubes);
@@ -1736,6 +1770,7 @@
     out->source_order = c->source_order;
     out->tree_order = c->tree_order;
     out->chunks_per_item_with_thresholds = c->cut_span;
+    out->coarse_block = c->d_lut_coarse ? kCoarseB : 0;
     full.struct_size = caller < sizeof(full) ? caller : sizeof(full);
     std::memcpy(user_out, &full, full.struct_size);
     return FGOICP_OK;
@@ -1789,6 +1824,41 @@
     for (int g = 0; g < G; ++g)
         if (offsets[g + 1] < offsets[g] || offsets[0] != 0) { set_error("fgoicp_bounds_submit: offsets must start at 0 and be non-decreasing"); return FGOICP_ERR_INVALID_ARG; }
     return ctx_bounds_submit(c, slot, G, R9, rot_span, fix_rot, offsets, tn4, twin, cut_above, ub_below_span);
+}
+
+int fgoicp_bounds_submit_free_ub(fgoicp_ctx* c, int slot, int G, const float* R9, const float* rot_span, const int* fix_rot, const int* offsets,
+                                 const float* tn4, const int* twin, const float* cut_above, const float* ub_below_span) {
+    if (!c || slot < 0 || slot > 1 || G < 0 || (G > 0 && (!R9 || !rot_span || !fix_rot || !offsets || !tn4))) return FGOICP_ERR_INVALID_ARG;
+    static const int zero[1] = {0};
+    if (G == 0) offsets = zero;
+    for (int g = 0; g < G; ++g)
+        if (offsets[g + 1] < offsets[g] || offsets[0] != 0) { set_error("fgoicp_bounds_submit: offsets must start at 0 and be non-decreasing"); return FGOICP_ERR_INVALID_ARG; }
+    return ctx_bounds_submit(c, slot, G, R9, rot_span, fix_rot, offsets, tn4, twin, cut_above, ub_below_span, true);
+}
+
+int fgoicp_lut_coarse_read(fgoicp_ctx* c, int* dims3, float* out, size_t capacity) {
+    if (!c) return FGOICP_ERR_INVALID_ARG;
+    if (!c->d_lut_coarse) { set_error("fgoicp_lut_coarse_read: the context has no coarse table"); return FGOICP_ERR_INVALID_ARG; }
+    const size_t total = (size_t)c->coarse_dims[0] * c->coarse_dims[1] * c->coarse_dims[2];
+    if (dims3) for (int k = 0; k < 3; ++k) dims3[k] = c->coarse_dims[k];
+    if (!out) return FGOICP_OK;
+    if (capacity < total) { set_error("fgoicp_lut_coarse_read: buffer too small"); return FGOICP_ERR_INVALID_ARG; }
+    HIPCHK(hipSetDevice(c->device));
+    HIPCHK(hipMemcpyAsync(out, c->d_lut_coarse, total * sizeof(float), hipMemcpyDeviceToHost, c->stream));
+    HIPCHK(hipStreamSynchronize(c->stream));
+    return FGOICP_OK;
+}
+int fgoicp_lut_coarse_search(fgoicp_ctx* c, const float* q, size_t n, float* out) {
+    if (c && !c->d_lut_coarse) { set_error("fgoicp_lut_coarse_search: the context has no coarse table"); return FGOICP_ERR_INVALID_ARG; }
+    return lut_query(c, q, n, out, [&](const float* dq, float* dout) {
+        CoarseLut cl;
+        cl.max = c->d_lut_coarse; cl.nx = c->coarse_dims[0]; cl.ny = c->coarse_dims[1];
+        launch_lut_coarse_search(cl, c->geom, dq, n, dout, c->stream);
+    });
+}
+int fgoicp_ctx_free_ub_stats(fgoicp_ctx* c, uint64_t* out4, int reset) {
+    if (!c) return FGOICP_ERR_INVALID_ARG;
+    return ctx_free_ub_stats(c, out4, reset);
 }
 
 int fgoicp_ctx_cut_stats(fgoicp_ctx* c, uint64_t* items_offered, uint64_t* items_cut, int reset) {
diff --git a/fast-go-icp_amd/csrc/device/ctx.hpp b/fast-go-icp_amd/csrc/device/ctx.hpp
--- a/fast-go-icp_amd/csrc/device/ctx.hpp
+++ b/fast-go-icp_amd/csrc/device/ctx.hpp
@@ -34,6 +34,8 @@
     int source_order = 0, tree_order = 0;
     fgoicp::Dev<uint32_t> d_lut_idx;
     fgoicp::Dev<float2> d_lut_zp;
+    fgoicp::Dev<float> d_lut_coarse;
+    int coarse_dims[3] = {0, 0, 0};
     fgoicp::LutGeom geom{};
     fgoicp::BvhOwned bvh_tgt;
     bool brute_force_nn = false;
@@ -55,10 +57,12 @@
         fgoicp::Dev<unsigned> d_hist_xcd, d_xoff;
         fgoicp::Dev<double2> d_partials;
         fgoicp::Dev<double> d_cut_acc;
+        fgoicp::Dev<double> d_cut_acc_ub;
         fgoicp::Dev<float> d_row_cut;
         unsigned* d_row_term = nullptr;
         fgoicp::Dev<fgoicp::TickGate> d_cut_gate;
         bool win_cut = false;
+        bool win_free_ub = false;
         fgoicp::Mapped<float> h_lb, h_ub;
         fgoicp::Dev<float> d_evals;
         fgoicp::Mapped<float> h_row_span;
@@ -70,6 +74,8 @@
         bool inflight = false;
     };
     fgoicp::Dev<unsigned long long> d_cut_stat;
+    fgoicp::Dev<unsigned long long> d_free_stat;
+    uint64_t free_stat_base[4] = {0, 0, 0, 0};
     uint64_t cut_items_offered = 0;
     uint64_t cut_verify_windows = 0, cut_verify_rows = 0, cut_verify_above = 0, cut_verify_bad = 0;
     uint64_t cut_stat_base = 0;
@@ -172,7 +178,9 @@
                      const float* tn4, float* lb_out, float* ub_out, const float* cut_above = nullptr);
 int ctx_cut_stats(fgoicp_ctx* c, uint64_t* items_offered, uint64_t* items_cut, int reset);
 int ctx_bounds_submit(fgoicp_ctx* c, int slot, int G, const float* R9, const float* rot_span, const int* fix_rot, const int* offsets, const float* tn4,
-                      const int* twin = nullptr, const float* cut_above = nullptr, const float* ub_below_span = nullptr);
+                      const int* twin = nullptr, const float* cut_above = nullptr, const float* ub_below_span = nullptr,
+                      bool free_ub = false );
+int ctx_free_ub_stats(fgoicp_ctx* c, uint64_t* out4, int reset);
 int ctx_bounds_collect(fgoicp_ctx* c, int slot, float* lb_out, float* ub_out);
 int ctx_set_inliers(fgoicp_ctx* c, size_t k);
 inline unsigned trim_ctx_flags(unsigned flags, float f) { return flags | (f > 0.0f ? (unsigned)FGOICP_FLAG_CURVE_ORDER : 0u); }
diff --git a/fast-go-icp_amd/csrc/device/kernels.hip b/fast-go-icp_amd/csrc/device/kernels.hip
--- a/fast-go-icp_amd/csrc/device/kernels.hip
+++ b/fast-go-icp_amd/csrc/device/kernels.hip
@@ -211,13 +211,16 @@
 
 constexpr int kTickXcds = 16;
 
+constexpr unsigned kRowTerminal = 1u, kRowFreeUb = 2u;
 __device__ __forceinline__ void cut_prefill(const TickSub& sb, int s, int chunk_first, int chunk_end, int row_chunks, const TickCut& cut, double2* __restrict__ partials) {
     const bool cutting = sb.cut0 < kCutNone && (!sb.dual || sb.cut1 < kCutNone);
     if (chunk_first == 0) {
-        *reinterpret_cast<uint2*>(cut.gate + s) = make_uint2(0u, (cutting ? kGateCutting : 0u) | sb.term << 1);
+        const bool free_eval = cutting && sb.term == kSubFreeUb;
+        *reinterpret_cast<uint2*>(cut.gate + s) = make_uint2(0u, (cutting ? kGateCutting : 0u) | (sb.term & (kSubTerm0 | kSubTerm1)) << 1 | (free_eval ? kGateFreeUb : 0u));
         cut.row_cut[sb.out0] = sb.cut0;
-        cut.row_term[sb.out0] = sb.term & kSubTerm0;
-        if (sb.dual) { cut.row_cut[sb.out1] = sb.cut1; cut.row_term[sb.out1] = sb.term & kSubTerm1; }
+        const unsigned free_ub = sb.term & kSubFreeUb ? kRowFreeUb : 0u;
+        cut.row_term[sb.out0] = sb.term & kSubTerm0 ? kRowTerminal : free_ub;
+        if (sb.dual) { cut.row_cut[sb.out1] = sb.cut1; cut.row_term[sb.out1] = sb.term & kSubTerm1 ? kRowTerminal : free_ub; }
     }
     if (!cutting) return;
     for (int chunk = chunk_first; chunk < chunk_end; ++chunk) {
@@ -825,27 +828,39 @@
     const double2* row = partials + (size_t)s * nchunk;
     double u = 0.0, l = 0.0;
     unsigned skipped = 0;
+    unsigned lb_only = 0;
+    unsigned decided = 0;
     for (int c = threadIdx.x; c < nchunk; c += 64) {
         const double2 v = row[c];
-        skipped += v.x < 0.0 ? 1u : 0u;
+        skipped += v.x == -1.0 ? 1u : 0u;
+        lb_only += v.x == kUbDecidedMarker ? 1u : 0u;
+        decided += v.x <= kUbDecidedMarker ? 1u : 0u;
         u += v.x;
         l += v.y;
     }
     u = wave_sum(u);
     l = wave_sum(l);
+    for (int off = 32; off > 0; off >>= 1) decided += __shfl_down(decided, off);
     if (cut.stat) {
         for (int off = 32; off > 0; off >>= 1) skipped += __shfl_down(skipped, off);
         if (threadIdx.x == 0 && skipped) atomicAdd(&cut.stat[s & (kCutStatSlots - 1)], (unsigned long long)skipped);
+    }
+    if (cut.free_stat) {
+        for (int off = 32; off > 0; off >>= 1) lb_only += __shfl_down(lb_only, off);
+        if (threadIdx.x == 0 && lb_only) atomicAdd(&cut.free_stat[s & (kCutStatSlots - 1)], (unsigned long long)lb_only);
     }
     if (threadIdx.x == 0) {
         float ubf = (float)u, lbf = (float)l;
         if (cut.row_cut) {
             const float T = cut.row_cut[s];
-            if (lbf >= T || (cut.row_term[s] && ubf >= T)) lbf = ubf = T;
+            const unsigned rule = cut.row_term[s];
+            if (lbf >= T || (rule == kRowTerminal && ubf >= T)) lbf = ubf = T;
+            else if (rule == kRowFreeUb && (decided || ubf >= T)) ubf = T;
         }
         out_ub[s] = ubf;
         out_lb[s] = lbf;
     }
+    if (cut.acc_ub && threadIdx.x >= 2 && threadIdx.x < 4) cut.acc_ub[2 * (size_t)s + threadIdx.x - 2] = 0.0;
     if (cut.acc && threadIdx.x < 2) cut.acc[2 * (size_t)s + threadIdx.x] = 0.0;
 }
 
@@ -899,6 +914,31 @@
         const int y = (int)(r % g.dy);
         const int z = (int)(r / g.dy);
         out[n] = lut[((size_t)(z + 1) * g.py + (y + 1)) * g.px + (x + 1)];
+    }
+}
+
+__global__ __launch_bounds__(kBlock) void lut_coarse_max_kernel(const float* __restrict__ lut, LutGeom g, int nx, int ny, int nz, float* __restrict__ out) {
+    const size_t total = (size_t)nx * ny * nz;
+    for (size_t n = (size_t)blockIdx.x * kBlock + threadIdx.x; n < total; n += (size_t)gridDim.x * kBlock) {
+        const int bx = (int)(n % nx);
+        const size_t r = n / nx;
+        const int by = (int)(r % ny), bz = (int)(r / ny);
+        const int x1 = min(bx * kCoarseB + kCoarseB, g.px - 1), y1 = min(by * kCoarseB + kCoarseB, g.py - 1), z1 = min(bz * kCoarseB + kCoarseB, g.pz - 1);
+        float m = 0.0f;
+        for (int z = bz * kCoarseB; z <= z1; ++z)
+            for (int y = by * kCoarseB; y <= y1; ++y)
+                for (int x = bx * kCoarseB; x <= x1; ++x) m = fmaxf(m, lut[((size_t)z * g.py + y) * g.px + x]);
+        out[n] = m;
+    }
+}
+__global__ __launch_bounds__(kBlock) void lut_coarse_search_kernel(CoarseLut cl, LutGeom g, const float* __restrict__ q, size_t n, float* __restrict__ out) {
+    for (size_t i = (size_t)blockIdx.x * kBlock + threadIdx.x; i < n; i += (size_t)gridDim.x * kBlock) {
+        int ix, iy, iz;
+        float w;
+        tex_axis((q[3 * i] + g.off_x) * g.scale, g.dx, g.quantize, ix, w);
+        tex_axis((q[3 * i + 1] + g.off_y) * g.scale, g.dy, g.quantize, iy, w);
+        tex_axis((q[3 * i + 2] + g.off_z) * g.scale, g.dz, g.quantize, iz, w);
+        out[i] = cl.max[((iz >> kCoarseShift) * cl.ny + (iy >> kCoarseShift)) * cl.nx + (ix >> kCoarseShift)] * (1.0f + kCoarseMargin);
     }
 }
 
@@ -1949,6 +1989,15 @@
     hipLaunchKernelGGL(lut_unpad_kernel, dim3(4096), dim3(kBlock), 0, s, lut_padded, g, out);
 }
 
+void launch_lut_coarse_max(const float* lut_padded, const LutGeom& g, float* out, hipStream_t s) {
+    const int nx = coarse_blocks(g.px), ny = coarse_blocks(g.py), nz = coarse_blocks(g.pz);
+    const size_t total = (size_t)nx * ny * nz;
+    hipLaunchKernelGGL(lut_coarse_max_kernel, dim3((unsigned)std::min<size_t>((total + kBlock - 1) / kBlock, 65535)), dim3(kBlock), 0, s, lut_padded, g, nx, ny, nz, out);
+}
+void launch_lut_coarse_search(const CoarseLut& coarse, const LutGeom& g, const float* q_xyz, size_t n, float* out, hipStream_t s) {
+    if (n == 0) return;
+    hipLaunchKernelGGL(lut_coarse_search_kernel, dim3((unsigned)std::min<size_t>((n + kBlock - 1) / kBlock, 65535)), dim3(kBlock), 0, s, coarse, g, q_xyz, n, out);
+}
 void launch_lut_nodes(const float* lut, const LutGeom& g, const int* xyz, size_t n, float* out, hipStream_t s) {
     const unsigned blocks = (unsigned)((n + kBlock - 1) / kBlock);
     hipLaunchKernelGGL(lut_nodes_kernel, dim3(blocks < 4096 ? (blocks ? blocks : 1) : 4096), dim3(kBlock), 0, s, lut, g, xyz, n, out);
diff --git a/fast-go-icp_amd/csrc/device/kernels.hpp b/fast-go-icp_amd/csrc/device/kernels.hpp
--- a/fast-go-icp_amd/csrc/device/kernels.hpp
+++ b/fast-go-icp_amd/csrc/device/kernels.hpp
@@ -43,7 +43,7 @@
     unsigned term;
     int pad_;
 };
-constexpr unsigned kSubTerm0 = 1u, kSubTerm1 = 2u;
+constexpr unsigned kSubTerm0 = 1u, kSubTerm1 = 2u, kSubFreeUb = 4u;
 static_assert(sizeof(TickSub) == 48, "TickSub is copied in 16-byte units");
 constexpr int kCutStatSlots = 64;
 constexpr float kCutNone = 3.0e38f;
@@ -53,9 +53,24 @@
 };
 static_assert(sizeof(TickGate) == 8, "TickGate is read and written as one 8-byte word");
 constexpr unsigned kGateCutting = 1u;
-constexpr unsigned kGateTerm0 = 2u, kGateTerm1 = 4u;
+constexpr unsigned kGateTerm0 = 2u, kGateTerm1 = 4u, kGateFreeUb = 8u;
+constexpr unsigned kGateUbDecided = 1u, kGateDone = 2u;
+constexpr double kUbDecidedMarker = -2.0;
+#ifndef FGOICP_COARSE_SHIFT
+#define FGOICP_COARSE_SHIFT 3
+#endif
+constexpr int kCoarseShift = FGOICP_COARSE_SHIFT, kCoarseB = 1 << kCoarseShift;
+constexpr float kCoarseMargin = 1.0e-5f;
+struct CoarseLut {
+    const float* max = nullptr;
+    int nx = 0, ny = 0;
+};
+inline int coarse_blocks(int padded) { return ((padded - 2) >> kCoarseShift) + 1; }
 struct TickCut {
     double* acc = nullptr;
+    double* acc_ub = nullptr;
+    CoarseLut coarse;
+    unsigned long long* free_stat = nullptr;
     TickGate* gate = nullptr;
     float* row_cut = nullptr;
     unsigned* row_term = nullptr;
@@ -63,6 +78,7 @@
     const unsigned* tier_split = nullptr;
     int probe = 0;
 };
+constexpr int kFreeStatSlots = 4 * kCutStatSlots;
 constexpr int kTickNumKeys = 1 << 15;
 void launch_tick_sort(const LutGeom& g, const float4* chunk_cen, int nchunk, const TickGroup* groups, const TickSub* subs, int nsub, int cell_shift,
                       unsigned short* keys, unsigned* ranks , unsigned* hist ,
@@ -175,6 +191,8 @@
 void launch_lut_quad(const float* lut_padded, const LutGeom& g, float4* qd, hipStream_t s);
 void launch_lut_quad_apron(const float* lut_padded, const LutGeom& g, float4* qd , hipStream_t s);
 void launch_lut_zpair_apron(const float* lut_padded, const LutGeom& g, float2* zp , hipStream_t s);
+void launch_lut_coarse_max(const float* lut_padded, const LutGeom& g, float* out, hipStream_t s);
+void launch_lut_coarse_search(const CoarseLut& coarse, const LutGeom& g, const float* q_xyz, size_t n, float* out, hipStream_t s);
 void launch_lut_unpad(const float* lut_padded, const LutGeom& g, float* out, hipStream_t s);
 void launch_lut_search(const float* lut, const LutGeom& g, const float* q_xyz, size_t n, float* out, hipStream_t s);
 void launch_lut_nodes(const float* lut_padded, const LutGeom& g, const int* xyz , size_t n, float* out, hipStream_t s);
diff --git a/fast-go-icp_amd/csrc/host/driver.hpp b/fast-go-icp_amd/csrc/host/driver.hpp
--- a/fast-go-icp_amd/csrc/host/driver.hpp
+++ b/fast-go-icp_amd/csrc/host/driver.hpp
@@ -1047,8 +1047,16 @@
     static int submit_leaf(O& ops, int slot, Half& h, long) {
         return ops.bounds_submit(slot, (int)h.live.size(), h.R9.data(), h.spans.data(), h.fix.data(), h.offsets.data(), h.tn4.data(), h.twin.data(), h.cut.data());
     }
+    template <class O>
+    static auto submit_free_ub(O& ops, int slot, Half& h, int) -> decltype(ops.bounds_submit_free_ub(slot, 0, h.R9.data(), h.spans.data(), h.fix.data(), h.offsets.data(), h.tn4.data(), h.twin.data(), h.cut.data(), h.leaf.data())) {
+        return ops.bounds_submit_free_ub(slot, (int)h.live.size(), h.R9.data(), h.spans.data(), h.fix.data(), h.offsets.data(), h.tn4.data(), h.twin.data(), h.cut.data(), h.leaf.data());
+    }
+    template <class O>
+    static int submit_free_ub(O& ops, int slot, Half& h, long) {
+        return submit_leaf(ops, slot, h, 0);
+    }
     int submit_half(int slot, Half& h) {
-        if (use_cut_) return submit_leaf(ops_, slot, h, 0);
+        if (use_cut_) return submit_free_ub(ops_, slot, h, 0);
         return ops_.bounds_submit(slot, (int)h.live.size(), h.R9.data(), h.spans.data(), h.fix.data(), h.offsets.data(), h.tn4.data(), h.twin.data(), nullptr);
     }
     void consume_half(Half& h, std::vector<Task*>& tasks, bool par) {
diff --git a/fast-go-icp_amd/csrc/host/solver.cpp b/fast-go-icp_amd/csrc/host/solver.cpp
--- a/fast-go-icp_amd/csrc/host/solver.cpp
+++ b/fast-go-icp_amd/csrc/host/solver.cpp
@@ -26,6 +26,10 @@
     int bounds_submit_leaf(int slot, int G, const float* R9, const float* rot_span, const int* fix_rot, const int* offsets, const float* tn4,
                            const int* twin, const float* cut_above, const float* ub_below_span) {
         return ctx_bounds_submit(ctx, slot, G, R9, rot_span, fix_rot, offsets, tn4, twin, cut_above, ub_below_span);
+    }
+    int bounds_submit_free_ub(int slot, int G, const float* R9, const float* rot_span, const int* fix_rot, const int* offsets, const float* tn4,
+                              const int* twin, const float* cut_above, const float* ub_below_span) {
+        return ctx_bounds_submit(ctx, slot, G, R9, rot_span, fix_rot, offsets, tn4, twin, cut_above, ub_below_span, true);
     }
     int bounds_collect(int slot, float* lb, float* ub) { return ctx_bounds_collect(ctx, slot, lb, ub); }
     bool async() const { return pipeline; }
diff --git a/fast-go-icp_amd/registration.py b/fast-go-icp_amd/registration.py
--- a/fast-go-icp_amd/registration.py
+++ b/fast-go-icp_amd/registration.py
@@ -479,7 +479,21 @@
         return dict(lut_dims=tuple(i.lut_dims), lut_layout=i.lut_layout, lut_nodes=i.lut_nodes, lut_bytes=i.lut_bytes,
                     source_points_per_face_voxel=i.source_points_per_face_voxel, points_per_item=i.points_per_item,
                     items_per_evaluation=i.items_per_evaluation, max_subcubes_per_window=i.max_subcubes_per_window,
-                    source_order=i.source_order, tree_order=i.tree_order, chunks_per_item_with_thresholds=i.chunks_per_item_with_thresholds)
+                    source_order=i.source_order, tree_order=i.tree_order, chunks_per_item_with_thresholds=i.chunks_per_item_with_thresholds,
+                    coarse_block=i.coarse_block)
+
+    def lut_coarse_read(self):
+        d = (C.c_int * 3)()
+        _lib.check(self._lib.fgoicp_lut_coarse_read(self._h, d, None, 0), "fgoicp_lut_coarse_read")
+        out = np.empty(d[0] * d[1] * d[2], dtype=np.float32)
+        _lib.check(self._lib.fgoicp_lut_coarse_read(self._h, d, _fp(out), out.size), "fgoicp_lut_coarse_read")
+        return out.reshape(d[2], d[1], d[0])
+
+    def lut_coarse_search(self, queries):
+        q = _cloud(queries)
+        out = np.empty(len(q), dtype=np.float32)
+        _lib.check(self._lib.fgoicp_lut_coarse_search(self._h, _fp(q), len(q), _fp(out)), "fgoicp_lut_coarse_search")
+        return out
 
     def lut_read(self):
         dx, dy, dz = self.lut_dims()
@@ -643,7 +657,7 @@
                    "fgoicp_bounds_multi")
         return [(lb[offs[g]:offs[g + 1]], ub[offs[g]:offs[g + 1]]) for g in range(G)]
 
-    def compute_bounds_cut(self, Rs, rot_spans, fix_rots, tnode_groups, cut_above, twin=None, slot=0, ub_below_span=None):
+    def compute_bounds_cut(self, Rs, rot_spans, fix_rots, tnode_groups, cut_above, twin=None, slot=0, ub_below_span=None, free_ub=False):
         G = len(Rs)
         Rg = np.concatenate([to_glm(R) for R in Rs]).astype(np.float32) if G else np.zeros(0, np.float32)
         spans = np.asarray(rot_spans, dtype=np.float32)
@@ -659,7 +673,11 @@
         ub = np.empty(len(tn), dtype=np.float32)
         args = (self._h, int(slot), G, _fp(Rg), _fp(spans), fr.ctypes.data_as(_lib.c_int_p), offs.ctypes.data_as(_lib.c_int_p),
                 _fp(tn), None if tw is None else tw.ctypes.data_as(_lib.c_int_p), None if cut is None else _fp(cut))
-        if ub_below_span is None:
+        if free_ub:
+            leaf = None if ub_below_span is None else np.ascontiguousarray(ub_below_span, dtype=np.float32)
+            assert leaf is None or len(leaf) == G
+            _lib.check(self._lib.fgoicp_bounds_submit_free_ub(*args, None if leaf is None else _fp(leaf)), "fgoicp_bounds_submit_free_ub")
+        elif ub_below_span is None:
             _lib.check(self._lib.fgoicp_bounds_submit_cut(*args), "fgoicp_bounds_submit_cut")
         else:
             leaf = np.ascontiguousarray(ub_below_span, dtype=np.float32)
@@ -672,6 +690,11 @@
         a = C.c_uint64(); b = C.c_uint64()
         _lib.check(self._lib.fgoicp_ctx_cut_stats(self._h, C.byref(a), C.byref(b), int(reset)), "fgoicp_ctx_cut_stats")
         return a.value, b.value
+
+    def free_ub_stats(self, reset=False):
+        out = (C.c_uint64 * 4)()
+        _lib.check(self._lib.fgoicp_ctx_free_ub_stats(self._h, out, int(reset)), "fgoicp_ctx_free_ub_stats")
+        return tuple(int(v) for v in out)
 
     def procrustes(self, working):
         w = _cloud(working)
diff --git a/include/fgoicp_amd.h b/include/fgoicp_amd.h
--- a/include/fgoicp_amd.h
+++ b/include/fgoicp_amd.h
@@ -53,6 +53,7 @@
     int source_order;
     int tree_order;
     int chunks_per_item_with_thresholds;
+    int coarse_block;
 } fgoicp_ctx_info;
 int fgoicp_ctx_get_info(const fgoicp_ctx* ctx, fgoicp_ctx_info* out);
 int fgoicp_lut_nodes(fgoicp_ctx* ctx, const int* xyz, size_t n, float* out);
@@ -71,7 +72,12 @@
                              const int* offsets, const float* tnodes4, const int* twin, const float* cut_above);
 int fgoicp_bounds_submit_leaf(fgoicp_ctx* ctx, int slot, int G, const float* R9, const float* rot_span, const int* fix_rot,
                               const int* offsets, const float* tnodes4, const int* twin, const float* cut_above, const float* ub_below_span);
+int fgoicp_bounds_submit_free_ub(fgoicp_ctx* ctx, int slot, int G, const float* R9, const float* rot_span, const int* fix_rot,
+                                 const int* offsets, const float* tnodes4, const int* twin, const float* cut_above, const float* ub_below_span);
 int fgoicp_bounds_collect(fgoicp_ctx* ctx, int slot, float* lb_out, float* ub_out);
+int fgoicp_lut_coarse_read(fgoicp_ctx* ctx, int* dims3, float* out, size_t capacity_floats);
+int fgoicp_lut_coarse_search(fgoicp_ctx* ctx, const float* q_xyz, size_t n, float* out);
+int fgoicp_ctx_free_ub_stats(fgoicp_ctx* ctx, uint64_t* out4, int reset);
 int fgoicp_ctx_cut_stats(fgoicp_ctx* ctx, uint64_t* items_offered, uint64_t* items_cut, int reset);
 
 int fgoicp_sse(fgoicp_ctx* ctx, const float* R9, const float* t3, float* sse_out);
```

Result: slower. 11.91 million subcubes/s (-1.7%).
